# bergmanlab/TELR

Hardware: AMD Instinct MI355X
Metric: gbp_aligned_per_s (higher is better)
Workload: dtype int16

## Files before the change

### __graft_entry__.py

```python
import os
import sys

ROOT = os.path.dirname(os.path.abspath(__file__))
if ROOT not in sys.path:
    sys.path.insert(0, ROOT)


def build():
    from telr_amd import build as tb
    tb.build(verbose=True)
    from oracle import binding as ob
    ob.build()
    import telr_amd
    from telr_amd import _lib
    _lib.lib()


def smoke():
    import numpy as np
    from telr_amd.aligner import Engine
    from telr_amd.presets import preset
    from telr_amd.fasta import read_fasta
    from oracle import binding as ob
    d = os.path.join(ROOT, "tests", "data")
    _, ts = read_fasta(os.path.join(d, "ref_38kb.fasta"))
    _, qs = read_fasta(os.path.join(d, "reads.fasta"))
    eng = Engine(0)
    print("device:", eng.device_name())
    for pname in ("ngmlr-ont", "map-ont"):
        io, mo = preset(pname)
        ix = eng.index(ts, io)
        res = ix.map(qs, mo)
        ref = ob.OracleIndex(ts, io).map(qs, mo)
        assert len(res.alns) == len(ref["alns"]) and len(res.alns) > 0
        for f in ("qid", "tid", "qs", "qe", "ts", "te", "mlen", "blen", "dp_score", "flags", "mapq", "n_cigar"):
            np.testing.assert_array_equal(res.alns[f], ref["alns"][f], err_msg=pname + " " + f)
        for i in range(len(res.alns)):
            a, b = res.alns[i], ref["alns"][i]
            np.testing.assert_array_equal(res.cigars[a["cigar_off"]:a["cigar_off"] + a["n_cigar"]],
                                          ref["cigars"][b["cigar_off"]:b["cigar_off"] + b["n_cigar"]])
        print("smoke ok (%s): %d alignment records, bit-exact vs oracle" % (pname, len(res.alns)))


if __name__ == "__main__":
    build()
    if "--smoke" in sys.argv:
        smoke()
```

### telr_amd/_lib.py

```python
import ctypes as C
import os
from ._abi import IdxOpt, MapOpt, Aln, Counters, InsOpt, GenoOpt, DraftOpt, BridgeOpt, RefTeOpt, N_STAGES

os.environ.setdefault("GPU_MAX_HW_QUEUES", "2")
_HERE = os.path.dirname(os.path.abspath(__file__))
SO_PATH = os.environ.get("TELR_LIB") or os.path.join(_HERE, "libtelrhip.so")

EXPORTS = [
    "telr_init", "telr_destroy", "telr_strerror", "telr_last_error", "telr_device_name", "telr_preset",
    "telr_seqset_create", "telr_seqset_subset", "telr_seqset_subset_rc", "telr_seqset_free", "telr_seqset_bases", "telr_seqset_count",
    "telr_index_build", "telr_index_free", "telr_index_stats", "telr_map",
    "telr_result_from_arrays", "telr_result_count", "telr_result_alns", "telr_result_cigar_count", "telr_result_cigars", "telr_result_wait", "telr_result_free",
    "telr_init_background", "telr_release_scratch", "telr_device_mem", "telr_write_paf", "telr_write_sam", "telr_write_bam", "telr_write_bam_dev", "telr_bam_prepare", "telr_bam_release_wait", "telr_bam_discard", "telr_write_bam_slice", "telr_bam_segment_info", "telr_bam_segment_entries", "telr_bam_segment_write", "telr_bam_segment_free", "telr_bai_write", "telr_result_from_device_cigars", "telr_seqset_packed", "telr_seqset_from_packed", "telr_consensus_build", "telr_poa_build", "telr_consensus_count", "telr_consensus_seq", "telr_consensus_off", "telr_consensus_len", "telr_consensus_free", "telr_fasta_load", "telr_fasta_count", "telr_fasta_bases", "telr_fasta_extent", "telr_fasta_seq", "telr_fasta_off", "telr_fasta_len", "telr_fasta_names", "telr_fasta_free", "telr_depth_medians", "telr_window_reads", "telr_stage_ms", "telr_stage_name", "telr_last_counters", "telr_last_dp_classes",
    "telr_seqset_attach_qual", "telr_seqset_has_qual", "telr_fasta_qual", "telr_fasta_qual_off", "telr_write_sam_qual", "telr_write_bam_qual",
    "telr_ins_opt_default", "telr_call_insertions", "telr_ins_calls_count", "telr_ins_calls_calls", "telr_ins_calls_sig_count", "telr_ins_calls_sigs",
    "telr_ins_calls_read_off", "telr_ins_calls_reads", "telr_ins_calls_free",
    "telr_geno_opt_default", "telr_genotype_insertions", "telr_ins_geno_count", "telr_ins_geno_gt", "telr_ins_geno_ref_off", "telr_ins_geno_ref_reads",
    "telr_ins_geno_ambig_off", "telr_ins_geno_ambig_reads", "telr_ins_geno_free",
    "telr_draft_opt_default", "telr_draft_contigs", "telr_drafts_count", "telr_drafts_data", "telr_draft_contigs_free",
    "telr_bam_load", "telr_bam_in_free", "telr_bam_in_target_count", "telr_bam_in_target_names", "telr_bam_in_target_lens", "telr_bam_in_read_count",
    "telr_bam_in_read_names", "telr_bam_in_read_lens", "telr_bam_in_seqset", "telr_bam_in_result", "telr_bam_in_detach_seqset", "telr_bam_in_detach_result",
    "telr_bam_in_counters", "telr_bam_in_ascii", "telr_bam_in_phase_ms", "telr_bam_load_chunked", "telr_bam_chunk_plan", "telr_bam_in_chunk_info",
    "telr_seqset_extract", "telr_seqset_pieces", "telr_seqset_join",
    "telr_bridge_opt_default", "telr_bridge_contigs", "telr_bridges_count", "telr_bridges_data", "telr_bridge_contigs_free",
# ... 22 lines not shown
    L = C.CDLL(SO_PATH)
    vp, i32, i64, cp = C.c_void_p, C.c_int32, C.c_int64, C.c_char_p
    L.telr_init.restype = C.c_int; L.telr_init.argtypes = [C.c_int, C.POINTER(vp)]
    L.telr_init_background.restype = C.c_int; L.telr_init_background.argtypes = [C.c_int, C.POINTER(vp)]
    L.telr_release_scratch.restype = C.c_int; L.telr_release_scratch.argtypes = [vp]
    L.telr_device_mem.restype = C.c_int; L.telr_device_mem.argtypes = [vp, C.POINTER(i64), C.POINTER(i64)]
    L.telr_destroy.restype = None; L.telr_destroy.argtypes = [vp]
    L.telr_strerror.restype = cp; L.telr_strerror.argtypes = [C.c_int]
    L.telr_last_error.restype = cp; L.telr_last_error.argtypes = [vp]
    L.telr_device_name.restype = C.c_int; L.telr_device_name.argtypes = [vp, cp, C.c_int]
    L.telr_preset.restype = C.c_int; L.telr_preset.argtypes = [cp, C.POINTER(IdxOpt), C.POINTER(MapOpt)]
    L.telr_seqset_create.restype = C.c_int; L.telr_seqset_create.argtypes = [vp, i32, vp, vp, vp, C.POINTER(vp)]
    L.telr_seqset_subset.restype = C.c_int; L.telr_seqset_subset.argtypes = [vp, vp, i32, vp, C.POINTER(vp)]
    L.telr_seqset_subset_rc.restype = C.c_int; L.telr_seqset_subset_rc.argtypes = [vp, vp, i32, vp, vp, C.POINTER(vp)]
    L.telr_seqset_packed.restype = C.c_int; L.telr_seqset_packed.argtypes = [vp, C.POINTER(vp), C.POINTER(vp), C.POINTER(i64), C.POINTER(i64)]
    L.telr_seqset_from_packed.restype = C.c_int; L.telr_seqset_from_packed.argtypes = [vp, i32, vp, vp, i64, vp, i64, C.POINTER(vp)]
    L.telr_seqset_free.restype = None; L.telr_seqset_free.argtypes = [vp]
    L.telr_seqset_bases.restype = i64; L.telr_seqset_bases.argtypes = [vp]
    L.telr_seqset_count.restype = i32; L.telr_seqset_count.argtypes = [vp]
    L.telr_seqset_attach_qual.restype = C.c_int; L.telr_seqset_attach_qual.argtypes = [vp, vp, vp, vp, i32]
    L.telr_seqset_has_qual.restype = C.c_int; L.telr_seqset_has_qual.argtypes = [vp]
    L.telr_seqset_extract.restype = C.c_int; L.telr_seqset_extract.argtypes = [vp, vp, i64, vp, vp, vp, vp, vp, vp]
    L.telr_seqset_pieces.restype = C.c_int; L.telr_seqset_pieces.argtypes = [vp, vp, i32, vp, vp, vp, vp, C.POINTER(vp)]
    L.telr_seqset_join.restype = C.c_int; L.telr_seqset_join.argtypes = [vp, vp, i32, vp, vp, vp, vp, vp, C.POINTER(vp)]
    L.telr_tile_plan.restype = C.c_int; L.telr_tile_plan.argtypes = [i32, vp, i32, i32, vp, i64, C.POINTER(i64)]
    L.telr_refte_opt_default.restype = None; L.telr_refte_opt_default.argtypes = [C.POINTER(RefTeOpt)]
    L.telr_annotate_hits.restype = C.c_int; L.telr_annotate_hits.argtypes = [vp, vp, i64, vp, i32, vp, i32, C.POINTER(RefTeOpt), C.POINTER(vp)]
    L.telr_te_feats_count.restype = i64; L.telr_te_feats_count.argtypes = [vp]
    L.telr_te_feats_data.restype = vp; L.telr_te_feats_data.argtypes = [vp]
    L.telr_te_feats_free.restype = None; L.telr_te_feats_free.argtypes = [vp]
    L.telr_index_build.restype = C.c_int; L.telr_index_build.argtypes = [vp, vp, C.POINTER(IdxOpt), C.POINTER(vp)]
    L.telr_index_free.restype = None; L.telr_index_free.argtypes = [vp]
    L.telr_index_stats.restype = C.c_int; L.telr_index_stats.argtypes = [vp, C.POINTER(i64), C.POINTER(i64)]
    L.telr_map.restype = C.c_int; L.telr_map.argtypes = [vp, vp, vp, vp, C.POINTER(MapOpt), C.POINTER(vp)]
    L.telr_result_from_arrays.restype = C.c_int; L.telr_result_from_arrays.argtypes = [vp, vp, i64, vp, i64, C.POINTER(vp)]
    L.telr_result_count.restype = i64; L.telr_result_count.argtypes = [vp]
    L.telr_result_alns.restype = vp; L.telr_result_alns.argtypes = [vp]
    L.telr_result_cigar_count.restype = i64; L.telr_result_cigar_count.argtypes = [vp]
    L.telr_result_cigars.restype = vp; L.telr_result_cigars.argtypes = [vp]
    L.telr_result_wait.restype = C.c_int; L.telr_result_wait.argtypes = [vp]
    L.telr_result_free.restype = None; L.telr_result_free.argtypes = [vp]
    L.telr_depth_medians.restype = C.c_int
    L.telr_depth_medians.argtypes = [vp, vp, i32, vp, i32, vp, vp, vp, vp]
    L.telr_ins_opt_default.restype = None; L.telr_ins_opt_default.argtypes = [C.POINTER(InsOpt)]
    L.telr_call_insertions.restype = C.c_int; L.telr_call_insertions.argtypes = [vp, vp, i32, C.POINTER(InsOpt), C.POINTER(vp)]
    for fn in ("telr_ins_calls_count", "telr_ins_calls_sig_count"):
        getattr(L, fn).restype = i64; getattr(L, fn).argtypes = [vp]
    for fn in ("telr_ins_calls_calls", "telr_ins_calls_sigs", "telr_ins_calls_read_off", "telr_ins_calls_reads"):
        getattr(L, fn).restype = vp; getattr(L, fn).argtypes = [vp]
    L.telr_ins_calls_free.restype = None; L.telr_ins_calls_free.argtypes = [vp]
    L.telr_geno_opt_default.restype = None; L.telr_geno_opt_default.argtypes = [C.POINTER(GenoOpt)]
    L.telr_genotype_insertions.restype = C.c_int; L.telr_genotype_insertions.argtypes = [vp, vp, i32, i64, vp, vp, vp, C.POINTER(GenoOpt), C.POINTER(vp)]
    L.telr_ins_geno_count.restype = i64; L.telr_ins_geno_count.argtypes = [vp]
    for fn in ("telr_ins_geno_gt", "telr_ins_geno_ref_off", "telr_ins_geno_ref_reads", "telr_ins_geno_ambig_off", "telr_ins_geno_ambig_reads"):
        getattr(L, fn).restype = vp; getattr(L, fn).argtypes = [vp]
    L.telr_ins_geno_free.restype = None; L.telr_ins_geno_free.argtypes = [vp]
    L.telr_draft_opt_default.restype = None; L.telr_draft_opt_default.argtypes = [C.POINTER(DraftOpt)]
    L.telr_draft_contigs.restype = C.c_int
    L.telr_draft_contigs.argtypes = [vp, vp, i32, i64, vp, vp, vp, i64, vp, vp, C.POINTER(DraftOpt), C.POINTER(vp), C.POINTER(vp)]
    L.telr_drafts_count.restype = i64; L.telr_drafts_count.argtypes = [vp]
    L.telr_drafts_data.restype = vp; L.telr_drafts_data.argtypes = [vp]
    L.telr_draft_contigs_free.restype = None; L.telr_draft_contigs_free.argtypes = [vp]
    L.telr_bridge_opt_default.restype = None; L.telr_bridge_opt_default.argtypes = [C.POINTER(BridgeOpt)]
    L.telr_bridge_contigs.restype = C.c_int
    L.telr_bridge_contigs.argtypes = [vp, vp, i32, i64, vp, vp, vp, i64, vp, vp, vp, C.POINTER(BridgeOpt), C.POINTER(vp)]
    L.telr_bridges_count.restype = i64; L.telr_bridges_count.argtypes = [vp]
    L.telr_bridges_data.restype = vp; L.telr_bridges_data.argtypes = [vp]
    L.telr_bridge_contigs_free.restype = None; L.telr_bridge_contigs_free.argtypes = [vp]
    L.telr_bam_load.restype = C.c_int; L.telr_bam_load.argtypes = [vp, cp, i32, C.POINTER(vp)]
    L.telr_bam_in_free.restype = None; L.telr_bam_in_free.argtypes = [vp]
    for fn in ("telr_bam_in_target_count", "telr_bam_in_read_count"):
        getattr(L, fn).restype = i32; getattr(L, fn).argtypes = [vp]
    for fn in ("telr_bam_in_target_names", "telr_bam_in_target_lens", "telr_bam_in_read_names", "telr_bam_in_read_lens", "telr_bam_in_seqset", "telr_bam_in_result",
               "telr_bam_in_detach_seqset", "telr_bam_in_detach_result"):
        getattr(L, fn).restype = vp; getattr(L, fn).argtypes = [vp]
    L.telr_bam_in_counters.restype = C.c_int; L.telr_bam_in_counters.argtypes = [vp, vp]
    L.telr_bam_in_ascii.restype = C.c_int; L.telr_bam_in_ascii.argtypes = [vp, vp, vp]
    L.telr_bam_in_phase_ms.restype = C.c_int; L.telr_bam_in_phase_ms.argtypes = [vp, vp]
    L.telr_bam_load_chunked.restype = C.c_int; L.telr_bam_load_chunked.argtypes = [vp, cp, i32, i64, C.POINTER(vp)]
    L.telr_bam_chunk_plan.restype = C.c_int; L.telr_bam_chunk_plan.argtypes = [i64, vp, i64, vp, i64, C.POINTER(i64)]
    L.telr_bam_in_chunk_info.restype = C.c_int; L.telr_bam_in_chunk_info.argtypes = [vp, vp]
    L.telr_reads_load.restype = C.c_int; L.telr_reads_load.argtypes = [vp, cp, i32, i64, C.POINTER(vp)]
    L.telr_reads_in_free.restype = None; L.telr_reads_in_free.argtypes = [vp]
    L.telr_reads_in_count.restype = i32; L.telr_reads_in_count.argtypes = [vp]
    for fn in ("telr_reads_in_names", "telr_reads_in_lens", "telr_reads_in_seqset", "telr_reads_in_detach_seqset"):
        getattr(L, fn).restype = vp; getattr(L, fn).argtypes = [vp]
    for fn in ("telr_reads_in_counters", "telr_reads_in_chunk_info", "telr_reads_in_phase_ms"):
        getattr(L, fn).restype = C.c_int; getattr(L, fn).argtypes = [vp, vp]
    L.telr_debug_bgzf_inflate.restype = C.c_int; L.telr_debug_bgzf_inflate.argtypes = [vp, cp, vp, i64, C.POINTER(i64)]
    L.telr_debug_seqset_qual.restype = i64; L.telr_debug_seqset_qual.argtypes = [vp, vp, i64]
    L.telr_window_reads.restype = C.c_int; L.telr_window_reads.argtypes = [vp, i64, i32, vp, vp, vp, vp, vp, i64, vp]
    L.telr_write_paf.restype = C.c_int; L.telr_write_paf.argtypes = [vp, vp, vp, C.c_int, cp, C.c_int]
    L.telr_write_sam.restype = C.c_int
    L.telr_write_sam.argtypes = [vp, i32, vp, vp, vp, vp, i32, vp, vp, vp, vp, i32, cp, cp, cp, cp, cp]
    L.telr_write_bam.restype = C.c_int
    L.telr_write_bam.argtypes = [vp, i32, vp, vp, vp, vp, i32, vp, vp, vp, vp, i32, cp, cp, cp, cp, cp, i32, i32]
    L.telr_write_sam_qual.restype = C.c_int
    L.telr_write_sam_qual.argtypes = L.telr_write_sam.argtypes + [vp, vp, i32]
    L.telr_write_bam_qual.restype = C.c_int
    L.telr_write_bam_qual.argtypes = L.telr_write_bam.argtypes + [vp, vp, i32]
    L.telr_write_bam_dev.restype = C.c_int
    L.telr_write_bam_dev.argtypes = [vp, vp, vp, vp, vp, vp, i32, cp, cp, cp, cp, cp, i32, i32]
    L.telr_write_bam_dev_targets.restype = C.c_int
    L.telr_write_bam_dev_targets.argtypes = L.telr_write_bam_dev.argtypes
    L.telr_part_plan.restype = C.c_int; L.telr_part_plan.argtypes = [i32, vp, i64, vp, C.POINTER(i32)]
    L.telr_part_plan_error.restype = cp; L.telr_part_plan_error.argtypes = []
    L.telr_merge_parts.restype = C.c_int; L.telr_merge_parts.argtypes = [vp, i32, vp, vp, vp, i32, C.POINTER(MapOpt), C.POINTER(vp)]
    L.telr_debug_merge_ms.restype = C.c_int; L.telr_debug_merge_ms.argtypes = [vp]
    L.telr_fasta_load.restype = C.c_int; L.telr_fasta_load.argtypes = [cp, C.POINTER(vp)]
    L.telr_fasta_count.restype = i32; L.telr_fasta_count.argtypes = [vp]
    L.telr_fasta_bases.restype = i64; L.telr_fasta_bases.argtypes = [vp]
    L.telr_fasta_extent.restype = i64; L.telr_fasta_extent.argtypes = [vp]
    for fn in ("telr_fasta_seq", "telr_fasta_off", "telr_fasta_len", "telr_fasta_names", "telr_fasta_qual", "telr_fasta_qual_off"):
        getattr(L, fn).restype = vp; getattr(L, fn).argtypes = [vp]
    L.telr_fasta_free.restype = None; L.telr_fasta_free.argtypes = [vp]
    L.telr_consensus_build.restype = C.c_int; L.telr_consensus_build.argtypes = [vp, vp, vp, vp, i32, C.POINTER(vp)]
    L.telr_poa_build.restype = C.c_int; L.telr_poa_build.argtypes = [vp, vp, vp, vp, i32, C.POINTER(vp)]
    L.telr_consensus_count.restype = i32; L.telr_consensus_count.argtypes = [vp]
    for fn in ("telr_consensus_seq", "telr_consensus_off", "telr_consensus_len"):
        getattr(L, fn).restype = vp; getattr(L, fn).argtypes = [vp]
    L.telr_consensus_free.restype = None; L.telr_consensus_free.argtypes = [vp]
    L.telr_bam_prepare.restype = C.c_int; L.telr_bam_prepare.argtypes = [vp, cp, i64]
    L.telr_bam_release_wait.restype = C.c_int; L.telr_bam_release_wait.argtypes = []
    L.telr_bam_discard.restype = C.c_int; L.telr_bam_discard.argtypes = [vp]
    L.telr_write_bam_slice.restype = C.c_int; L.telr_write_bam_slice.argtypes = [vp, vp, vp, vp, vp, vp, i32, cp, cp, cp, cp, vp, i32, i32, C.POINTER(vp)]
    L.telr_bam_segment_info.restype = C.c_int; L.telr_bam_segment_info.argtypes = [vp, vp]
    L.telr_bam_segment_entries.restype = C.c_int; L.telr_bam_segment_entries.argtypes = [vp, i64, vp, vp, vp, vp, vp]
    L.telr_bam_segment_write.restype = C.c_int; L.telr_bam_segment_write.argtypes = [vp, vp, cp, i64, i32]
    L.telr_bam_segment_free.restype = None; L.telr_bam_segment_free.argtypes = [vp]
    L.telr_bai_write.restype = C.c_int; L.telr_bai_write.argtypes = [cp, i64, vp, vp, vp, vp, C.c_uint64, i64, i32, vp]
    L.telr_result_from_device_cigars.restype = C.c_int; L.telr_result_from_device_cigars.argtypes = [vp, vp, i64, vp, i64, C.POINTER(vp)]
    L.telr_debug_bam_twin.restype = C.c_int; L.telr_debug_bam_twin.argtypes = []
    L.telr_debug_result_twin.restype = i64; L.telr_debug_result_twin.argtypes = [vp, vp, i64]
    L.telr_debug_bam_sink_ms.restype = C.c_int; L.telr_debug_bam_sink_ms.argtypes = [vp]
    L.telr_debug_bam_ms.restype = C.c_int; L.telr_debug_bam_ms.argtypes = [vp]
    L.telr_debug_huff.restype = C.c_int; L.telr_debug_huff.argtypes = [vp, i32, i32, vp]
    L.telr_debug_check_records.restype = C.c_int; L.telr_debug_check_records.argtypes = [vp, i64, vp, i64, vp, i32, vp, i32, C.POINTER(i64)]
    L.telr_debug_deflate_host.restype = C.c_int; L.telr_debug_deflate_host.argtypes = [vp, i32, vp, i32, vp]
    L.telr_stage_ms.restype = C.c_int; L.telr_stage_ms.argtypes = [vp, vp]
    L.telr_stage_name.restype = cp; L.telr_stage_name.argtypes = [C.c_int]
    L.telr_last_counters.restype = C.c_int; L.telr_last_counters.argtypes = [vp, C.POINTER(Counters)]
    L.telr_last_dp_classes.restype = C.c_int; L.telr_last_dp_classes.argtypes = [vp, vp]
    L.telr_debug_n_anchor.restype = i64; L.telr_debug_n_anchor.argtypes = [vp]
    L.telr_debug_dp_retries.restype = i64; L.telr_debug_dp_retries.argtypes = [vp]
    L.telr_debug_pk_launches.restype = i64; L.telr_debug_pk_launches.argtypes = [vp]
    L.telr_debug_fetch.restype = C.c_int; L.telr_debug_fetch.argtypes = [vp, cp, vp, i64]
    L.telr_debug_n_chain.restype = i64; L.telr_debug_n_chain.argtypes = [vp]
    L.telr_debug_chains.restype = vp; L.telr_debug_chains.argtypes = [vp]
    L.telr_debug_index.restype = C.c_int; L.telr_debug_index.argtypes = [vp, vp, vp, vp, vp]
    L.telr_debug_pack.restype = C.c_int; L.telr_debug_pack.argtypes = [cp, i32, C.c_int, vp, vp]
    L.telr_debug_mid_occ.restype = i32; L.telr_debug_mid_occ.argtypes = [vp, C.POINTER(MapOpt)]
    L.telr_debug_dp_limits.restype = C.c_int; L.telr_debug_dp_limits.argtypes = [C.POINTER(MapOpt), vp]
    L.telr_debug_dp_class_table.restype = C.c_int; L.telr_debug_dp_class_table.argtypes = [vp]
    L.telr_debug_map_plan.restype = C.c_int; L.telr_debug_map_plan.argtypes = [vp, i32, i32, C.c_double, C.c_int, C.c_int, C.c_int, C.c_int, vp, vp]
    L.telr_debug_dp.restype = C.c_int; L.telr_debug_dp.argtypes = [vp, vp, vp, C.POINTER(MapOpt), vp, i32, vp, vp, vp, i64]
    L.telr_debug_stitch.restype = C.c_int; L.telr_debug_stitch.argtypes = [vp, i32, vp, vp, vp, vp, vp, i32, vp, vp, i64]
    L.telr_debug_align.restype = C.c_int
    L.telr_debug_align.argtypes = [vp, vp, vp, C.POINTER(MapOpt), i32, vp, vp, vp, vp, vp, vp, i64, C.POINTER(i32), vp]
    L.telr_debug_chain.restype = C.c_int; L.telr_debug_chain.argtypes = [vp, i32, vp, vp, C.POINTER(MapOpt), vp, vp]
    L.telr_debug_backtrack.restype = C.c_int
    L.telr_debug_backtrack.argtypes = [vp, i32, vp, vp, vp, vp, vp, i32, vp, vp, C.POINTER(MapOpt), vp, vp, vp, vp, vp, vp, vp, i64, vp]
    _lib = L
    return L
```

### telr_amd/aligner.py

```python
import ctypes as C
import numpy as np
from . import _lib
from ._abi import IdxOpt, MapOpt, Counters, InsOpt, GenoOpt, DraftOpt, BridgeOpt, RefTeOpt, ALN_DTYPE, INS_SIG_DTYPE, INS_CALL_DTYPE, GENO_DTYPE, DRAFT_DTYPE, BRIDGE_DTYPE, TILE_DTYPE, \
    TE_FEAT_DTYPE, TELR_E_ARG, TELR_E_RANGE, MF_PER_TARGET, MF_KEEP_CIGARS, N_STAGES, N_DPCLS, STITCH_CHAIN_COLUMNS, ALIGN_CHAIN_COLUMNS, ALIGN_PROB_COLUMNS
from .fasta import concat

BAM_CHUNK_FIT = -1

def _np_from(ptr, n, dtype):
    if n == 0 or not ptr:
        return np.zeros(0, dtype=dtype)
    dt = np.dtype(dtype)
    buf = (C.c_char * (n * dt.itemsize)).from_address(ptr)
    return np.frombuffer(buf, dtype=dt, count=n).copy()


def _ic_arrays(entry, ic, with_sigs=False):
    calls = np.ascontiguousarray(ic.calls, dtype=INS_CALL_DTYPE)
    sigs = np.ascontiguousarray(ic.sigs, dtype=INS_SIG_DTYPE) if with_sigs else None
    read_off = np.ascontiguousarray(ic.read_off, dtype=np.int64)
    reads = np.ascontiguousarray(ic.reads, dtype=np.int32)
    if len(read_off) != len(calls) + 1 or (len(calls) and int(read_off[-1]) > len(reads)):
        raise _lib.TelrError("%s: read_off must hold len(calls) + 1 offsets into reads" % entry)
    return calls, read_off, reads, sigs


def _qual_arrays(qual):
    if isinstance(qual, tuple) and len(qual) == 2:
        buf, off = qual
    else:
        buf, off, _ = concat([q.encode("latin-1") if isinstance(q, str) else q for q in qual])
    return np.ascontiguousarray(buf, dtype=np.uint8), np.ascontiguousarray(off, dtype=np.int64)


_DEFERRED = None


class deferred_frees:

    def __enter__(self):
        global _DEFERRED
        self.outer = _DEFERRED
        if _DEFERRED is None:
            _DEFERRED = []
        return self

    def __exit__(self, *exc):
        global _DEFERRED
        if self.outer is None:
            todo, _DEFERRED = _DEFERRED, None
            for fn, h in todo:
                fn(h)
        return False


class Engine:

    def __init__(self, device=0, background=False):
        self.L = _lib.lib()
        h = C.c_void_p()
        rc = (self.L.telr_init_background if background else self.L.telr_init)(device, C.byref(h))
        if rc != 0:
            raise _lib.TelrError("telr_init(%d): %s" % (device, self.L.telr_strerror(rc).decode()))
        self.h = h
        self.device = device

    def _chk(self, rc, what):
        if rc != 0:
            raise _lib.TelrError("%s: %s [%s]" % (what, self.L.telr_strerror(rc).decode(),
                                                  self.L.telr_last_error(self.h).decode()))

    def device_name(self):
        b = C.create_string_buffer(256)
        self.L.telr_device_name(self.h, b, 256)
        return b.value.decode()

    def seqset(self, seqs, qual=None):
        return SeqSet(self, seqs, qual)

    def index(self, targets, io):
        return Index(self, targets, io)

    @staticmethod
    def part_plan(lengths, max_bases=0):
        a = np.ascontiguousarray(lengths, dtype=np.int32)
        L = _lib.lib()
        part_of = np.zeros(max(len(a), 1), np.int32); n = C.c_int32(0)
        rc = L.telr_part_plan(len(a), a.ctypes.data, int(max_bases), part_of.ctypes.data, C.byref(n))
        if rc != 0:
            raise _lib.TelrError("telr_part_plan: %s [%s]" % (L.telr_strerror(rc).decode(), L.telr_part_plan_error().decode()), rc)
        return part_of[:len(a)]

    def index_parts(self, targets, io, max_part_bases=0, like=None):
        return PartIndex(self, targets, io, max_part_bases, like)

    @staticmethod
    def bam_chunk_plan(isize, chunk_bytes):
        a = np.ascontiguousarray(isize, dtype=np.int32)
        L = _lib.lib()
        first = np.zeros(max(len(a), 1), np.int64); n = C.c_int64(0)
        rc = L.telr_bam_chunk_plan(len(a), a.ctypes.data, int(chunk_bytes), first.ctypes.data, len(a), C.byref(n))
        if rc != 0:
            raise _lib.TelrError("telr_bam_chunk_plan: %s" % L.telr_strerror(rc).decode(), rc)
        return first[:int(n.value)]

    def load_bam(self, path, keep_qual=False, chunk_bytes=None):
        return BamInput(self, path, keep_qual, chunk_bytes)

    def load_reads(self, path, keep_qual=False, chunk_bytes=0):
        return ReadsInput(self, path, keep_qual, chunk_bytes)

    def stage_ms(self):
        a = np.zeros(N_STAGES, np.float32)
        self.L.telr_stage_ms(self.h, a.ctypes.data)
        return {self.L.telr_stage_name(i).decode(): float(a[i]) for i in range(N_STAGES)}

    def counters(self):
        c = Counters()
        self.L.telr_last_counters(self.h, C.byref(c))
        return {k: getattr(c, k) for k, _ in Counters._fields_}

    def dp_classes(self):
        a = np.zeros(N_DPCLS * 4, np.int64)
        self.L.telr_last_dp_classes(self.h, a.ctypes.data)
        return a.reshape(N_DPCLS, 4)

    DP_LIMITS = ("pk_steps_limit", "pk_wide_limit", "pk_wide_maxd", "pk_ext_limit", "pk_ext_maxd", "tb4_mask", "tb4_steps", "tag8_steps")

    @staticmethod
    def dp_limits(mo):
        a = np.zeros(8, np.int32)
        rc = _lib.lib().telr_debug_dp_limits(C.byref(mo), a.ctypes.data)
        if rc != 0:
            raise _lib.TelrError("telr_debug_dp_limits: %d" % rc, rc)
        return dict(zip(Engine.DP_LIMITS, (int(v) for v in a)))

    DP_CLASS_COLUMNS = ("maxd", "lanes", "regs", "row_dwords", "interleaved", "tiled")

    @staticmethod
    def dp_class_table():
        a = np.zeros((N_DPCLS, 6), np.int32)
        rc = _lib.lib().telr_debug_dp_class_table(a.ctypes.data)
        if rc != 0:
            raise _lib.TelrError("telr_debug_dp_class_table: %d" % rc, rc)
        return a

    MAP_PLAN_MODES = ("serial", "in_turn", "two_in_flight")

    @staticmethod
    def map_plan(lengths, per_base=0.0, qtarget=False, vote=False, debug=0, pipe_nomem=False):
        a = np.ascontiguousarray(lengths, dtype=np.int32)
        out = np.zeros(3, np.int64); ends = np.zeros(max(len(a), 1), np.int32)
        rc = _lib.lib().telr_debug_map_plan(a.ctypes.data, len(a), int(a.max()) if len(a) else 0, float(per_base), int(bool(qtarget)),
                                            int(bool(vote)), int(debug), int(bool(pipe_nomem)), out.ctypes.data, ends.ctypes.data)
        if rc != 0:
            raise _lib.TelrError("telr_debug_map_plan: %d" % rc, rc)
        return Engine.MAP_PLAN_MODES[int(out[0])], int(out[1]), [int(e) for e in ends[:int(out[2])]]

    @staticmethod
    def tile_plan(lengths, tile, stride):
        a = np.ascontiguousarray(lengths, dtype=np.int32)
        L = _lib.lib()
        need = C.c_int64(0)
        rc = L.telr_tile_plan(len(a), a.ctypes.data, int(tile), int(stride), None, 0, C.byref(need))
        if rc != 0 and not (rc == TELR_E_RANGE and need.value > 0):
            raise _lib.TelrError("telr_tile_plan: %s" % L.telr_strerror(rc).decode(), rc)
        out = np.zeros(need.value, TILE_DTYPE)
        if need.value:
            rc = L.telr_tile_plan(len(a), a.ctypes.data, int(tile), int(stride), out.ctypes.data, len(out), C.byref(need))
            if rc != 0:
                raise _lib.TelrError("telr_tile_plan: %s" % L.telr_strerror(rc).decode(), rc)
        return out

    def annotate_hits(self, r, tiles, target_len, n_families, opt=None):
        o = RefTeOpt.default() if opt is None else opt
        tiles = np.ascontiguousarray(tiles, dtype=TILE_DTYPE)
        tl = np.ascontiguousarray(target_len, dtype=np.int32)
        h = C.c_void_p()
        L = self.L
        rc = L.telr_annotate_hits(self.h, r, len(tiles), tiles.ctypes.data, len(tl), tl.ctypes.data, int(n_families), C.byref(o), C.byref(h))
        if rc != 0:
            raise _lib.TelrError("telr_annotate_hits: %s [%s]" % (L.telr_strerror(rc).decode(), L.telr_last_error(self.h).decode()), rc)
        try:
            return _np_from(L.telr_te_feats_data(h), int(L.telr_te_feats_count(h)), TE_FEAT_DTYPE)
        finally:
            L.telr_te_feats_free(h)

    def debug_dp(self, queries, targets, mo, probs):
        P = np.ascontiguousarray(probs, dtype=np.int32).reshape(-1, 12)
        npb = len(P)
        res = np.zeros((npb, 8), np.int32); tb = np.zeros(npb, np.int64)
        steps = P[:, 4].astype(np.int64) + P[:, 5]
        cap = int((6 * steps + 16).sum()) + 16
        cig = np.zeros(cap, np.uint32)
        self._chk(self.L.telr_debug_dp(self.h, queries.h, targets.h, C.byref(mo), P.ctypes.data, npb, res.ctypes.data,
                                       tb.ctypes.data, cig.ctypes.data, cap), "telr_debug_dp")
        out = {k: res[:, i].copy() for i, k in enumerate(("cls", "retry", "score", "bi", "bj", "mlen"))}
        out["tb_off"] = tb
        out["cigars"] = [cig[res[x, 7]:res[x, 7] + res[x, 6]].copy() for x in range(npb)]
        return out

    def debug_stitch(self, p_off, has_left, prob, cigars, cx_scale=0):
        O = np.ascontiguousarray(p_off, dtype=np.int32)
        HL = np.ascontiguousarray(has_left, dtype=np.int32)
        P = np.ascontiguousarray(prob, dtype=np.int32).reshape(-1, 5)
        if len(O) < 1 or len(HL) != len(O) - 1 or len(cigars) != len(P) or (len(O) > 1 and int(O[-1]) != len(P)):
            raise _lib.TelrError("telr_debug_stitch: p_off must hold n_chain + 1 offsets ending at the problem count", TELR_E_ARG)
        co = np.zeros(len(P) + 1, np.int64)
        co[1:] = np.cumsum([len(c) for c in cigars])
        raw = np.ascontiguousarray(np.concatenate([np.asarray(c, np.uint32) for c in cigars]) if len(cigars) else np.zeros(0), dtype=np.uint32)
        nk, cap = len(O) - 1, len(raw) + 1
        out = np.zeros((nk, len(STITCH_CHAIN_COLUMNS)), np.int32); cig = np.zeros(cap, np.uint32)
        self._chk(self.L.telr_debug_stitch(self.h, nk, O.ctypes.data, HL.ctypes.data, P.ctypes.data, co.ctypes.data, raw.ctypes.data, int(cx_scale),
                                           out.ctypes.data, cig.ctypes.data, cap), "telr_debug_stitch")
        r = {k: out[:, i].copy() for i, k in enumerate(STITCH_CHAIN_COLUMNS[:-1])}
        r["cigars"] = [cig[out[k, 8]:out[k, 8] + out[k, 7]].copy() for k in range(nk)]
        return r

    def debug_align(self, queries, targets, mo, chains, prob_off, probs):
        Cn = np.ascontiguousarray(chains, dtype=np.int32).reshape(-1, 7)
        O = np.ascontiguousarray(prob_off, dtype=np.int32)
        P = np.ascontiguousarray(probs, dtype=np.int32).reshape(-1, 12)
        if len(O) != len(Cn) + 1 or (len(Cn) and int(O[-1]) != len(P)):
            raise _lib.TelrError("telr_debug_align: prob_off must hold n_chain + 1 offsets ending at the problem count", TELR_E_ARG)
        nk, npb = len(Cn), len(P)
        cap = int((P[:, 4].astype(np.int64) + P[:, 5] + 2).sum()) + 16
        co = np.zeros((nk, len(ALIGN_CHAIN_COLUMNS)), np.int32); po = np.zeros((npb, len(ALIGN_PROB_COLUMNS)), np.int32)
        cig = np.zeros(cap, np.uint32); acc = np.zeros(N_DPCLS * 4 + 1, np.int64); n_retry = C.c_int32(0)
        self._chk(self.L.telr_debug_align(self.h, queries.h, targets.h, C.byref(mo), nk, Cn.ctypes.data, O.ctypes.data, P.ctypes.data, co.ctypes.data,
                                          po.ctypes.data, cig.ctypes.data, cap, C.byref(n_retry), acc.ctypes.data), "telr_debug_align")
        return dict(chains={k: co[:, i].copy() for i, k in enumerate(ALIGN_CHAIN_COLUMNS[:-1])},
                    cigars=[cig[co[k, 8]:co[k, 8] + co[k, 7]].copy() for k in range(nk)],
                    probs={k: po[:, i].copy() for i, k in enumerate(ALIGN_PROB_COLUMNS)}, n_retry=int(n_retry.value), acc=acc)

    def debug_chain(self, keys, q_aoff, mo):
        K = np.ascontiguousarray(keys, dtype=np.uint64)
        O = np.ascontiguousarray(q_aoff, dtype=np.int32)
        if len(O) < 1 or int(O[-1]) != len(K):
            raise ValueError("q_aoff must hold nq + 1 offsets ending at len(keys)")
        f = np.zeros(len(K), np.int32); p = np.zeros(len(K), np.int32)
        self._chk(self.L.telr_debug_chain(self.h, len(O) - 1, K.ctypes.data, O.ctypes.data, C.byref(mo), f.ctypes.data, p.ctypes.data),
                  "telr_debug_chain")
        return f, p

    def debug_backtrack(self, keys, q_aoff, f, p, qlen, goff, tlen, mo):
        K = np.ascontiguousarray(keys, dtype=np.uint64)
        O = np.ascontiguousarray(q_aoff, dtype=np.int32)
        F = np.ascontiguousarray(f, dtype=np.int32); P = np.ascontiguousarray(p, dtype=np.int32)
        QL = np.ascontiguousarray(qlen, dtype=np.int32)
        G = np.ascontiguousarray(goff, dtype=np.uint32); TL = np.ascontiguousarray(tlen, dtype=np.int32)
        nq, nt, na = len(O) - 1, len(TL), len(K)
        if nq < 0 or len(F) != na or len(P) != na or len(QL) != nq or len(G) != nt + 1:
            raise ValueError("array lengths: q_aoff nq + 1, f / p one per key, qlen nq, goff n_targets + 1")
        if nq < 1 or int(O[-1]) != na:
            raise _lib.TelrError("telr_debug_backtrack: q_aoff must hold nq + 1 >= 2 offsets ending at len(keys)")
        cap = 3 * na + 8
        ch_off = np.zeros(nq + 1, np.int32); chains = np.zeros((na + 1, 9), np.int32); ch_aoff = np.zeros(na + 2, np.int32)
        canch = np.zeros(na + 1, np.uint64); kept = np.zeros((na + 1, 10), np.int32); prob_off = np.zeros(na + 2, np.int32)
        probs = np.zeros((cap, 12), np.int32); n_out = np.zeros(3, np.int64)
        self._chk(self.L.telr_debug_backtrack(self.h, nq, O.ctypes.data, K.ctypes.data, F.ctypes.data, P.ctypes.data, QL.ctypes.data, nt,
                                              G.ctypes.data, TL.ctypes.data, C.byref(mo), ch_off.ctypes.data, chains.ctypes.data,
                                              ch_aoff.ctypes.data, canch.ctypes.data, kept.ctypes.data, prob_off.ctypes.data,
                                              probs.ctypes.data, cap, n_out.ctypes.data), "telr_debug_backtrack")
        nch, nk, npb = (int(v) for v in n_out)
        return dict(chains=chains[:nch].copy(), ch_off=ch_off, ch_aoff=ch_aoff[:nch + 1].copy(), canch=canch[:int(ch_aoff[nch])].copy(),
                    kept=kept[:nk].copy(), prob_off=prob_off[:nk + 1].copy(), probs=probs[:npb].copy())

    def release_scratch(self):
        self._chk(self.L.telr_release_scratch(self.h), "telr_release_scratch")

    def mem_info(self):
        fr, tot = C.c_int64(), C.c_int64()
        self._chk(self.L.telr_device_mem(self.h, C.byref(fr), C.byref(tot)), "telr_device_mem")
        return fr.value, tot.value

    def worker(self):
        w = getattr(self, "_worker", None)
        if w is None:
            w = self._worker = Engine(self.device, background=True)
        return w

    def close(self):
        w = getattr(self, "_worker", None)
        if w is not None:
            self._worker = None
            w.close()
        if getattr(self, "h", None):
            self.L.telr_destroy(self.h)
# ... 722 lines not shown
```

### telr_amd/build.py

```python
import os
import subprocess
import sys

HERE = os.path.dirname(os.path.abspath(__file__))
SRC = os.path.join(HERE, "csrc")
SO = os.path.join(HERE, "libtelrhip.so")
SOURCES = ["telr_engine.hip"]
DEPS = sorted(f for f in os.listdir(SRC) if f.endswith((".hip", ".h"))) + ["../../include/telr_hip.h"]


def needs_build():
    if not os.path.exists(SO):
        return True
    t = os.path.getmtime(SO)
    return any(os.path.getmtime(os.path.join(SRC, d)) > t for d in DEPS)


def build(force=False, verbose=False):
    if not force and not needs_build():
        return SO
    hipcc = os.environ.get("HIPCC", "/opt/rocm/bin/hipcc")
    cmd = [hipcc, "-O3", "-std=c++17", "--offload-arch=gfx950", "-fPIC", "-shared", "-o", SO] + \
          os.environ.get("TELR_EXTRA_FLAGS", "").split() + [os.path.join(SRC, s) for s in SOURCES] + ["-lz"]
    if verbose:
        print(" ".join(cmd), file=sys.stderr)
    subprocess.check_call(cmd)
    return SO


if __name__ == "__main__":
    build(force="--force" in sys.argv, verbose=True)
    print(SO)
```

### telr_amd/csrc/kernels.hip.h

```cpp
#pragma once
#include <hip/hip_runtime.h>
#include <stdint.h>

#define TELR_NEG      (-(1 << 28))
#include "part_plan.h"
#define SK_TILE       1024
#define SK_THREADS    256
#define DP_DMAX       4096

struct ChainOpt {
    int32_t max_gap, bw, min_cnt, min_chain_score, chain_gap_q8, chain_skip_q8;
    int32_t dense_n, dense_span, mw_n;
};
struct DpOpt {
    int32_t a, b, q, e, q2, e2, sc_ambi, zdrop;
    int32_t cx_scale, cx_open, cx_emax, cx_emin, cx_dec, cx_flat;
};
__host__ __device__ __forceinline__ int d_cx_ext(const DpOpt &o, int len) { int v = o.cx_emax - o.cx_dec * len; return v > o.cx_emin ? v : o.cx_emin; }
__host__ __device__ __forceinline__ int d_cx_cost(const DpOpt &o, int L)
{
    int t = o.cx_open;
    for (int i = 0; i < L && i < o.cx_flat; ++i) t += d_cx_ext(o, i);
    if (L > o.cx_flat) t += (L - o.cx_flat) * o.cx_emin;
    return t;
// ... 2162 lines not shown
    return c < 0 ? (int)CLS_LDSMAX : c;
}
template <typename F> constexpr uint32_t dp_cls_mask(F f) { uint32_t m = 0; for (int c = 0; c < DP_NCLS; ++c) if (f(DP_CLASS[c])) m |= 1u << c; return m; }
constexpr bool dp_row_is_reg(const DpClassRow &r) { return r.layout != TBL_BYTES; }
constexpr bool dp_row_is_rows2(const DpClassRow &r) { return r.layout == TBL_LINES || r.layout == TBL_TILES || r.layout == TBL_INTERLEAVED; }
constexpr bool dp_row_is_tiled(const DpClassRow &r) { return r.layout == TBL_TILES; }
constexpr bool dp_row_is_interleaved(const DpClassRow &r) { return r.layout == TBL_INTERLEAVED; }
constexpr bool dp_row_counts_cells(const DpClassRow &r) { return r.family == DPF_PK || r.family == DPF_PKW; }
constexpr bool dp_row_is_pk(const DpClassRow &r) { return r.family == DPF_PK; }
constexpr uint32_t CLSM_REGS = dp_cls_mask(dp_row_is_reg), CLSM_ROWS2 = dp_cls_mask(dp_row_is_rows2), CLSM_TILED = dp_cls_mask(dp_row_is_tiled),
                   CLSM_INTERLEAVED = dp_cls_mask(dp_row_is_interleaved), CLSM_CELLS = dp_cls_mask(dp_row_counts_cells), CLSM_PK = dp_cls_mask(dp_row_is_pk);
__host__ __device__ __forceinline__ constexpr bool d_cls_in(int cls, uint32_t mask) { return (mask >> cls) & 1u; }
constexpr int CLS_REGS_FIRST = __builtin_ctz(CLSM_REGS), CLS_ROWS2_FIRST = __builtin_ctz(CLSM_ROWS2);
static_assert(CLSM_REGS == ((1u << DP_NCLS) - (1u << CLS_REGS_FIRST)) && CLSM_ROWS2 == ((1u << DP_NCLS) - (1u << CLS_ROWS2_FIRST)), "these layouts take the upper class numbers");
__host__ __device__ __forceinline__ bool d_tb_regs(int cls) { return cls >= CLS_REGS_FIRST; }
__host__ __device__ __forceinline__ bool d_tb_rows2(int cls) { return cls >= CLS_ROWS2_FIRST; }
__host__ __device__ __forceinline__ bool d_tb_tiled(int cls) { return d_cls_in(cls, CLSM_TILED); }
__host__ __device__ __forceinline__ bool d_tb_interleaved(int cls) { return d_cls_in(cls, CLSM_INTERLEAVED); }
__host__ __device__ __forceinline__ int d_cls_slots(int cls) { return DP_CLASS[cls].slots; }
__host__ __device__ __forceinline__ int d_onep_d(int q, int e, int q2, int e2) { return e > e2 ? (q2 - q + (e - e2) - 1) / (e - e2) : 1 << 20; }
__host__ __device__ __forceinline__ bool d_tb4(int cls, int tb4) { return (DP_CLASS[cls].nibble & tb4) != 0; }
__host__ __device__ __forceinline__ int d_tb4_rowb(int cls) { return 4 * ((DP_CLASS[cls].regs + 1) / 2); }
__device__ __forceinline__ bool d_any_n(const uint32_t *__restrict__ nmask, int64_t lo, int n)
{
    if (n <= 0) return false;
    const int64_t hi = lo + n - 1;
    for (int64_t w = lo >> 5; w <= (hi >> 5); ++w) {
        uint32_t m = nmask[w];
        if (w == (lo >> 5)) m &= ~0u << (int)(lo & 31);
        if (w == (hi >> 5)) m &= ~0u >> (31 - (int)(hi & 31));
        if (m) return true;
    }
    return false;
}
__global__ void k_prob_sizes(DpProb *__restrict__ probs, int32_t np, int fill_margin, DpLimits L,
                             const uint32_t *__restrict__ qnmask, const uint32_t *__restrict__ tnmask,
                             int64_t *__restrict__ tb_bytes, int64_t *__restrict__ cig_ops)
{
    int i = blockIdx.x * blockDim.x + threadIdx.x;
    if (i >= np) return;
    const DpProb P = probs[i];
    int D = P.dhi - P.dlo + 1, stride = (D + 2) / 2;
    int cls = d_dp_class(P.kind, D, P.m + P.n, L);
    if (d_tb_rows2(cls) && P.kind < 3) {
        const bool hasn = d_any_n(qnmask, P.qstep > 0 ? P.qi0 : P.qi0 - P.m + 1, P.m) || d_any_n(tnmask, P.tstep > 0 ? P.ti0 : P.ti0 - P.n + 1, P.n);
        if (hasn) { DpLimits L0 = L; L0.pk_steps = L0.pk_ext = L0.pk_wide = 0; cls = d_dp_class(P.kind, D, P.m + P.n, L0); }
    }
    const int tb4 = L.tb4_mask;
    if (d_tb4(cls, tb4) && P.m + P.n > L.tb4_steps) cls = CLS_PK40;
    int64_t tb;
    if (P.kind == 5) {
        const int S = P.m < P.n ? P.m : P.n, lm = P.m < S + P.dhi ? P.m : S + P.dhi, ln = P.n < S + P.dhi ? P.n : S + P.dhi;
        tb = (2 * (int64_t)(lm + ln + 1) * (D * 4 + stride) + 127) & ~127LL;
    }
    else if (P.kind >= 3) tb = 0;
    else if (d_tb4(cls, tb4)) tb = ((int64_t)(((P.m + P.n) / 2 + 2) / 2) * (2 * d_tb4_rowb(cls)) + 63) & ~63LL;
    else if (d_tb_tiled(cls)) tb = (int64_t)(((P.m + P.n) / 2 + 4) / 4) * d_cls_slots(cls) * 16;
    else if (d_tb_rows2(cls)) tb = ((int64_t)((P.m + P.n) / 2 + 1) * d_cls_slots(cls) * 4 + 63) & ~63LL;
    else if (d_tb_regs(cls)) tb = (int64_t)((P.m + P.n) / 4 + 1) * d_cls_slots(cls) * 4;
    else tb = ((int64_t)(P.m + P.n + 1) * stride + 127) & ~127LL;
    int cells = 0;
    if (d_cls_in(cls, CLSM_CELLS)) for (int d = P.dlo; d <= P.dhi; ++d) {
        int ilo = d < 0 ? 1 - d : 1, ihi = P.n - d < P.m ? P.n - d : P.m;
        if (ihi >= ilo) cells += ihi - ilo + 1;
    }
    probs[i].pad[0] = cls | (fill_margin << 8); probs[i].pad[1] = cells;
    tb_bytes[i] = tb;
    if (P.kind == 5) { const int S = P.m < P.n ? P.m : P.n; cig_ops[i] = 3 * (int64_t)(2 * (S + P.dhi) + 2); }
    else cig_ops[i] = P.kind == 3 ? 2 : (int64_t)P.m + P.n;
}
struct ClsOff { int32_t off[DP_NCLS + 1]; };
__device__ __forceinline__ int d_cls_of_pos(const ClsOff &off, int i) { int c = 0; while (c < DP_NCLS - 1 && i >= off.off[c + 1]) ++c; return c; }
__global__ void __launch_bounds__(256) k_tb_gather(const int64_t *__restrict__ tb_bytes, const int32_t *__restrict__ list, int32_t np, ClsOff off, int64_t *__restrict__ out)
{
    const int32_t i = blockIdx.x * blockDim.x + threadIdx.x;
    if (i == np) out[np] = 0;
    if (i >= np) return;
    const int c = d_cls_of_pos(off, i);
    if (!d_tb_interleaved(c)) { out[i] = tb_bytes[list[i]]; return; }
    const int first = off.off[c] + ((i - off.off[c]) & ~63);
    const int last = first + 63 < off.off[c + 1] - 1 ? first + 63 : off.off[c + 1] - 1;
    out[i] = i == last ? tb_bytes[list[first]] * 64 : 0;
}
__global__ void __launch_bounds__(256) k_tb_scatter(DpProb *__restrict__ probs, const int32_t *__restrict__ list, int32_t np, ClsOff off, const int64_t *__restrict__ toff)
{
    const int32_t i = blockIdx.x * blockDim.x + threadIdx.x;
    if (i >= np) return;
    const int c = d_cls_of_pos(off, i);
    probs[list[i]].tb_off = toff[i] + (d_tb_interleaved(c) ? (int64_t)((i - off.off[c]) & 63) * 8 : 0);
}
__global__ void __launch_bounds__(256) k_prob_assign(DpProb *__restrict__ probs, int32_t np, const int64_t *__restrict__ tb_off, const int64_t *__restrict__ cig_off,
                                                     int32_t *__restrict__ cls_cnt, uint32_t *__restrict__ sort_key, int32_t *__restrict__ sort_val)
{
    __shared__ int32_t lcnt[DP_NCLS];
    int i = blockIdx.x * blockDim.x + threadIdx.x;
    if (threadIdx.x < DP_NCLS) lcnt[threadIdx.x] = 0;
    __syncthreads();
    if (i < np) {
        probs[i].tb_off = tb_off[i];
        if (cig_off) probs[i].cig_off = cig_off[i];
        const int c = probs[i].kind >= 3 ? 0 : (probs[i].pad[0] & 0xff);
        atomicAdd(&lcnt[c], 1);
        int steps = probs[i].m + probs[i].n; if (steps > 0x7FFFF) steps = 0x7FFFF;
        sort_key[i] = (uint32_t)c << 19 | (uint32_t)(0x7FFFF - steps);
        sort_val[i] = i;
    }
    __syncthreads();
    if (threadIdx.x < DP_NCLS && lcnt[threadIdx.x]) atomicAdd(&cls_cnt[threadIdx.x], lcnt[threadIdx.x]);
}

__global__ void k_retry_collect(const int32_t *__restrict__ flag, int32_t np, int32_t *__restrict__ cnt, int32_t *__restrict__ list)
{
    const int i = blockIdx.x * blockDim.x + threadIdx.x;
    const bool f = i < np && flag[i];
    const uint64_t m = __ballot(f);
    if (!m) return;
    const int lane = threadIdx.x & 63;
    int base = 0;
    if (lane == __ffsll((unsigned long long)m) - 1) base = atomicAdd(cnt, __popcll(m));
    base = __shfl(base, __ffsll((unsigned long long)m) - 1);
    if (f) list[base + __popcll(m & ((1ULL << lane) - 1))] = i;
}
__global__ void k_retry_build(const DpProb *__restrict__ probs, const int32_t *__restrict__ list, int32_t n, int32_t bw, int32_t band_q4, DpProb *__restrict__ out)
{
    int k = blockIdx.x * blockDim.x + threadIdx.x;
    if (k >= n) return;
    DpProb P = probs[list[k]];
    const int W = d_fill_band(P.m, P.n, bw, band_q4), W2 = d_fill_band_wide(P.m, P.n, bw, band_q4), dl = P.n - P.m;
    const int lo = d_even_lo((dl < 0 ? dl : 0) - W2), hi = (dl > 0 ? dl : 0) + W2;
    P.chain = list[k];
    P.pad[1] = 0;
    if (W2 > W && hi - lo + 1 <= DP_DMAX) { P.dlo = lo; P.dhi = hi; P.kind = 0; } else P.kind = 4;
    out[k] = P;
}
__global__ void k_retry_merge(const DpProb *__restrict__ probs2, const DpRes *__restrict__ res2, int32_t n, DpRes *__restrict__ res)
{
    int k = blockIdx.x * blockDim.x + threadIdx.x;
    if (k >= n || probs2[k].kind == 4) return;
    DpRes r = res2[k];
    r.cells += res[probs2[k].chain].cells;
    res[probs2[k].chain] = r;
}

struct DpArgs {
    const uint32_t *qseq2, *qnmask, *tseq2, *tnmask;
    int64_t qtot, ttot;
    const DpProb *probs; const int32_t *list; int32_t nlist;
    DpOpt o;
    uint8_t *tb; uint32_t *cig; DpRes *res;
    int32_t dcap;
    int32_t *retry;
    int32_t tb4;
    int32_t tag8_steps;
};

__device__ __forceinline__ int64_t d_wave_max64(int64_t v)
{
#pragma unroll
    for (int o = 32; o >= 1; o >>= 1) {
        int64_t w = (int64_t)((uint64_t)(uint32_t)__shfl_xor((int)(uint32_t)v, o) | (uint64_t)(uint32_t)__shfl_xor((int)(uint32_t)((uint64_t)v >> 32), o) << 32);
        v = w > v ? w : v;
    }
    return v;
}

__device__ __forceinline__ uint32_t d_cell(const DpOpt &o, int32_t hd, int32_t hl, int32_t e1l, int32_t e2l, int32_t hu, int32_t f1u, int32_t f2u,
                                           int qb, int tbv, int32_t &h, int32_t &ve1, int32_t &vf1, int32_t &ve2, int32_t &vf2)
{
    uint32_t t = 0; int32_t op, g;
    if (o.cx_scale) {
        const int le = e2l < 0 ? 0 : e2l > o.cx_flat ? o.cx_flat : e2l, lf = f2u < 0 ? 0 : f2u > o.cx_flat ? o.cx_flat : f2u;
        op = hl - o.cx_open - d_cx_ext(o, 0); g = e1l - d_cx_ext(o, le); if (g > op) { ve1 = g; t |= 8; ve2 = le + 1; } else { ve1 = op; ve2 = 1; }
        op = hu - o.cx_open - d_cx_ext(o, 0); g = f1u - d_cx_ext(o, lf); if (g > op) { vf1 = g; t |= 16; vf2 = lf + 1; } else { vf1 = op; vf2 = 1; }
        if (ve2 > o.cx_flat) ve2 = o.cx_flat;
        if (vf2 > o.cx_flat) vf2 = o.cx_flat;
        int scx;
        if (qb > 3 || tbv > 3) scx = -o.sc_ambi; else if (qb == tbv) { scx = o.a; t |= 128; } else scx = -o.b;
        h = hd + scx; uint32_t srcx = 0;
        if (ve1 > h) { h = ve1; srcx = 1; }
        if (vf1 > h) { h = vf1; srcx = 2; }
        return t | srcx;
    }
    op = hl - o.q - o.e;   g = e1l - o.e;  if (g > op) { ve1 = g; t |= 8; }  else ve1 = op;
    op = hu - o.q - o.e;   g = f1u - o.e;  if (g > op) { vf1 = g; t |= 16; } else vf1 = op;
    op = hl - o.q2 - o.e2; g = e2l - o.e2; if (g > op) { ve2 = g; t |= 32; } else ve2 = op;
    op = hu - o.q2 - o.e2; g = f2u - o.e2; if (g > op) { vf2 = g; t |= 64; } else vf2 = op;
    int sc;
    if (qb > 3 || tbv > 3) sc = -o.sc_ambi; else if (qb == tbv) { sc = o.a; t |= 128; } else sc = -o.b;
    h = hd + sc; uint32_t src = 0;
    if (ve1 > h) { h = ve1; src = 1; }
    if (vf1 > h) { h = vf1; src = 2; }
    if (ve2 > h) { h = ve2; src = 3; }
    if (vf2 > h) { h = vf2; src = 4; }
    return t | src;
}

__device__ __forceinline__ void d_wave_sync() { __builtin_amdgcn_fence(__ATOMIC_ACQ_REL, "workgroup"); __builtin_amdgcn_wave_barrier(); __builtin_amdgcn_fence(__ATOMIC_ACQ_REL, "workgroup"); }
__device__ __forceinline__ void d_longgap_half(const DpArgs &A, const DpProb &P, int side, int lm, int ln, int m, int n, int lane, int32_t *lds,
                                               int32_t *Hg, uint8_t *tbg, int &ncell)
{
    const DpOpt o = A.o;
    const int dlo = P.dlo, dhi = P.dhi, D = dhi - dlo + 1, stride = (D + 2) / 2;
    const int qstep = side ? -P.qstep : P.qstep, tstep = side ? -P.tstep : P.tstep;
    const int64_t qi0 = side ? P.qi0 + (int64_t)P.qstep * (m - 1) : P.qi0, ti0 = side ? P.ti0 + (int64_t)P.tstep * (n - 1) : P.ti0;
    int32_t *H = lds, *E1 = H + (A.dcap + 2), *F1 = E1 + (A.dcap + 2), *E2 = F1 + (A.dcap + 2), *F2 = E2 + (A.dcap + 2);
    d_wave_sync();
    for (int x = lane; x < D + 2; x += 64) { H[x] = TELR_NEG; E1[x] = TELR_NEG; F1[x] = TELR_NEG; E2[x] = TELR_NEG; F2[x] = TELR_NEG; }
    d_wave_sync();
    if (lane == 0) { H[0 - dlo + 1] = 0; Hg[0 - dlo] = 0; }
    d_wave_sync();
    for (int a = 1; a <= lm + ln; ++a) {
        int d0 = -a > dlo ? -a : dlo; if (a - 2 * lm > d0) d0 = a - 2 * lm;
        int d1 = a < dhi ? a : dhi;   if (2 * ln - a < d1) d1 = 2 * ln - a;
        if (((d0 - a) & 1) != 0) ++d0;
        for (int d = d0 + 2 * lane; d <= d1; d += 128) {
            const int i = (a - d) >> 1, j = (a + d) >> 1, x = d - dlo + 1;
            int32_t h, ve1, vf1, ve2, vf2;
            if (i == 0) { ve1 = -(o.q + j * o.e); ve2 = -(o.q2 + j * o.e2); vf1 = vf2 = TELR_NEG; h = ve1 > ve2 ? ve1 : ve2; }
            else if (j == 0) { vf1 = -(o.q + i * o.e); vf2 = -(o.q2 + i * o.e2); ve1 = ve2 = TELR_NEG; h = vf1 > vf2 ? vf1 : vf2; }
            else {
                int qb = d_base(A.qseq2, A.qnmask, qi0 + (int64_t)qstep * (i - 1));
                int tbv = d_base(A.tseq2, A.tnmask, ti0 + (int64_t)tstep * (j - 1));
                if (P.qcomp && qb < 4) qb = 3 - qb;
                const uint32_t t = d_cell(o, H[x], H[x - 1], E1[x - 1], E2[x - 1], H[x + 1], F1[x + 1], F2[x + 1], qb, tbv, h, ve1, vf1, ve2, vf2);
                tbg[(int64_t)a * stride + ((d - dlo) >> 1)] = (uint8_t)t;
                ++ncell;
            }
            if (h < TELR_NEG) h = TELR_NEG;
            if (ve1 < TELR_NEG) ve1 = TELR_NEG;
            if (vf1 < TELR_NEG) vf1 = TELR_NEG;
            if (ve2 < TELR_NEG) ve2 = TELR_NEG;
            if (vf2 < TELR_NEG) vf2 = TELR_NEG;
            H[x] = h; E1[x] = ve1; F1[x] = vf1; E2[x] = ve2; F2[x] = vf2;
            Hg[(int64_t)a * D + (d - dlo)] = h;
        }
        d_wave_sync();
    }
}
__device__ __forceinline__ int d_longgap_walk(const uint8_t *tbg, int dlo, int stride, int i, int j, uint32_t *out, int no, int &mcols, int &mlen)
{
    int state = 0;
    auto push = [&](uint32_t op) { if (no > 0 && (out[no - 1] & 0xfu) == op) out[no - 1] += 16u; else out[no++] = 16u | op; };
    while (i > 0 && j > 0) {
        const uint32_t t = tbg[(int64_t)(i + j) * stride + ((j - i - dlo) >> 1)];
        if (state == 0) state = (int)(t & 7u);
        if (state == 0) { push(0u); ++mcols; mlen += (int)(t >> 7 & 1u); --i; --j; }
        else if (state == 1) { push(2u); if (!(t & 8u))  state = 0; --j; }
        else if (state == 2) { push(1u); if (!(t & 16u)) state = 0; --i; }
        else if (state == 3) { push(2u); if (!(t & 32u)) state = 0; --j; }
        else                 { push(1u); if (!(t & 64u)) state = 0; --i; }
    }
    if (i > 0) { if (no > 0 && (out[no - 1] & 0xfu) == 1u) out[no - 1] += (uint32_t)i << 4; else out[no++] = (uint32_t)i << 4 | 1u; }
    if (j > 0) { if (no > 0 && (out[no - 1] & 0xfu) == 2u) out[no - 1] += (uint32_t)j << 4; else out[no++] = (uint32_t)j << 4 | 2u; }
    return no;
}
__device__ void d_longgap(const DpArgs &A, const DpProb &P, int prob, int lane, int32_t *lds)
{
    const DpOpt o = A.o;
    const int m = P.m, n = P.n, ins = m > n, S = ins ? n : m, W = P.dhi, dlo = P.dlo, D = P.dhi - dlo + 1, stride = (D + 2) / 2;
    const int lm = m < S + W ? m : S + W, ln = n < S + W ? n : S + W, na = lm + ln + 1;
    uint8_t *base = A.tb + P.tb_off;
    int32_t *HL = (int32_t*)base, *HR = HL + (int64_t)na * D;
    uint8_t *tbL = (uint8_t*)(HR + (int64_t)na * D), *tbR = tbL + (int64_t)na * stride;
    int ncell = 0;
    d_longgap_half(A, P, 0, lm, ln, m, n, lane, lds, HL, tbL, ncell);
    d_longgap_half(A, P, 1, lm, ln, m, n, lane, lds, HR, tbR, ncell);
    __threadfence_block();
    d_wave_sync();
    const int lim = ins ? lm : ln;
    int64_t bestk = INT64_MIN; int b_al = 0, b_ar = 0;
    for (int c = lane; c <= S; c += 64) {
        int64_t vl = INT64_MIN, vr = INT64_MIN; int al = 0, ar = 0;
        for (int k = c - W; k <= c + W; ++k) {
            if (k < 0 || k > lim) continue;
            const int i = ins ? k : c, j = ins ? c : k, d = j - i;
            if (d < dlo || d > P.dhi) continue;
            const int32_t h = HL[(int64_t)(i + j) * D + (d - dlo)];
            if (h <= TELR_NEG / 2) continue;
            const int64_t v = (int64_t)h + (int64_t)o.e2 * k;
            if (v > vl) { vl = v; al = k; }
        }
        const int c2 = S - c;
        for (int k = c2 - W; k <= c2 + W; ++k) {
            if (k < 0 || k > lim) continue;
            const int i = ins ? k : c2, j = ins ? c2 : k, d = j - i;
            if (d < dlo || d > P.dhi) continue;
            const int32_t h = HR[(int64_t)(i + j) * D + (d - dlo)];
            if (h <= TELR_NEG / 2) continue;
            const int64_t v = (int64_t)h + (int64_t)o.e2 * k;
            if (v > vr) { vr = v; ar = k; }
        }
        if (vl == INT64_MIN || vr == INT64_MIN) continue;
        if ((ins ? m : n) - al - ar < 1) continue;
        const int64_t key = (vl + vr) * 65536LL + (int64_t)(0xffff - c);
        if (key > bestk) { bestk = key; b_al = al; b_ar = ar; }
    }
    const int64_t wk = d_wave_max64(bestk);
    const uint64_t who = __ballot(bestk == wk);
    const int src = __ffsll((unsigned long long)who) - 1;
    const int bc = 0xffff - (int)(wk & 0xffff), al = __shfl(b_al, src), ar = __shfl(b_ar, src);
    int nc = ncell;
#pragma unroll
    for (int s = 32; s >= 1; s >>= 1) nc += __shfl_xor(nc, s);
    if (lane == 0) {
        const int g = (ins ? m : n) - al - ar;
        const int li = ins ? al : bc, lj = ins ? bc : al, ri = ins ? ar : S - bc, rj = ins ? S - bc : ar;
// ... 255 lines not shown
    uint32_t tbw[R];
#pragma unroll
    for (int r = 0; r < R; ++r) tbw[r] = 0;
    int ncell = 0;
    for (int a = 1; a <= amax; ++a) {
        const int sh = 8 * (a & 3);
        if (a & 1) {
            if ((((a - 1) >> 1) & 31) == 0) d_stream_fill(TS, A.tseq2, A.tnmask, P.ti0, ts_, ((a + de0 + 1) >> 1) + R - 2, 0, A.ttot);
#pragma unroll
            for (int r = 0; r < R - 1; ++r) tbs[r] = tbs[r + 1];
            tbs[R - 1] = d_stream_next(TS);
            int32_t hu = DPP_SHL1(TELR_NEG, He[0]), f1u = DPP_SHL1(TELR_NEG, F1e[0]), f2u = DPP_SHL1(TELR_NEG, F2e[0]);
            if (LPP < 64 && l == LPP - 1) { hu = TELR_NEG; f1u = TELR_NEG; f2u = TELR_NEG; }
            if (NW > 1 && wl == 63 && wv < NW - 1) { const int32_t *x = xch + (0 * NW + wv + 1) * 3; hu = x[0]; f1u = x[1]; f2u = x[2]; }
#pragma unroll
            for (int r = 0; r < R; ++r) {
                const int32_t uh = r < R - 1 ? He[r < R - 1 ? r + 1 : r] : hu, uf1 = r < R - 1 ? F1e[r < R - 1 ? r + 1 : r] : f1u, uf2 = r < R - 1 ? F2e[r < R - 1 ? r + 1 : r] : f2u;
                if ((uint32_t)(a - aloO[r]) <= (uint32_t)spanO[r]) {
                    int32_t h, ve1, vf1, ve2, vf2;
                    uint32_t t = d_cell_nc(o, Ho[r], He[r], E1e[r], E2e[r], uh, uf1, uf2, qbs[r], tbs[r], h, ve1, vf1, ve2, vf2);
                    tbw[r] |= t << sh; ++ncell;
                    Ho[r] = h; E1o[r] = ve1; F1o[r] = vf1; E2o[r] = ve2; F2o[r] = vf2;
                }
            }
        } else {
            if ((((a >> 1) - 1) & 31) == 0) d_stream_fill(QS, A.qseq2, A.qnmask, P.qi0, qs_, ((a - de0) >> 1) - 1, P.qcomp, A.qtot);
#pragma unroll
            for (int r = R - 1; r > 0; --r) qbs[r] = qbs[r - 1];
            qbs[0] = d_stream_next(QS);
            int32_t hl = DPP_SHR1(TELR_NEG, Ho[R - 1]), e1l = DPP_SHR1(TELR_NEG, E1o[R - 1]), e2l = DPP_SHR1(TELR_NEG, E2o[R - 1]);
            if (LPP < 64 && l == 0) { hl = TELR_NEG; e1l = TELR_NEG; e2l = TELR_NEG; }
            if (NW > 1 && wl == 0 && wv > 0) { const int32_t *x = xch + (1 * NW + wv - 1) * 3; hl = x[0]; e1l = x[1]; e2l = x[2]; }
#pragma unroll
            for (int r = R - 1; r >= 0; --r) {
                const int32_t lh = r > 0 ? Ho[r > 0 ? r - 1 : 0] : hl, le1 = r > 0 ? E1o[r > 0 ? r - 1 : 0] : e1l, le2 = r > 0 ? E2o[r > 0 ? r - 1 : 0] : e2l;
                if ((uint32_t)(a - aloE[r]) <= (uint32_t)spanE[r]) {
                    int32_t h, ve1, vf1, ve2, vf2;
                    uint32_t t = d_cell_nc(o, He[r], lh, le1, le2, Ho[r], F1o[r], F2o[r], qbs[r], tbs[r], h, ve1, vf1, ve2, vf2);
                    tbw[r] |= t << sh; ++ncell;
                    He[r] = h; E1e[r] = ve1; F1e[r] = vf1; E2e[r] = ve2; F2e[r] = vf2;
                }
            }
        }
        if (NW > 1) {
            if (a & 1) { if (wl == 63) { int32_t *x = xch + (1 * NW + wv) * 3; x[0] = Ho[R - 1]; x[1] = E1o[R - 1]; x[2] = E2o[R - 1]; } }
            else if (wl == 0) { int32_t *x = xch + (0 * NW + wv) * 3; x[0] = He[0]; x[1] = F1e[0]; x[2] = F2e[0]; }
            __syncthreads();
        }
        if ((a & 3) == 3 || a == amax) {
            if ((a >> 2) <= last_row) {
#pragma unroll
                for (int r = 0; r < R; ++r) tb32[(int64_t)(a >> 2) * SLOTS + l * R + r] = tbw[r];
            }
#pragma unroll
            for (int r = 0; r < R; ++r) tbw[r] = 0;
        }
    }
#pragma unroll
    for (int s = (NW > 1 ? 32 : LPP / 2); s >= 1; s >>= 1) ncell += __shfl_xor(ncell, s);
    if (NW > 1) {
        if (wl == 0) atomicAdd(&ncell_sh, ncell);
        __syncthreads();
        ncell = ncell_sh;
    }
    if (have) {
        const int xf = (n - m) - de0;
        if (xf >= 0 && xf < 2 * R) {
            int32_t sc = TELR_NEG;
#pragma unroll
            for (int r = 0; r < R; ++r) { if (xf == 2 * r) sc = He[r]; if (xf == 2 * r + 1) sc = Ho[r]; }
            DpRes Rr; Rr.score = sc; Rr.bi = m; Rr.bj = n; Rr.nops = 0; Rr.mlen = 0; Rr.cells = ncell; Rr.tbases = n; Rr.mcols = 0;
            A.res[prob] = Rr;
        }
    }
}

typedef short pk_s2 __attribute__((ext_vector_type(2)));
__device__ __forceinline__ pk_s2 PKS(uint32_t v) { return __builtin_bit_cast(pk_s2, v); }
__device__ __forceinline__ uint32_t PKU(pk_s2 v) { return __builtin_bit_cast(uint32_t, v); }
__device__ __forceinline__ uint32_t pk_add(uint32_t a, uint32_t b) { return PKU(PKS(a) + PKS(b)); }
__device__ __forceinline__ uint32_t pk_sub(uint32_t a, uint32_t b) { return PKU(PKS(a) - PKS(b)); }
__device__ __forceinline__ uint32_t pk_max(uint32_t a, uint32_t b) { return PKU(__builtin_elementwise_max(PKS(a), PKS(b))); }
__device__ __forceinline__ uint32_t pk_min(uint32_t a, uint32_t b) { return PKU(__builtin_elementwise_min(PKS(a), PKS(b))); }
__device__ __forceinline__ uint32_t pk_mul(uint32_t a, uint32_t b) { return PKU(PKS(a) * PKS(b)); }
__device__ __forceinline__ uint32_t pk_sign(uint32_t a)
{
    uint32_t r;
    asm("v_pk_ashrrev_i16 %0, 15, %1 op_sel_hi:[0,1]" : "=v"(r) : "v"(a));
    return r;
}
__device__ __forceinline__ uint32_t pk_sel(uint32_t m, uint32_t a, uint32_t b)
{
    uint32_t r;
    asm("v_bfi_b32 %0, %1, %2, %3" : "=v"(r) : "v"(m), "v"(a), "v"(b));
    return r;
}
__device__ __forceinline__ uint32_t pk_dup(int v) { return ((uint32_t)v & 0xffffu) * 0x00010001u; }
#define PK_NEG 0xC000C000u
#ifdef TB_NT
typedef uint32_t tb_u2 __attribute__((ext_vector_type(2)));
#define TB_ST2(p, a, b) __builtin_nontemporal_store(tb_u2{(a), (b)}, (tb_u2*)(p))
#define TB_LD2(p) ({ const tb_u2 v_ = __builtin_nontemporal_load((const tb_u2*)(p)); make_uint2(v_.x, v_.y); })
#else
#define TB_ST2(p, a, b) (*(uint2*)(p) = make_uint2((a), (b)))
#define TB_LD2(p) (*(const uint2*)(p))
#endif

struct PkConst { uint32_t qe, e, q2e2, e2, ab, b, a, nab, qeF, q2e2F;
                 uint32_t cx_oe0, cx_e1, cx_emin, cx_dec; };

template <bool ONEP = false>
__device__ __forceinline__ uint32_t d_cell_pk(const PkConst &c, uint32_t hd, uint32_t hl, uint32_t e1l, uint32_t e2l, uint32_t hu, uint32_t f1u, uint32_t f2u,
                                              uint32_t qb, uint32_t tbv, uint32_t &h, uint32_t &ve1, uint32_t &vf1, uint32_t &ve2, uint32_t &vf2)
{
    uint32_t op, g, t;
    op = pk_sub(hl, c.qe);   g = pk_sub(e1l, c.e);  ve1 = pk_max(op, g); t  = pk_sign(pk_sub(op, g)) & 0x00080008u;
    op = pk_sub(hu, c.qe);   g = pk_sub(f1u, c.e);  vf1 = pk_max(op, g); t |= pk_sign(pk_sub(op, g)) & 0x00100010u;
    if (!ONEP) {
        op = pk_sub(hl, c.q2e2); g = pk_sub(e2l, c.e2); ve2 = pk_max(op, g); t |= pk_sign(pk_sub(op, g)) & 0x00200020u;
        op = pk_sub(hu, c.q2e2); g = pk_sub(f2u, c.e2); vf2 = pk_max(op, g); t |= pk_sign(pk_sub(op, g)) & 0x00400040u;
    } else { ve2 = PK_NEG; vf2 = PK_NEG; }
    const uint32_t eq = pk_sign(pk_sub(qb ^ tbv, 0x00010001u));
    const uint32_t sc = pk_sub(eq & c.ab, c.b);
    t |= eq & 0x00800080u;
    h = pk_add(hd, sc);
    uint32_t m, src;
    m = pk_sign(pk_sub(h, ve1)); h = pk_max(h, ve1); src = m & 0x00010001u;
    m = pk_sign(pk_sub(h, vf1)); h = pk_max(h, vf1); src = pk_sel(m, 0x00020002u, src);
    if (!ONEP) {
        m = pk_sign(pk_sub(h, ve2)); h = pk_max(h, ve2); src = pk_sel(m, 0x00030003u, src);
        m = pk_sign(pk_sub(h, vf2)); h = pk_max(h, vf2); src = pk_sel(m, 0x00040004u, src);
    }
    return t | src;
}

__device__ __forceinline__ uint32_t d_cell_pk_cx(const PkConst &c, uint32_t hd, uint32_t hl, uint32_t el, uint32_t xel, uint32_t hu, uint32_t fu, uint32_t xfu,
                                                 uint32_t qb, uint32_t tbv, uint32_t &h, uint32_t &ve, uint32_t &vf, uint32_t &nxe, uint32_t &nxf)
{
    uint32_t op, g, m, t;
    op = pk_sub(hl, c.cx_oe0); g = pk_sub(el, xel); ve = pk_max(op, g); m = pk_sign(pk_sub(op, g)); t  = m & 0x00080008u;
    nxe = pk_sel(m, pk_max(pk_sub(xel, c.cx_dec), c.cx_emin), c.cx_e1);
    op = pk_sub(hu, c.cx_oe0); g = pk_sub(fu, xfu); vf = pk_max(op, g); m = pk_sign(pk_sub(op, g)); t |= m & 0x00100010u;
    nxf = pk_sel(m, pk_max(pk_sub(xfu, c.cx_dec), c.cx_emin), c.cx_e1);
    const uint32_t eq = pk_sign(pk_sub(qb ^ tbv, 0x00010001u));
    const uint32_t sc = pk_sub(eq & c.ab, c.b);
    t |= eq & 0x00800080u;
    h = pk_add(hd, sc);
    uint32_t src;
    m = pk_sign(pk_sub(h, ve)); h = pk_max(h, ve); src = m & 0x00010001u;
    m = pk_sign(pk_sub(h, vf)); h = pk_max(h, vf); src = pk_sel(m, 0x00020002u, src);
    return t | src;
}

template <int SH>
__device__ __forceinline__ uint32_t d_cell_pk4(const PkConst &c, uint32_t hd, uint32_t hl, uint32_t e1l, uint32_t hu, uint32_t f1u,
                                               uint32_t qb, uint32_t tbv, uint32_t &h, uint32_t &ve1, uint32_t &vf1)
{
    const uint32_t et = pk_max(pk_sub(hl, c.qe), pk_sub(e1l, c.e));
    const uint32_t ft = pk_max(pk_sub(hu, c.qeF), pk_sub(f1u, c.e));
    asm("v_and_or_b32 %0, %1, %2, %3" : "=v"(ve1) : "v"(et), "v"(0xFFFCFFFCu), "v"(0x00010001u));
    vf1 = ft & 0xFFFCFFFCu;
    uint32_t ne, hda = pk_add(hd, c.a), ht;
    asm("v_pk_min_u16 %0, %1, %2" : "=v"(ne) : "v"(qb ^ tbv), "v"(0x00010001u));
    asm("v_pk_mad_i16 %0, %1, %2, %3" : "=v"(ht) : "v"(ne), "v"(c.nab), "v"(hda));
    ht = pk_max(pk_max(ht, ve1), vf1);
    h = ht & 0xFFFCFFFCu;
    uint32_t n = ht & 0x00030003u;
    asm("v_lshl_or_b32 %0, %1, %2, %3" : "=v"(n) : "v"(et & 0x00010001u), "v"(2), "v"(n));
    asm("v_lshl_or_b32 %0, %1, %2, %3" : "=v"(n) : "v"(ft & 0x00010001u), "v"(3), "v"(n));
    return SH ? n << SH : n;
}

__device__ __forceinline__ uint32_t d_cell_pk8(const PkConst &c, uint32_t hd, uint32_t hl, uint32_t e1l, uint32_t e2l, uint32_t hu, uint32_t f1u, uint32_t f2u,
                                               uint32_t qb, uint32_t tbv, uint32_t &h, uint32_t &ve1, uint32_t &vf1, uint32_t &ve2, uint32_t &vf2)
{
    const uint32_t et1 = pk_max(pk_sub(hl, c.qe), pk_sub(e1l, c.e));
    const uint32_t ft1 = pk_max(pk_sub(hu, c.qeF), pk_sub(f1u, c.e));
    const uint32_t et2 = pk_max(pk_sub(hl, c.q2e2), pk_sub(e2l, c.e2));
    const uint32_t ft2 = pk_max(pk_sub(hu, c.q2e2F), pk_sub(f2u, c.e2));
    asm("v_and_or_b32 %0, %1, %2, %3" : "=v"(ve1) : "v"(et1), "v"(0xFFF8FFF8u), "v"(0x00030003u));
    asm("v_and_or_b32 %0, %1, %2, %3" : "=v"(vf1) : "v"(ft1), "v"(0xFFF8FFF8u), "v"(0x00020002u));
    asm("v_and_or_b32 %0, %1, %2, %3" : "=v"(ve2) : "v"(et2), "v"(0xFFF8FFF8u), "v"(0x00010001u));
    vf2 = ft2 & 0xFFF8FFF8u;
    uint32_t ne, hda = pk_add(hd, c.a), ht;
    asm("v_pk_min_u16 %0, %1, %2" : "=v"(ne) : "v"(qb ^ tbv), "v"(0x00010001u));
    asm("v_pk_mad_i16 %0, %1, %2, %3" : "=v"(ht) : "v"(ne), "v"(c.nab), "v"(hda));
    ht = pk_max(pk_max(ht, ve1), pk_max(vf1, pk_max(ve2, vf2)));
    h = ht & 0xFFF8FFF8u;
    uint32_t n = ht & 0x00070007u;
    asm("v_lshl_or_b32 %0, %1, %2, %3" : "=v"(n) : "v"(et1 & 0x00010001u), "v"(3), "v"(n));
    asm("v_lshl_or_b32 %0, %1, %2, %3" : "=v"(n) : "v"(ft1 & 0x00010001u), "v"(4), "v"(n));
    asm("v_lshl_or_b32 %0, %1, %2, %3" : "=v"(n) : "v"(et2 & 0x00010001u), "v"(5), "v"(n));
    asm("v_lshl_or_b32 %0, %1, %2, %3" : "=v"(n) : "v"(ft2 & 0x00010001u), "v"(6), "v"(n));
    return n;
}

template <int R> __device__ __forceinline__ void d_push_q(uint32_t (&qb)[R], uint32_t v)
{
#pragma unroll
    for (int r = R - 1; r >= 1; --r) qb[r] = __builtin_amdgcn_alignbit(qb[r], qb[r - 1], 16);
    qb[0] = (qb[0] << 16) | v;
}
template <int R> __device__ __forceinline__ void d_push_t(uint32_t (&tb)[R], uint32_t v)
{
#pragma unroll
    for (int r = 0; r < R - 1; ++r) tb[r] = __builtin_amdgcn_alignbit(tb[r + 1], tb[r], 16);
    tb[R - 1] = (tb[R - 1] >> 16) | (v << 16);
}

template <int LPP, int R> __device__ __forceinline__ int d_pk_rowmax(const uint32_t (&hv)[R])
{
    uint32_t M = hv[0];
#pragma unroll
    for (int r = 1; r < R; ++r) M = pk_max(M, hv[r]);
    int lo = (int)(short)(M & 0xffffu), hi = (int)M >> 16, cur = lo > hi ? lo : hi;
#pragma unroll
    for (int s = 1; s < LPP; s <<= 1) { const int v = __shfl_xor(cur, s); cur = v > cur ? v : cur; }
    return cur;
}
template <int LPP, int R> __device__ __forceinline__ int d_pk_argd(const uint32_t (&hv)[R], int cur, int de0, int par)
{
    int d = 0x7fffffff;
#pragma unroll
    for (int r = R - 1; r >= 0; --r) {
        const int lo = (int)(short)(hv[r] & 0xffffu), hi = (int)hv[r] >> 16;
        if (hi == cur) d = de0 + 4 * r + 2 + par;
        if (lo == cur) d = de0 + 4 * r + par;
    }
#pragma unroll
    for (int s = 1; s < LPP; s <<= 1) { const int v = __shfl_xor(d, s); d = v < d ? v : d; }
    return d;
}
__device__ __forceinline__ int d_step_cells(int a, int m, int n, int dlo, int dhi)
{
    int lo = dlo > a - 2 * m ? dlo : a - 2 * m; if (2 - a > lo) lo = 2 - a;
    int hi = dhi < 2 * n - a ? dhi : 2 * n - a; if (a - 2 < hi) hi = a - 2;
    if ((lo - a) & 1) ++lo;
    return hi >= lo ? ((hi - lo) >> 1) + 1 : 0;
}

template <int LPP, int R, bool EXT, int NW = 1, int FULL = 0, bool ONEP = false, bool TB4 = false, bool TAG8 = false, bool CX = false>
__device__ __forceinline__ void d_dp_pkr(const DpArgs &A, const int32_t *__restrict__ list, int nlist, int first_prob, uint32_t *xch = nullptr)
{
    static_assert(NW == 1 || LPP == 64 * NW, "multi-wave problems use whole waves");
    static_assert(!TB4 || (ONEP && LPP == 1 && !EXT), "nibble spill: one-piece cell, one problem per lane");
    static_assert(!TAG8 || (!ONEP && !TB4 && !EXT && NW == 1), "tagged two-piece cell: fills of the one-launch classes");
    static_assert(!CX || (!ONEP && !TB4 && !TAG8), "convex cell: plain flags, byte spill");
    constexpr int RW = LPP * R;
    const int lane = threadIdx.x, sub = lane / LPP, l = lane % LPP;
    const int wv = NW > 1 ? lane >> 6 : 0, wl = lane & 63;
    const int pi = first_prob + sub;
    const bool have = pi < nlist;
    const int prob = list[have ? pi : 0];
    const DpProb P = A.probs[prob];
    const DpOpt o = A.o;
    PkConst c; c.qe = pk_dup(o.q + o.e); c.e = pk_dup(o.e); c.q2e2 = pk_dup(o.q2 + o.e2); c.e2 = pk_dup(o.e2);
    c.ab = pk_dup(o.a + o.b); c.b = pk_dup(o.b); c.a = pk_dup(o.a); c.nab = pk_dup(-(o.a + o.b)); c.qeF = c.qe;
    c.q2e2F = c.q2e2;
    c.cx_oe0 = pk_dup(o.cx_open + d_cx_ext(o, 0)); c.cx_e1 = pk_dup(d_cx_ext(o, 1)); c.cx_emin = pk_dup(o.cx_emin); c.cx_dec = pk_dup(o.cx_dec);
    const uint32_t XN = CX ? c.cx_emin : PK_NEG;
    if constexpr (TB4) {
        c.qe = pk_dup(4 * (o.q + o.e) - 2); c.qeF = pk_dup(4 * (o.q + o.e) - 1); c.e = pk_dup(4 * o.e);
        c.a = pk_dup(4 * o.a + 2); c.nab = pk_dup(-4 * (o.a + o.b));
    }
    if constexpr (TAG8) {
        c.qe = pk_dup(8 * (o.q + o.e) - 4); c.qeF = pk_dup(8 * (o.q + o.e) - 3); c.e = pk_dup(8 * o.e);
        c.q2e2 = pk_dup(8 * (o.q2 + o.e2) - 2); c.q2e2F = pk_dup(8 * (o.q2 + o.e2) - 1); c.e2 = pk_dup(8 * o.e2);
        c.a = pk_dup(8 * o.a + 4); c.nab = pk_dup(-8 * (o.a + o.b));
    }
    const int m = have ? P.m : 0, n = have ? P.n : 0, dlo = P.dlo;
    const int de0 = dlo + 4 * R * l;
    const int dhi = have ? P.dhi : dlo - 1;
    uint32_t He[R], E1e[R], E2e[R], F1e[R], F2e[R], Ho[R], E1o[R], E2o[R], F1o[R], F2o[R], inE[R], inO[R], qb[R], tbv[R];
#pragma unroll
    for (int r = 0; r < R; ++r) {
        He[r] = E1e[r] = F1e[r] = Ho[r] = E1o[r] = F1o[r] = PK_NEG; E2e[r] = F2e[r] = E2o[r] = F2o[r] = XN;
        if constexpr (TB4) { E1e[r] |= 0x00010001u; E1o[r] |= 0x00010001u; }
        if constexpr (TAG8) { E1e[r] |= 0x00030003u; E1o[r] |= 0x00030003u; F1e[r] |= 0x00020002u; F1o[r] |= 0x00020002u; E2e[r] |= 0x00010001u; E2o[r] |= 0x00010001u; }
        const int d0 = de0 + 4 * r;
        if (d0 == 0) He[r] &= 0xffff0000u;
        if (d0 + 2 == 0) He[r] &= 0x0000ffffu;
        inE[r] = (d0 <= dhi ? 0x0000ffffu : 0u) | (d0 + 2 <= dhi ? 0xffff0000u : 0u);
        inO[r] = (d0 + 1 <= dhi ? 0x0000ffffu : 0u) | (d0 + 3 <= dhi ? 0xffff0000u : 0u);
        qb[r] = 0; tbv[r] = 0;
    }
    const int mn = m + n;
    int amax = mn, amin = have ? mn : 0x7fffffff;
    if (NW == 1) {
#pragma unroll
        for (int s = 32; s >= 1; s >>= 1) { int v = __shfl_xor(amax, s); amax = v > amax ? v : amax; v = __shfl_xor(amin, s); amin = v < amin ? v : amin; }
    }
    amin = __builtin_amdgcn_readfirstlane(amin);
    uint32_t *tb32 = (uint32_t*)(A.tb + P.tb_off) + (EXT ? ((l * R) >> 2) * 16 + ((l * R) & 3) : l * R);
    const int last_row = have ? mn >> 1 : -1;
    const int qs_ = P.qstep, ts_ = P.tstep;
    BaseStream QS, TS;
    d_stream_fill_acgt(QS, A.qseq2, P.qi0, qs_, -(de0 >> 1) - 2 * R, P.qcomp, A.qtot);
    d_stream_fill_acgt(TS, A.tseq2, P.ti0, ts_, (de0 >> 1) - 1, 0, A.ttot);
#pragma unroll
    for (int z = 0; z < 2 * R; ++z) {
        uint32_t qv = (uint32_t)d_stream_next_acgt(QS), tv = (uint32_t)d_stream_next_acgt(TS);
        if (EXT) { if (-(de0 >> 1) - 2 * R + z >= m) qv |= 8u; if ((de0 >> 1) - 1 + z >= n) tv |= 8u; }
        d_push_q<R>(qb, qv); d_push_t<R>(tbv, tv);
    }
    int qleft = 32 - 2 * R, tleft = 32 - 2 * R;
    int best = 0, bi = 0, bj = 0, prev_cur = -16384, done = have ? 0 : 1, ncell = 0;
    const int zdrop = o.zdrop;
    constexpr bool REB = CX;
    int off = 0, fin_off = 0;
    const bool first = l == 0, last = l == LPP - 1;
    const int xf = (n - m) - de0;
    const bool fin_here = have && xf >= 0 && xf < 4 * R;
    const int fin_r = xf >> 2, fin_hi = (xf >> 1) & 1;
    uint32_t fin = PK_NEG, te[R], prow[R];
#pragma unroll
    for (int r = 0; r < R; ++r) { te[r] = 0; prow[r] = 0; }
    if (NW > 1) {
        if (wl == 0) { uint32_t *x = xch + (0 * NW + wv) * 3; x[0] = He[0]; x[1] = F1e[0]; x[2] = F2e[0]; }
        __syncthreads();
    }
    for (int k = 0; 2 * k <= amax; ++k) {
        uint32_t h, ve1, vf1, ve2, vf2;
        if (k > 0) {
            const int a = 2 * k;
            if (qleft == 0) { d_stream_fill_acgt(QS, A.qseq2, P.qi0, qs_, ((a - de0) >> 1) - 1, P.qcomp, A.qtot); qleft = 32; }
            { uint32_t qv = (uint32_t)d_stream_next_acgt(QS); if (EXT && ((a - de0) >> 1) - 1 >= m) qv |= 8u; d_push_q<R>(qb, qv); } --qleft;
            uint32_t ph = PK_NEG, pe1 = PK_NEG, pe2 = XN;
            if (LPP > 1) {
                ph = DPP_SHR1((int)PK_NEG, (int)Ho[R - 1]); pe1 = DPP_SHR1((int)PK_NEG, (int)E1o[R - 1]); pe2 = DPP_SHR1((int)XN, (int)E2o[R - 1]);
                if (NW > 1 && wl == 0 && wv > 0) { const uint32_t *x = xch + (1 * NW + wv - 1) * 3; ph = x[0]; pe1 = x[1]; pe2 = x[2]; }
                if (first) { ph = PK_NEG; pe1 = PK_NEG; pe2 = XN; }
            }
#pragma unroll
            for (int r = 0; r < R; ++r) {
                const uint32_t lh = r ? Ho[r - 1] : ph, le1 = r ? E1o[r - 1] : pe1, le2 = r ? E2o[r - 1] : pe2;
                const uint32_t hl = __builtin_amdgcn_alignbit(Ho[r], lh, 16), e1l = __builtin_amdgcn_alignbit(E1o[r], le1, 16), e2l = __builtin_amdgcn_alignbit(E2o[r], le2, 16);
                if constexpr (TB4) { te[r] = d_cell_pk4<0>(c, He[r], hl, e1l, Ho[r], F1o[r], qb[r], tbv[r], h, ve1, vf1); ve2 = PK_NEG; vf2 = PK_NEG; }
                else if constexpr (TAG8) te[r] = d_cell_pk8(c, He[r], hl, e1l, e2l, Ho[r], F1o[r], F2o[r], qb[r], tbv[r], h, ve1, vf1, ve2, vf2);
                else if constexpr (CX) te[r] = d_cell_pk_cx(c, He[r], hl, e1l, e2l, Ho[r], F1o[r], F2o[r], qb[r], tbv[r], h, ve1, vf1, ve2, vf2);
                else te[r] = d_cell_pk<ONEP>(c, He[r], hl, e1l, e2l, Ho[r], F1o[r], F2o[r], qb[r], tbv[r], h, ve1, vf1, ve2, vf2);
                if (r < FULL) { He[r] = h; F1e[r] = vf1; F2e[r] = vf2; }
                else { He[r] = (h & inE[r]) | (PK_NEG & ~inE[r]); F1e[r] = (vf1 & inE[r]) | (PK_NEG & ~inE[r]); F2e[r] = (vf2 & inE[r]) | (XN & ~inE[r]); }
                E1e[r] = ve1; E2e[r] = ve2;
            }
            if (!EXT && a >= amin) {
#pragma unroll
                for (int r = 0; r < R; ++r) if (a == mn && r == fin_r) { fin = He[r]; fin_off = off; }
            }
            if (NW > 1) {
                if (wl == 0) { uint32_t *x = xch + (0 * NW + wv) * 3; x[0] = He[0]; x[1] = F1e[0]; x[2] = F2e[0]; }
                __syncthreads();
            }
            if (EXT) {
                uint32_t hv[R];
#pragma unroll
                for (int r = 0; r < R; ++r) hv[r] = pk_sel(pk_sign(PKU(PKS(qb[r] | tbv[r]) << (pk_s2)(12))), PK_NEG, He[r]);
                const int cur_rel = d_pk_rowmax<LPP, R>(hv), cur = cur_rel + off;
                if (!done) {
                    if (cur > best) { const int cd = d_pk_argd<LPP, R>(hv, cur_rel, de0, 0); best = cur; bi = (a - cd) >> 1; bj = (a + cd) >> 1; }
                    ncell += d_step_cells(a, m, n, dlo, dhi);
                    if (best - (cur > prev_cur ? cur : prev_cur) > zdrop || a >= mn) done = 1;
                }
                prev_cur = cur;
            }
        }
        {
            const int a = 2 * k + 1;
            if (tleft == 0) { d_stream_fill_acgt(TS, A.tseq2, P.ti0, ts_, ((a + de0 + 1) >> 1) + 2 * R - 2, 0, A.ttot); tleft = 32; }
            { uint32_t tv = (uint32_t)d_stream_next_acgt(TS); if (EXT && ((a + de0 + 1) >> 1) + 2 * R - 2 >= n) tv |= 8u; d_push_t<R>(tbv, tv); } --tleft;
            uint32_t nh = PK_NEG, nf1 = PK_NEG, nf2 = XN;
            if (LPP > 1) {
                nh = DPP_SHL1((int)PK_NEG, (int)He[0]); nf1 = DPP_SHL1((int)PK_NEG, (int)F1e[0]); nf2 = DPP_SHL1((int)XN, (int)F2e[0]);
                if (NW > 1 && wl == 63 && wv < NW - 1) { const uint32_t *x = xch + (0 * NW + wv + 1) * 3; nh = x[0]; nf1 = x[1]; nf2 = x[2]; }
                if (last) { nh = PK_NEG; nf1 = PK_NEG; nf2 = XN; }
            }
            uint32_t row[R];
#pragma unroll
            for (int r = 0; r < R; ++r) {
                const uint32_t uh = r < R - 1 ? He[r + 1] : nh, uf1 = r < R - 1 ? F1e[r + 1] : nf1, uf2 = r < R - 1 ? F2e[r + 1] : nf2;
                const uint32_t hu = __builtin_amdgcn_alignbit(uh, He[r], 16), f1u = __builtin_amdgcn_alignbit(uf1, F1e[r], 16), f2u = __builtin_amdgcn_alignbit(uf2, F2e[r], 16);
                uint32_t t;
                if constexpr (TB4) { t = d_cell_pk4<4>(c, Ho[r], He[r], E1e[r], hu, f1u, qb[r], tbv[r], h, ve1, vf1); ve2 = PK_NEG; vf2 = PK_NEG; }
                else if constexpr (TAG8) t = d_cell_pk8(c, Ho[r], He[r], E1e[r], E2e[r], hu, f1u, f2u, qb[r], tbv[r], h, ve1, vf1, ve2, vf2);
                else if constexpr (CX) t = d_cell_pk_cx(c, Ho[r], He[r], E1e[r], E2e[r], hu, f1u, f2u, qb[r], tbv[r], h, ve1, vf1, ve2, vf2);
                else t = d_cell_pk<ONEP>(c, Ho[r], He[r], E1e[r], E2e[r], hu, f1u, f2u, qb[r], tbv[r], h, ve1, vf1, ve2, vf2);
                if (r < FULL) { Ho[r] = h; F1o[r] = vf1; F2o[r] = vf2; }
                else { Ho[r] = (h & inO[r]) | (PK_NEG & ~inO[r]); F1o[r] = (vf1 & inO[r]) | (PK_NEG & ~inO[r]); F2o[r] = (vf2 & inO[r]) | (XN & ~inO[r]); }
                E1o[r] = ve1; E2o[r] = ve2;
                row[r] = TB4 ? (te[r] | t) : __builtin_amdgcn_perm(t, te[r], 0x06040200u);
            }
            if (!EXT && a >= amin) {
#pragma unroll
                for (int r = 0; r < R; ++r) if (a == mn && r == fin_r) { fin = Ho[r]; fin_off = off; }
            }
            if (EXT) {
                uint32_t hv[R];
#pragma unroll
                for (int r = 0; r < R; ++r) hv[r] = pk_sel(pk_sign(PKU(PKS(qb[r] | tbv[r]) << (pk_s2)(12))), PK_NEG, Ho[r]);
                const int cur_rel = d_pk_rowmax<LPP, R>(hv), cur = cur_rel + off;
                if (!done) {
                    if (cur > best) { const int cd = d_pk_argd<LPP, R>(hv, cur_rel, de0, 1); best = cur; bi = (a - cd) >> 1; bj = (a + cd) >> 1; }
                    ncell += d_step_cells(a, m, n, dlo, dhi);
                    if (best - (cur > prev_cur ? cur : prev_cur) > zdrop || a >= mn) done = 1;
                }
                prev_cur = cur;
            }
            if constexpr (TB4) {
                constexpr int RW4 = (R + 1) / 2;
                uint32_t rq[RW4];
#pragma unroll
                for (int j = 0; j < RW4; ++j) rq[j] = __builtin_amdgcn_perm(2 * j + 1 < R ? row[2 * j + 1] : 0u, row[2 * j], 0x06040200u);
                uint32_t sq[2 * RW4 + 1];
                if (k & 1) {
#pragma unroll
                    for (int j = 0; j < RW4; ++j) { sq[j] = prow[j]; sq[RW4 + j] = rq[j]; }
                    sq[2 * RW4] = 0;
                    uint32_t *dst = tb32 + (int64_t)((k - 1) / 2 * RW4) * 128;
                    if (k <= last_row) {
#pragma unroll
                        for (int u = 0; u < RW4; ++u) TB_ST2(dst + u * 128, sq[2 * u], sq[2 * u + 1]);
                    } else if (k - 1 <= last_row) {
#pragma unroll
                        for (int u = 0; u < (RW4 + 1) / 2; ++u) TB_ST2(dst + u * 128, sq[2 * u], sq[2 * u + 1]);
                    }
                } else {
#pragma unroll
                    for (int j = 0; j < RW4; ++j) prow[j] = rq[j];
                    if (2 * (k + 1) > amax && k <= last_row) {
#pragma unroll
                        for (int j = 0; j < RW4; ++j) sq[j] = rq[j];
                        sq[RW4] = 0;
                        uint32_t *dst = tb32 + (int64_t)(k / 2 * RW4) * 128;
#pragma unroll
                        for (int u = 0; u < (RW4 + 1) / 2; ++u) TB_ST2(dst + u * 128, sq[2 * u], sq[2 * u + 1]);
                    }
                }
            } else if constexpr (LPP == 1 && !EXT) {
                uint32_t sq[2 * R + 1];
                if (k & 1) {
#pragma unroll
                    for (int r = 0; r < R; ++r) { sq[r] = prow[r]; sq[R + r] = row[r]; }
                    sq[2 * R] = 0;
                    uint32_t *dst = tb32 + (int64_t)((k - 1) / 2 * R) * 128;
                    if (k <= last_row) {
#pragma unroll
                        for (int u = 0; u < R; ++u) TB_ST2(dst + u * 128, sq[2 * u], sq[2 * u + 1]);
                    } else if (k - 1 <= last_row) {
#pragma unroll
                        for (int u = 0; u < (R + 1) / 2; ++u) TB_ST2(dst + u * 128, sq[2 * u], sq[2 * u + 1]);
                    }
                } else {
#pragma unroll
                    for (int r = 0; r < R; ++r) prow[r] = row[r];
                    if (2 * (k + 1) > amax && k <= last_row) {
#pragma unroll
                        for (int r = 0; r < R; ++r) sq[r] = row[r];
                        sq[R] = 0;
                        uint32_t *dst = tb32 + (int64_t)(k / 2 * R) * 128;
#pragma unroll
                        for (int u = 0; u < (R + 1) / 2; ++u) TB_ST2(dst + u * 128, sq[2 * u], sq[2 * u + 1]);
                    }
                }
            } else if constexpr (EXT) {
                static_assert(!EXT || R == 4 || R == 1, "tiled spill: a lane owns a whole 16-byte group (R = 4) or one dword of it (R = 1)");
                if (k <= last_row) {
                    uint32_t *dst = tb32 + (int64_t)(k >> 2) * (4 * RW) + (k & 3) * 4;
                    if constexpr (R == 4) *(uint4*)dst = make_uint4(row[0], row[1], row[2], row[3]);
                    else dst[0] = row[0];
                }
            } else if (k <= last_row) {
                uint32_t *dst = tb32 + (int64_t)k * RW;
                if constexpr (R % 4 == 0) {
#pragma unroll
                    for (int r = 0; r < R; r += 4) *(uint4*)(dst + r) = make_uint4(row[r], row[r + 1], row[r + 2], row[r + 3]);
                } else if constexpr (R % 2 == 0) {
#pragma unroll
                    for (int r = 0; r < R; r += 2) *(uint2*)(dst + r) = make_uint2(row[r], row[r + 1]);
                } else {
#pragma unroll
                    for (int r = 0; r < R; ++r) dst[r] = row[r];
                }
            }
        }
        if constexpr (REB) {
            if ((k & 31) == 31) {
                uint32_t hv[R];
#pragma unroll
                for (int r = 0; r < R; ++r) hv[r] = pk_max(He[r], Ho[r]);
                int mx = d_pk_rowmax<(LPP > 64 ? 64 : LPP), R>(hv);
                if (NW > 1) {
                    int32_t *xm = (int32_t*)(xch + 2 * NW * 3);
                    if (wl == 0) xm[wv] = mx;
                    __syncthreads();
#pragma unroll
                    for (int w_ = 0; w_ < NW; ++w_) mx = xm[w_] > mx ? xm[w_] : mx;
                }
                const int delta = mx < -8192 ? 0 : mx;
                const uint32_t dd = pk_dup(delta), thr = pk_dup(delta - 12000);
#define REB_ONE(x) { const uint32_t dead = pk_sign(pk_sub((x), thr)); (x) = pk_sel(dead, PK_NEG, pk_max(pk_sub((x), dd), PK_NEG)); }
#pragma unroll
                for (int r = 0; r < R; ++r) { REB_ONE(He[r]) REB_ONE(Ho[r]) REB_ONE(E1e[r]) REB_ONE(E1o[r]) REB_ONE(F1e[r]) REB_ONE(F1o[r]) }
#undef REB_ONE
                off += delta;
            }
        }
        if (NW > 1) {
            if (wl == 63) { uint32_t *x = xch + (1 * NW + wv) * 3; x[0] = Ho[R - 1]; x[1] = E1o[R - 1]; x[2] = E2o[R - 1]; }
            __syncthreads();
        }
        if (EXT && __all(done)) break;
    }
    if (EXT) {
        if (have && l == 0) {
            DpRes Rr; Rr.score = best; Rr.bi = bi; Rr.bj = bj; Rr.nops = 0; Rr.mlen = 0; Rr.cells = ncell; Rr.tbases = n; Rr.mcols = 0;
            A.res[prob] = Rr;
        }
        return;
    }
    if (fin_here) {
        int sc = (int)(short)(fin_hi ? (fin >> 16) : (fin & 0xffffu)) + fin_off;
        if constexpr (TB4) sc >>= 2;
        if constexpr (TAG8) sc >>= 3;
        DpRes Rr; Rr.score = sc; Rr.bi = m; Rr.bj = n; Rr.nops = 0; Rr.mlen = 0; Rr.cells = P.pad[1]; Rr.tbases = n; Rr.mcols = 0;
        A.res[prob] = Rr;
    }
}

#define PK_NC 9
static_assert(__builtin_popcount(CLSM_PK) == PK_NC, "PK_NC counts the DPF_PK rows of DP_CLASS");
__host__ __device__ __forceinline__ constexpr int PK_IDX(int cls) { return __builtin_popcount(CLSM_PK & ((1u << cls) - 1u)); }
__host__ __device__ __forceinline__ constexpr int PK_CLS(int c) { int cls = 0; for (int k = 0; k < DP_NCLS; ++k) if (d_cls_in(k, CLSM_PK) && PK_IDX(k) == c) cls = k; return cls; }
struct PkPlan { int32_t woff[PK_NC + 1]; };
__global__ void k_pk_waves(const DpProb *__restrict__ probs, const int32_t *__restrict__ cls_list, ClsOff off, PkPlan plan,
                           uint32_t *__restrict__ keys, uint32_t *__restrict__ vals)
{
    const int i = blockIdx.x * blockDim.x + threadIdx.x;
    if (i >= plan.woff[PK_NC]) return;
    int c = 0;
    while (i >= plan.woff[c + 1]) ++c;
    const int cls = PK_CLS(c), first = (i - plan.woff[c]) * (64 / DP_CLASS[cls].lpp);
    const DpProb P = probs[cls_list[off.off[cls] + first]];
    const uint32_t cost = (uint32_t)((P.m + P.n) * DP_CLASS[cls].regs);
    keys[i] = cost > 0xFFFFu ? 0xFFFFu : cost;
    vals[i] = (uint32_t)cls << 26 | (uint32_t)first;
}
enum PkCell : int { CELL_PLAIN, CELL_TAG8, CELL_CX, CELL_ONEP, CELL_NIBBLE };
__device__ __forceinline__ int d_pk_cell(int cls, const DpOpt &o, int tb4, int tag8_steps, const DpProb *__restrict__ probs, const int32_t *__restrict__ first)
{
    if (o.cx_scale) return CELL_CX;
    const int onep_d = d_onep_d(o.q, o.e, o.q2, o.e2);
    static_assert(DP_CLASS[CLS_PK16].nibble == 1 && DP_CLASS[CLS_PK20].nibble == 2, "the nibble classes and their tb4_mask bits");
    if ((cls == CLS_PK16 && onep_d >= DP_CLASS[CLS_PK16].maxd) || (cls == CLS_PK20 && onep_d >= DP_CLASS[CLS_PK20].maxd)) return d_tb4(cls, tb4) ? CELL_NIBBLE : CELL_ONEP;
    const DpProb P0 = probs[*first];
    return P0.m + P0.n <= tag8_steps ? CELL_TAG8 : CELL_PLAIN;
}
template <int CLS, bool EXACT, bool ONEP, bool TB4, bool TAG8, bool CX>
__device__ __forceinline__ void d_dp_pk_cls(const DpArgs &A, const int32_t *__restrict__ list, int n, int first)
{
    static_assert(DP_CLASS[CLS].family == DPF_PK && EXACT == (DP_CLASS[CLS].layout == TBL_INTERLEAVED && CLS != CLS_PK16), "class table");
    d_dp_pkr<DP_CLASS[CLS].lpp, DP_CLASS[CLS].regs, false, 1, EXACT ? DP_CLASS[CLS].regs - 1 : 0, ONEP, TB4, TAG8, CX>(A, list, n, first);
}
template <bool TAG8, bool CX>
__device__ __forceinline__ void d_dp_pk_any(int cls, const DpArgs &A, const int32_t *__restrict__ list, int n, int first)
{
    switch (cls) {
    case CLS_PK20: d_dp_pk_cls<CLS_PK20, true, false, false, TAG8, CX>(A, list, n, first); break;
    case CLS_PK24: d_dp_pk_cls<CLS_PK24, true, false, false, TAG8, CX>(A, list, n, first); break;
    case CLS_PK28: d_dp_pk_cls<CLS_PK28, true, false, false, TAG8, CX>(A, list, n, first); break;
    case CLS_PK32: d_dp_pk_cls<CLS_PK32, true, false, false, TAG8, CX>(A, list, n, first); break;
    case CLS_PK16: d_dp_pk_cls<CLS_PK16, false, false, false, TAG8, CX>(A, list, n, first); break;
    case CLS_PK40: d_dp_pk_cls<CLS_PK40, false, false, false, TAG8, CX>(A, list, n, first); break;
    case CLS_PK48: d_dp_pk_cls<CLS_PK48, false, false, false, TAG8, CX>(A, list, n, first); break;
    case CLS_PK128: d_dp_pk_cls<CLS_PK128, false, false, false, TAG8, CX>(A, list, n, first); break;
    default: d_dp_pk_cls<CLS_PK64, false, false, false, TAG8, CX>(A, list, n, first); break;
    }
}
#ifndef PK_WPE
#define PK_WPE 2
#endif
__global__ void __launch_bounds__(64) __attribute__((amdgpu_waves_per_eu(PK_WPE))) k_dp_pk(DpArgs A, const uint32_t *__restrict__ waves, const int32_t *__restrict__ cls_list,
                                              ClsOff off)
{
    const uint32_t w = waves[blockIdx.x];
    const int cls = (int)(w >> 26), first = (int)(w & 0x3ffffffu);
    const int32_t *list = cls_list + off.off[cls];
    const int n = off.off[cls + 1] - off.off[cls];
    const int cell = d_pk_cell(cls, A.o, A.tb4, A.tag8_steps, A.probs, list + first);
    if (cell == CELL_CX) { d_dp_pk_any<false, true>(cls, A, list, n, first); return; }
    if (cell >= CELL_ONEP && cls == CLS_PK16) { if (cell == CELL_NIBBLE) d_dp_pk_cls<CLS_PK16, false, true, true, false, false>(A, list, n, first); else d_dp_pk_cls<CLS_PK16, false, true, false, false, false>(A, list, n, first); return; }
    if (cell >= CELL_ONEP) { if (cell == CELL_NIBBLE) d_dp_pk_cls<CLS_PK20, true, true, true, false, false>(A, list, n, first); else d_dp_pk_cls<CLS_PK20, true, true, false, false, false>(A, list, n, first); return; }
    if (cell == CELL_TAG8) { d_dp_pk_any<true, false>(cls, A, list, n, first); return; }
    d_dp_pk_any<false, false>(cls, A, list, n, first);
}
template <int NW>
__global__ void __launch_bounds__(64 * NW) k_dp_pkw(DpArgs A)
{
    __shared__ uint32_t xch[2 * NW * 3 + NW];
    __builtin_amdgcn_s_setprio(3);
    if (A.o.cx_scale) d_dp_pkr<64 * NW, 1, false, NW, 0, false, false, false, true>(A, A.list, A.nlist, blockIdx.x, xch);
    else d_dp_pkr<64 * NW, 1, false, NW>(A, A.list, A.nlist, blockIdx.x, xch);
}
constexpr int PKX_LPP = DP_CLASS[CLS_PKX64].lpp, PKX_R = DP_CLASS[CLS_PKX64].regs;
__global__ void __launch_bounds__(64) k_dp_pkx(DpArgs A)
{
    __builtin_amdgcn_s_setprio(3);
    if (A.o.cx_scale) d_dp_pkr<PKX_LPP, PKX_R, true, 1, 0, false, false, false, true>(A, A.list, A.nlist, blockIdx.x * (64 / PKX_LPP));
    else d_dp_pkr<PKX_LPP, PKX_R, true>(A, A.list, A.nlist, blockIdx.x * (64 / PKX_LPP));
}
__global__ void __launch_bounds__(64) k_dp_pkx16(DpArgs A)
{
    __builtin_amdgcn_s_setprio(3);
    if (A.o.cx_scale) d_dp_pkr<16, 1, true, 1, 0, false, false, false, true>(A, A.list, A.nlist, blockIdx.x * 4);
    else d_dp_pkr<16, 1, true>(A, A.list, A.nlist, blockIdx.x * 4);
}

constexpr int PKX8_LPP = DP_CLASS[CLS_PKX128].lpp;
static_assert(DP_CLASS[CLS_PKX128].regs == 32 / PKX8_LPP && DP_CLASS[CLS_PKX256].lpp == 16 && DP_CLASS[CLS_PKX256].regs == 4, "class table");
__global__ void __launch_bounds__(64) k_dp_pkx_w8(DpArgs A)
{
    __builtin_amdgcn_s_setprio(3);
    if (A.o.cx_scale) d_dp_pkr<PKX8_LPP, 32 / PKX8_LPP, true, 1, 0, false, false, false, true>(A, A.list, A.nlist, blockIdx.x * (64 / PKX8_LPP));
    else d_dp_pkr<PKX8_LPP, 32 / PKX8_LPP, true>(A, A.list, A.nlist, blockIdx.x * (64 / PKX8_LPP));
}
__global__ void __launch_bounds__(64) k_dp_pkx_w16(DpArgs A)
{
    __builtin_amdgcn_s_setprio(3);
    if (A.o.cx_scale) d_dp_pkr<16, 4, true, 1, 0, false, false, false, true>(A, A.list, A.nlist, blockIdx.x * 4);
    else d_dp_pkr<16, 4, true>(A, A.list, A.nlist, blockIdx.x * 4);
}

#ifndef TB_SLOTS
#define TB_SLOTS 2
#endif
template <int LAYOUT>
__device__ __forceinline__ void d_traceback_lane(const DpProb *__restrict__ probs, DpRes *__restrict__ res, int pi,
                                                 const uint8_t *__restrict__ tb_all, uint32_t *__restrict__ cig, int32_t *__restrict__ retry,
                                                 uint32_t *stage)
{
    const int lane = threadIdx.x;
    const DpProb P = probs[pi];
    if (P.kind >= 3) return;
    const int dhi_ = P.dhi; int touched = 0;
    const int cls = P.pad[0] & 0xff, dlo = P.dlo, mg = P.pad[0] >> 8;
    const int D = P.dhi - dlo + 1, stride = (D + 2) / 2;
    const int lpp = d_cls_slots(cls);
    const bool packed = d_tb_regs(cls), tiled = d_tb_tiled(cls), rows2 = d_tb_rows2(cls);
    int i = res[pi].bi, j = res[pi].bj;
    uint32_t *cg = cig + P.cig_off;
    int no = 0, ml = 0, mc = 0, state = 0, cur_op = -1, cur_len = 0;
    const int rowb = tiled ? lpp * 16 : packed ? lpp * 4 : stride;
    int64_t tag0 = -1, tag1 = -1, pfb = -2;
    uint4 v0 = make_uint4(0, 0, 0, 0), v1 = v0, v2 = v0, v3 = v0, v4 = v0, v5 = v0, v6 = v0, v7 = v0;
    while (i > 0 && j > 0) {
        const int a = i + j, sl = (j - i - dlo) >> 1;
        const int64_t off = tiled ? ((((int64_t)(a >> 3) * (4 * lpp) + ((sl >> 3) << 4) + (((a >> 1) & 3) << 2) + ((sl >> 1) & 3)) << 2) + ((a & 1) << 1) + (sl & 1))
                          : (LAYOUT == 2 || rows2) ? ((((int64_t)(a >> 1) * lpp + (sl >> 1)) << 2) + ((a & 1) << 1) + (sl & 1))
                          : packed ? ((((int64_t)(a >> 2) * lpp + sl) << 2) + (a & 3)) : ((int64_t)a * stride + sl);
        const int64_t abs_off = P.tb_off + (d_tb_interleaved(cls) ? ((off >> 3) << 9) + (off & 7) : off), line = abs_off >> 6;
        const int slot = TB_SLOTS > 1 ? (int)(line & 1) : 0;
        if ((slot ? tag1 : tag0) != line) {
            const int64_t blk = line >> 1;
            if (pfb != blk) {
                const uint4 *src = (const uint4*)(tb_all + (blk << 7));
                v0 = src[0]; v1 = src[1]; v2 = src[2]; v3 = src[3]; v4 = src[4]; v5 = src[5]; v6 = src[6]; v7 = src[7];
            }
            uint32_t *dst = stage + slot * 1024 + lane;
            if (line & 1) {
                dst[0 * 64] = v4.x; dst[1 * 64] = v4.y; dst[2 * 64] = v4.z; dst[3 * 64] = v4.w;
                dst[4 * 64] = v5.x; dst[5 * 64] = v5.y; dst[6 * 64] = v5.z; dst[7 * 64] = v5.w;
                dst[8 * 64] = v6.x; dst[9 * 64] = v6.y; dst[10 * 64] = v6.z; dst[11 * 64] = v6.w;
                dst[12 * 64] = v7.x; dst[13 * 64] = v7.y; dst[14 * 64] = v7.z; dst[15 * 64] = v7.w;
            } else {
                dst[0 * 64] = v0.x; dst[1 * 64] = v0.y; dst[2 * 64] = v0.z; dst[3 * 64] = v0.w;
                dst[4 * 64] = v1.x; dst[5 * 64] = v1.y; dst[6 * 64] = v1.z; dst[7 * 64] = v1.w;
                dst[8 * 64] = v2.x; dst[9 * 64] = v2.y; dst[10 * 64] = v2.z; dst[11 * 64] = v2.w;
                dst[12 * 64] = v3.x; dst[13 * 64] = v3.y; dst[14 * 64] = v3.z; dst[15 * 64] = v3.w;
            }
            if (slot) tag1 = line; else tag0 = line;
            const int64_t nl = rowb >= 64 ? (abs_off - rowb) >> 6 : line - 1, nb = nl >> 1;
            pfb = blk;
            if (nb != blk && nl >= 0) {
                const uint4 *src = (const uint4*)(tb_all + (nb << 7));
                v0 = src[0]; v1 = src[1]; v2 = src[2]; v3 = src[3]; v4 = src[4]; v5 = src[5]; v6 = src[6]; v7 = src[7];
                pfb = nb;
            }
        }
        const int w = (int)(abs_off & 63);
        const uint8_t *st8 = (const uint8_t*)stage + ((slot * 1024 + lane) << 2);
        const uint32_t t = st8[(w >> 2) * 256 + (w & 3)];
        const int mij = i < j ? i : j, kr = tiled ? (a >> 1) & 3 : 0;
        const bool up1 = kr >= 1 && mij > 1, up2 = kr >= 2 && mij > 2, up3 = kr >= 3 && mij > 3;
        const uint32_t t1 = up1 ? st8[((w - 16) >> 2) * 256 + (w & 3)] : 0xffu, t2 = up2 ? st8[((w - 32) >> 2) * 256 + (w & 3)] : 0xffu, t3 = up3 ? st8[((w - 48) >> 2) * 256 + (w & 3)] : 0xffu;
        const uint32_t nd = (uint32_t)((t1 & 7u) != 0u) << 1 | (uint32_t)((t2 & 7u) != 0u) << 2 | (uint32_t)((t3 & 7u) != 0u) << 3;
        const uint32_t mb = (t >> 7) | ((t1 >> 7) & 1u) << 1 | ((t2 >> 7) & 1u) << 2 | ((t3 >> 7) & 1u) << 3;
        touched |= (j - i - dlo <= mg) | (dhi_ - (j - i) <= mg);
        const int s0 = state ? state : (int)(t & 7);
        const int isM = s0 == 0, isD = s0 & 1;
        const int op = isM ? 0 : (isD ? 2 : 1);
        const int nn = isM ? __builtin_ctz(nd | 16u) : 1;
        state = (isM || !((t >> (2 + s0)) & 1)) ? 0 : s0;
        ml += isM ? __builtin_popcount(mb & ((1u << nn) - 1u)) : 0; mc += isM ? nn : 0;
        i -= isM ? nn : (isD ^ 1); j -= isM ? nn : isD;
        const bool same = op == cur_op;
        if (!same && cur_len) cg[no++] = (uint32_t)cur_len << 4 | (uint32_t)cur_op;
        cur_len = same ? cur_len + nn : nn; cur_op = op;
    }
    if (i > 0) { if (cur_op == 1) cur_len += i; else { if (cur_len) cg[no++] = (uint32_t)cur_len << 4 | (uint32_t)cur_op; cur_op = 1; cur_len = i; } }
    if (j > 0) { if (cur_op == 2) cur_len += j; else { if (cur_len) cg[no++] = (uint32_t)cur_len << 4 | (uint32_t)cur_op; cur_op = 2; cur_len = j; } }
    if (cur_len) cg[no++] = (uint32_t)cur_len << 4 | (uint32_t)cur_op;
    res[pi].nops = no; res[pi].mlen = ml; res[pi].mcols = mc;
    if (retry && P.kind == 0 && touched && P.m + P.n <= ADAPT_MAX_STEPS) retry[pi] = 1;
}
__global__ void __launch_bounds__(64) k_traceback(const DpProb *__restrict__ probs, DpRes *__restrict__ res, int32_t np,
                                                  const uint8_t *__restrict__ tb_all, uint32_t *__restrict__ cig, int32_t *__restrict__ retry,
                                                  const int32_t *__restrict__ list)
{
    __shared__ uint32_t stage[TB_SLOTS * 16 * 64];
    const int ti = blockIdx.x * blockDim.x + threadIdx.x;
    if (ti >= np) return;
    d_traceback_lane<-1>(probs, res, list ? list[ti] : ti, tb_all, cig, retry, stage);
}
template <int ENC, bool IL>
__device__ __forceinline__ void d_traceback_rows(const DpProb *__restrict__ probs, DpRes *__restrict__ res, int pi, bool have, int lpp, int rb4_, const DpOpt o_,
                                                 const uint8_t *__restrict__ tb_all, uint32_t *__restrict__ cig, int32_t *__restrict__ retry,
                                                 uint32_t *stage)
{
    constexpr bool il = IL, tag8 = ENC == 1, nib = ENC == 2;
    const int rb4 = ENC == 2 ? rb4_ : 0;
    const int lane = threadIdx.x;
    DpProb P = probs[pi];
    if (P.kind >= 3) have = false;
    const int rowb = nib ? rb4 : lpp * 4, dlo = P.dlo, dhi_ = P.dhi, mg = P.pad[0] >> 8;
    int gc = 0;
    int i = 0, j = 0;
    if (have) { i = res[pi].bi; j = res[pi].bj; }
    const uint8_t *tb = tb_all + P.tb_off;
    uint32_t *cg = cig + P.cig_off;
    int no = 0, ml = 0, mc = 0, state = 0, cur_op = -1, cur_len = 0, touched = 0;
    const int mytop = have && i > 0 && j > 0 ? (i + j) >> 1 : -1;
    const int mytopline = mytop >= 0 ? (mytop * rowb + rowb - 1) >> 6 : -1;
    int rtop = mytop;
// ... 393 lines not shown
```

### telr_amd/csrc/telr_engine.hip

```cpp
#include <hip/hip_runtime.h>
#include <cstring>
#include <string.h>
#include <rocprim/rocprim.hpp>
#include <algorithm>
#include <atomic>
#include <immintrin.h>
#include <chrono>
#include <cmath>
#include <condition_variable>
#include <cstdio>
#include <cstdlib>
#include <cstring>
#include <map>
#include <memory>
#include <mutex>
#include <string>
#include <thread>
#include <sys/mman.h>
#include <vector>
#include "../../include/telr_hip.h"
#include "kernels.hip.h"
#include "range_plan.h"
#include "sam_records.h"
#define TELR_HAVE_SEED_ARGS 1
// ... 1127 lines not shown
}
extern "C" int64_t telr_result_cigar_count(const telr_result *r) { return r ? (int64_t)r->ncig : 0; }
extern "C" const uint32_t *telr_result_cigars(const telr_result *r) { result_wait(r); return r ? r->cig : nullptr; }
extern "C" void telr_result_free(telr_result *r) { delete r; }


static int host_threads()
{
    static int cached = 0;
    if (cached) return cached;
    int n = (int)std::thread::hardware_concurrency();
    if (FILE *f = fopen("/sys/fs/cgroup/cpu.max", "r")) {
        char q[64]; long period = 0;
        if (fscanf(f, "%63s %ld", q, &period) == 2 && strcmp(q, "max") != 0 && period > 0) {
            long quota = atol(q);
            int c = (int)((quota + period - 1) / period);
            if (c >= 1 && c < n) n = c;
        }
        fclose(f);
    }
    n = n + n / 2;
    if (const char *e = getenv("LOCAL_WORLD_SIZE")) { int v = atoi(e); if (v > 1) n = std::max(4, n / v); }
    if (const char *e = getenv("TELR_HOST_THREADS")) { int v = atoi(e); if (v > 0) n = v; }
    if (n < 1) n = 1;
    if (n > 48) n = 48;
    cached = n;
    return n;
}
static void unmap_in_pieces(void *p, size_t bytes)
{
    const size_t piece = (size_t)32 << 20;
    for (size_t o = 0; o < bytes; o += piece) { munmap((char*)p + o, std::min(piece, bytes - o)); std::this_thread::yield(); }
}
#include <condition_variable>
#include <functional>
#include <mutex>
#include <atomic>
class HostPool {
public:
    static HostPool &get() { static HostPool p; return p; }
    void run(int ntask, const std::function<void(int)> &f)
    {
        if (ntask <= 0) return;
        std::unique_lock<std::mutex> job(job_mu_);
        ensure(ntask - 1);
        {
            std::lock_guard<std::mutex> lk(mu_);
            fn_ = &f; ntask_ = ntask; next_.store(0); pending_ = ntask; ++gen_;
        }
        cv_.notify_all();
        work();
        std::unique_lock<std::mutex> lk(mu_);
        done_.wait(lk, [&] { return pending_ == 0 && active_ == 0; });
        fn_ = nullptr;
    }
private:
    HostPool() {}
    ~HostPool()
    {
        { std::lock_guard<std::mutex> lk(mu_); stop_ = true; ++gen_; }
        cv_.notify_all();
        for (auto &t : th_) t.join();
    }
    void ensure(int n) { while ((int)th_.size() < n && (int)th_.size() < 47) th_.emplace_back([this, g = gen_]() mutable { loop(g); }); }
    void work()
    {
        for (;;) {
            const int i = next_.fetch_add(1);
            if (i >= ntask_) break;
            (*fn_)(i);
            std::lock_guard<std::mutex> lk(mu_);
            if (--pending_ == 0) done_.notify_all();
        }
    }
    void loop(uint64_t seen)
    {
        for (;;) {
            {
                std::unique_lock<std::mutex> lk(mu_);
                cv_.wait(lk, [&] { return gen_ != seen; });
                seen = gen_;
                if (stop_) return;
                if (pending_ == 0) continue;
                ++active_;
            }
            work();
            std::lock_guard<std::mutex> lk(mu_);
            if (--active_ == 0 && pending_ == 0) done_.notify_all();
        }
    }
    std::mutex mu_, job_mu_;
    std::condition_variable cv_, done_;
    std::vector<std::thread> th_;
    const std::function<void(int)> *fn_ = nullptr;
    std::atomic<int> next_{0};
    int ntask_ = 0, pending_ = 0, active_ = 0;
    uint64_t gen_ = 0;
    bool stop_ = false;
};
template <typename F> static void parallel_ranges(int nt, int n, F f)
{
    if (n <= 0) return;
    if (nt > n) nt = n;
    if (nt <= 1 || n < 64) { f(0, 0, n); return; }
    HostPool::get().run(nt, [&](int t) {
        const int a = (int)((int64_t)n * t / nt), b = (int)((int64_t)n * (t + 1) / nt);
        f(t, a, b);
    });
}


static inline int cx_gap(const telr_map_opt *mo, int L)
{
    int t = mo->cx_open;
    for (int i = 0; i < L; ++i) { const int e = mo->cx_ext_max - mo->cx_decay * i; t += e > mo->cx_ext_min ? e : mo->cx_ext_min; }
    return t;
}
static inline bool pk_cx_ok(const telr_map_opt *mo, int D)
{
    const int S = mo->cx_scale, bS = mo->b * S, aS = mo->a * S;
    if (ab_on("no_pk") || bS > 400 || aS > 400 || mo->sc_ambi * S > 400 || mo->cx_open + mo->cx_ext_max > 320 || mo->cx_ext_max < mo->cx_ext_min || mo->cx_ext_min < 0 || mo->cx_decay < 0) return false;
    return cx_gap(mo, D) + aS * D / 2 <= 11900;
}
static inline int affine_steps(const telr_map_opt *mo, int hb, int D, int ha, int gap_open, int gap_ext)
{
    const int by_b = 2 * (hb - gap_open - D * gap_ext) / (mo->b > 0 ? mo->b : 1) - 2, by_a = ha / (mo->a > 0 ? mo->a : 1) - 2;
    const int lim = by_b < by_a ? by_b : by_a;
    return lim > 0 ? lim : 0;
}
static inline int pk_ext_d(const telr_map_opt *mo) { const int c = d_cls_fit<DPF_PKX>(2 * mo->ext_band + 2, DP_DMAX); return DP_CLASS[c < 0 ? (int)CLS_PKX256 : c].maxd; }
static DpLimits dp_limits(const telr_map_opt *mo)
{
    static const bool one_launch = ab_on("tb_one_launch"), tb8 = ab_on("tb8"), no_tag8 = ab_on("no_tag8");
    const bool cx = mo->cx_scale > 0;
    DpLimits L = { 0, 0, 0, 0, 64, 0, 0, 0 };
    if (cx) L.pk_steps = pk_cx_ok(mo, 128) ? 7900 : 0;
    else if (mo->b <= 9 && mo->a <= 4 && mo->q2 + mo->e2 <= 64 && mo->sc_ambi <= 9 && !ab_on("no_pk")) L.pk_steps = affine_steps(mo, 15800, 128, 32000, mo->q2, mo->e2);
    L.pk_wide_maxd = !cx || pk_cx_ok(mo, 1024) ? 1024 : pk_cx_ok(mo, 512) ? 512 : pk_cx_ok(mo, 256) ? 256 : 0;
    if (L.pk_steps && !ab_on("no_pkw")) L.pk_wide = cx ? (pk_cx_ok(mo, 256) ? 7900 : 0) : affine_steps(mo, 15800, 1024, 32000, mo->q2, mo->e2);
    if (L.pk_steps && !ab_on("no_pkext")) {
        const int D = pk_ext_d(mo);
        if (cx) L.pk_ext = mo->zdrop * mo->cx_scale <= 30000 && pk_cx_ok(mo, D) ? 7900 : 0;
        else if (mo->zdrop <= 4000) L.pk_ext = affine_steps(mo, 15800, D, 32000, mo->q2, mo->e2);
        if (L.pk_ext) L.pk_ext_maxd = D;
    }
    if (L.pk_steps && !cx && !one_launch && !tb8) {
        const int d = d_onep_d(mo->q, mo->e, mo->q2, mo->e2);
        for (const DpClassRow &r : DP_CLASS) if (r.nibble && d >= r.maxd) L.tb4_mask |= r.nibble;
    }
    L.tb4_steps = affine_steps(mo, 3850, 32, 7700, mo->q, mo->e);
    if (L.pk_steps && !cx && !one_launch && !no_tag8) L.tag8_steps = affine_steps(mo, 1975, 128, 4000, mo->q2, mo->e2);
    return L;
}
typedef void (*DpKernel)(DpArgs);
template <int CLS> static constexpr DpKernel reg_kernel() { return k_dp_reg<DP_CLASS[CLS].lpp, DP_CLASS[CLS].regs, (DP_CLASS[CLS].lpp + 63) / 64>; }
template <int CLS> static constexpr DpKernel pkw_kernel() { return k_dp_pkw<DP_CLASS[CLS].lpp / 64>; }
struct SideLaunch { int cls; DpKernel kernel; bool lane_walk; };
static const SideLaunch SIDE_LAUNCH[] = {
    { CLS_REG1024, reg_kernel<CLS_REG1024>(), false },
    { CLS_LDSMAX, k_dp_w4, false },
    { CLS_LDS1024, k_dp_w4, false },
    { CLS_PKW1024, pkw_kernel<CLS_PKW1024>(), false },
    { CLS_REG512, reg_kernel<CLS_REG512>(), false },
    { CLS_PKW512, pkw_kernel<CLS_PKW512>(), false },
    { CLS_PKX256, k_dp_pkx_w16, true },
    { CLS_PKX128, k_dp_pkx_w8, true },
    { CLS_PKX64, k_dp_pkx, true },
    { CLS_LDS256, k_dp, false },
    { CLS_REG256, reg_kernel<CLS_REG256>(), false },
    { CLS_PKW256, pkw_kernel<CLS_PKW256>(), false },
    { CLS_LDS128, k_dp, false },
    { CLS_LDS64, k_dp, true },
};
static int dp_pass(telr_ctx *ctx, const telr_seqset *qs, const telr_seqset *tg, const telr_map_opt *mo, DpProb *d_probs, int np, DpRes *d_res,
                   uint32_t **d_rawcig_io, int32_t *d_retry, const std::string &sfx, bool primary)
{
    hipStream_t st = ctx->stream;
    const DpLimits L = dp_limits(mo);
    int64_t *d_tbb, *d_cgo, *d_tboff, *d_cgoff; int32_t *d_clscnt, *d_clslist; uint32_t *d_clskey, *d_keytmp; int32_t *d_listtmp;
    ClsOff coff;
    TRY(ctx_buf_t(ctx, ("tb_bytes" + sfx).c_str(), (size_t)np + 1, &d_tbb));
    TRY(ctx_buf_t(ctx, ("cig_ops" + sfx).c_str(), (size_t)np + 1, &d_cgo));
    TRY(ctx_buf_t(ctx, ("tb_off" + sfx).c_str(), (size_t)np + 1, &d_tboff));
    TRY(ctx_buf_t(ctx, ("cig_off" + sfx).c_str(), (size_t)np + 1, &d_cgoff));
    TRY(ctx_buf_t(ctx, ("cls_cnt" + sfx).c_str(), 32, &d_clscnt));
    TRY(ctx_buf_t(ctx, ("cls_list" + sfx).c_str(), (size_t)np, &d_clslist));
    TRY(ctx_buf_t(ctx, ("cls_key" + sfx).c_str(), (size_t)np, &d_clskey));
    TRY(ctx_buf_t(ctx, ("cls_keytmp" + sfx).c_str(), (size_t)np, &d_keytmp));
    TRY(ctx_buf_t(ctx, ("cls_listtmp" + sfx).c_str(), (size_t)np, &d_listtmp));
    hipLaunchKernelGGL(k_prob_sizes, dim3((np + 255) / 256), dim3(256), 0, st, d_probs, np, primary ? mo->fill_margin : 0, L, qs->d_nmask, tg->d_nmask, d_tbb, d_cgo);
    HIPCHK(hipGetLastError());
    HIPCHK(hipMemsetAsync(d_tbb + np, 0, 8, st));
    HIPCHK(hipMemsetAsync(d_cgo + np, 0, 8, st));
    TRY((dev_exclusive_scan<int64_t, int64_t>(ctx, d_tbb, d_tboff, (size_t)np + 1)));
    if (primary) TRY((dev_exclusive_scan<int64_t, int64_t>(ctx, d_cgo, d_cgoff, (size_t)np + 1)));
    HIPCHK(hipMemsetAsync(d_clscnt, 0, 128, st));
    hipLaunchKernelGGL(k_prob_assign, dim3((np + 255) / 256), dim3(256), 0, st, d_probs, np, d_tboff, primary ? d_cgoff : (const int64_t*)nullptr, d_clscnt, d_clskey, d_listtmp);
    HIPCHK(hipGetLastError());
    int64_t tb_total = 0, cg_total = 0; int32_t h_cls[32];
    static_assert(DP_NCLS <= 32 && DP_NCLS == TELR_N_DPCLS, "class table");
    HIPCHK(hipMemcpyAsync(&tb_total, d_tboff + np, 8, hipMemcpyDeviceToHost, st));
    if (primary) HIPCHK(hipMemcpyAsync(&cg_total, d_cgoff + np, 8, hipMemcpyDeviceToHost, st));
    HIPCHK(hipMemcpyAsync(h_cls, d_clscnt, 128, hipMemcpyDeviceToHost, st));
    HIPCHK(hipStreamSynchronize(st));
    coff.off[0] = 0;
    for (int c = 0; c < DP_NCLS; ++c) coff.off[c + 1] = coff.off[c] + h_cls[c];
    {
        size_t tbytes = 0;
        HIPCHK(rocprim::radix_sort_pairs(nullptr, tbytes, d_clskey, d_keytmp, d_listtmp, d_clslist, (size_t)np, 0, 24, st));
        void *tmp; TRY(ctx_buf(ctx, "rp_tmp", tbytes, &tmp));
        HIPCHK(rocprim::radix_sort_pairs(tmp, tbytes, d_clskey, d_keytmp, d_listtmp, d_clslist, (size_t)np, 0, 24, st));
    }
    if (np > 0) {
        int64_t *d_tbs;
        TRY(ctx_buf_t(ctx, ("tb_sorted" + sfx).c_str(), (size_t)np + 1, &d_tbs));
        hipLaunchKernelGGL(k_tb_gather, dim3(np / 256 + 1), dim3(256), 0, st, d_tbb, d_clslist, np, coff, d_tbs);
        TRY((dev_exclusive_scan<int64_t, int64_t>(ctx, d_tbs, d_tboff, (size_t)np + 1)));
        hipLaunchKernelGGL(k_tb_scatter, dim3(np / 256 + 1), dim3(256), 0, st, d_probs, d_clslist, np, coff, d_tboff);
        HIPCHK(hipGetLastError());
        HIPCHK(hipMemcpyAsync(&tb_total, d_tboff + np, 8, hipMemcpyDeviceToHost, st));
        HIPCHK(hipStreamSynchronize(st));
    }
    uint8_t *d_tb;
    TRY(ctx_buf_t(ctx, ("tb" + sfx).c_str(), (size_t)tb_total + 256, &d_tb));
    if (primary) TRY(ctx_buf_t(ctx, "rawcig", (size_t)cg_total + 16, d_rawcig_io));
    DpArgs D; D.qseq2 = qs->d_seq2; D.qnmask = qs->d_nmask; D.tseq2 = tg->d_seq2; D.tnmask = tg->d_nmask; D.probs = d_probs;
    D.qtot = qs->padded_bases; D.ttot = tg->padded_bases;
    D.o.a = mo->a; D.o.b = mo->b; D.o.q = mo->q; D.o.e = mo->e; D.o.q2 = mo->q2; D.o.e2 = mo->e2; D.o.sc_ambi = mo->sc_ambi; D.o.zdrop = mo->zdrop;
    D.o.cx_scale = D.o.cx_open = D.o.cx_emax = D.o.cx_emin = D.o.cx_dec = D.o.cx_flat = 0;
    if (mo->cx_scale > 0) {
        const int S = mo->cx_scale;
        D.o.a *= S; D.o.b *= S; D.o.sc_ambi *= S; D.o.zdrop *= S;
        D.o.cx_scale = S; D.o.cx_open = mo->cx_open; D.o.cx_emax = mo->cx_ext_max; D.o.cx_emin = mo->cx_ext_min; D.o.cx_dec = mo->cx_decay;
        D.o.cx_flat = mo->cx_decay > 0 && mo->cx_ext_max > mo->cx_ext_min ? (mo->cx_ext_max - mo->cx_ext_min + mo->cx_decay - 1) / mo->cx_decay : 0;
    }
    D.tb = d_tb; D.cig = *d_rawcig_io; D.res = d_res; D.dcap = 0;
    D.retry = d_retry; D.tb4 = L.tb4_mask; D.tag8_steps = L.tag8_steps;
    static const bool tb_split = !ab_on("tb_one_launch");
    int nw = 0; uint32_t *d_wv2 = nullptr;
    {
        PkPlan plan; plan.woff[0] = 0;
        for (int c = 0; c < PK_NC; ++c) { const int ppw = 64 / DP_CLASS[PK_CLS(c)].lpp; plan.woff[c + 1] = plan.woff[c] + (h_cls[PK_CLS(c)] + ppw - 1) / ppw; }
        nw = plan.woff[PK_NC];
        if (nw > 0) {
            uint32_t *d_wk, *d_wv, *d_wk2;
            TRY(ctx_buf_t(ctx, ("pk_wkey" + sfx).c_str(), (size_t)nw, &d_wk));
            TRY(ctx_buf_t(ctx, ("pk_wval" + sfx).c_str(), (size_t)nw, &d_wv));
            TRY(ctx_buf_t(ctx, ("pk_wkey2" + sfx).c_str(), (size_t)nw, &d_wk2));
            TRY(ctx_buf_t(ctx, ("pk_wval2" + sfx).c_str(), (size_t)nw, &d_wv2));
            hipLaunchKernelGGL(k_pk_waves, dim3((nw + 255) / 256), dim3(256), 0, st, d_probs, d_clslist, coff, plan, d_wk, d_wv);
            HIPCHK(hipGetLastError());
            size_t tbytes = 0;
            HIPCHK(rocprim::radix_sort_pairs_desc(nullptr, tbytes, d_wk, d_wk2, d_wv, d_wv2, (size_t)nw, 0, 16, st));
            void *tmp; TRY(ctx_buf(ctx, "rp_tmp", tbytes, &tmp));
            HIPCHK(rocprim::radix_sort_pairs_desc(tmp, tbytes, d_wk, d_wk2, d_wv, d_wv2, (size_t)nw, 0, 16, st));
        }
    }
    HIPCHK(hipEventRecord(ctx->ev_fork, st));
    int side = 0;
    std::vector<hipStream_t> used;
    static const bool serial = getenv("TELR_SERIAL") != nullptr;
    auto side_stream = [&]() { if (serial) return st; hipStream_t s2 = ctx->side[side % TELR_NSIDE]; ++side; used.push_back(s2); return s2; };
    auto launch = [&](int c, DpKernel kernel, hipStream_t s2) -> int {
        const int nl = h_cls[c];
        int threads = DP_CLASS[c].lpp > 64 ? DP_CLASS[c].lpp : 64, ppb = DP_CLASS[c].lpp < 64 ? 64 / DP_CLASS[c].lpp : 1;
        size_t lds = 0;
        D.list = d_clslist + coff.off[c]; D.nlist = nl; D.dcap = 0;
        if (DP_CLASS[c].family == DPF_LDS) {
            D.dcap = DP_CLASS[c].maxd;
            lds = (size_t)(D.dcap + 2) * 5 * 4;
            static const bool one_wave = ab_on("dp_one_wave");
            if (one_wave) { kernel = k_dp; threads = 64; }
            if (lds > 48 * 1024) HIPCHK(hipFuncSetAttribute((const void*)kernel, hipFuncAttributeMaxDynamicSharedMemorySize, (int)lds));
        }
        if (c == CLS_PKX64 && nl < 8192) { kernel = k_dp_pkx16; ppb = 4; }
        hipLaunchKernelGGL(kernel, dim3((nl + ppb - 1) / ppb), dim3(threads), lds, s2, D);
        HIPCHK(hipGetLastError());
        return TELR_OK;
    };
    for (const SideLaunch &row : SIDE_LAUNCH) {
        const int c = row.cls, nl = h_cls[c];
        if (nl == 0) continue;
        hipStream_t s2 = side_stream();
        HIPCHK(hipStreamWaitEvent(s2, ctx->ev_fork, 0));
        TRY(launch(c, row.kernel, s2));
        if (tb_split) {
            const int tbw_max = 2048;
            if (row.lane_walk || nl > tbw_max) hipLaunchKernelGGL(k_traceback, dim3((nl + 63) / 64), dim3(64), 0, s2, d_probs, d_res, nl, d_tb, *d_rawcig_io, d_retry, D.list);
            else hipLaunchKernelGGL(k_traceback_w, dim3(nl), dim3(64), 0, s2, d_probs, d_res, nl, d_tb, *d_rawcig_io, d_retry, D.list);
            HIPCHK(hipGetLastError());
        }
    }
    D.dcap = 0;
    const bool tb_over = tb_split && !serial && nw > 0;
    if (primary) HIPCHK(hipEventRecord(ctx->evk[5], st));
    if (primary && nw > 0) ++ctx->pk_launches;
    if (nw > 0) {
        D.list = nullptr; D.nlist = 0;
        if (tb_over) { HIPCHK(hipStreamWaitEvent(ctx->tb_stream, ctx->ev_fork, 0)); if (primary) HIPCHK(hipEventRecord(ctx->evk[3], ctx->tb_stream)); }
        hipLaunchKernelGGL(k_dp_pk, dim3(nw), dim3(64), 0, st, D, d_wv2, d_clslist, coff);
        HIPCHK(hipGetLastError());
        if (tb_over) {
            HIPCHK(hipEventRecord(ctx->ev_pk, st));
            HIPCHK(hipStreamWaitEvent(ctx->tb_stream, ctx->ev_pk, 0));
            hipLaunchKernelGGL(k_traceback_pk, dim3(nw), dim3(64), 0, ctx->tb_stream, d_probs, d_res, d_tb, *d_rawcig_io, d_retry, d_wv2, d_clslist, coff, L.tb4_mask, D.o, L.tag8_steps);
            HIPCHK(hipGetLastError());
            if (primary) HIPCHK(hipEventRecord(ctx->evk[4], ctx->tb_stream));
            used.push_back(ctx->tb_stream);
        }
    }
    if (primary) HIPCHK(hipEventRecord(ctx->evk[0], st));
    if (h_cls[CLS_REG64]) TRY(launch(CLS_REG64, reg_kernel<CLS_REG64>(), st));
    if (h_cls[CLS_REG128]) TRY(launch(CLS_REG128, reg_kernel<CLS_REG128>(), st));
    if (primary) HIPCHK(hipEventRecord(ctx->evk[1], st));
    if (tb_split) {
        if (!tb_over && primary) HIPCHK(hipEventRecord(ctx->evk[3], st));
        if (!tb_over && nw > 0) hipLaunchKernelGGL(k_traceback_pk, dim3(nw), dim3(64), 0, st, d_probs, d_res, d_tb, *d_rawcig_io, d_retry, d_wv2, d_clslist, coff, L.tb4_mask, D.o, L.tag8_steps);
        for (int c : { (int)CLS_REG128, (int)CLS_REG64 }) {
            if (h_cls[c] == 0) continue;
            hipLaunchKernelGGL(k_traceback, dim3((h_cls[c] + 63) / 64), dim3(64), 0, st, d_probs, d_res, h_cls[c], d_tb, *d_rawcig_io, d_retry, (const int32_t*)(d_clslist + coff.off[c]));
        }
        if (!tb_over && primary) HIPCHK(hipEventRecord(ctx->evk[4], st));
        HIPCHK(hipGetLastError());
    }
    for (size_t u = 0; u < used.size(); ++u) {
        HIPCHK(hipEventRecord(ctx->ev_side[u % TELR_NSIDE], used[u]));
        HIPCHK(hipStreamWaitEvent(st, ctx->ev_side[u % TELR_NSIDE], 0));
    }
#ifdef TB_PROF
    if (nw > 0) {
        HIPCHK(hipDeviceSynchronize());
        unsigned long long h[8]; HIPCHK(hipMemcpyFromSymbol(h, HIP_SYMBOL(g_tb_prof), sizeof(h)));
        unsigned long long z[8] = {0, 0, 0, 0, ~0ULL, 0, 0, 0}; HIPCHK(hipMemcpyToSymbol(HIP_SYMBOL(g_tb_prof), z, sizeof(z)));
        if (h[2]) fprintf(stderr, "[tb prof] k_traceback_pk: %llu waves, span %.3f ms, longest wave %.3f ms (%llu lines), mean wave %.3f ms, %.1f lines per wave, wave-ms / span = %.1f waves on the device on average\n",
                          h[2], (double)(h[5] - h[4]) / 1e5, (double)(h[1] >> 16) / 1e5, h[1] & 0xffffULL, (double)h[0] / (double)h[2] / 1e5, (double)h[3] / (double)h[2], (double)h[0] / (double)(h[5] - h[4] ? h[5] - h[4] : 1));
    }
#endif
    if (!tb_split) {
        if (primary) HIPCHK(hipEventRecord(ctx->evk[3], st));
        hipLaunchKernelGGL(k_traceback, dim3((np + 63) / 64), dim3(64), 0, st, d_probs, d_res, np, d_tb, *d_rawcig_io, d_retry, (const int32_t*)nullptr);
        if (primary) HIPCHK(hipEventRecord(ctx->evk[4], st));
    }
    HIPCHK(hipGetLastError());
    return TELR_OK;
}

struct HostTrace {
    bool on; const char *tag; std::chrono::steady_clock::time_point t0, last;
    HostTrace(const char *t) : tag(t) { static const bool e = trace_on("host"); on = e; t0 = last = std::chrono::steady_clock::now(); }
    void mark(const char *what) {
        if (!on) return;
        auto now = std::chrono::steady_clock::now();
        fprintf(stderr, "[host %s] %-28s +%7.3f ms  (%8.3f)\n", tag, what, std::chrono::duration<double, std::milli>(now - last).count(), std::chrono::duration<double, std::milli>(now - t0).count());
        last = now;
    }
};

struct OccCut { int32_t mid_occ; const int32_t *d_tmid; };
static int chain_dispatch(telr_ctx *ctx, hipStream_t st, const telr_map_opt *mo, const uint64_t *d_skeys, const int32_t *d_qaoff, int nq, int32_t na,
                          int32_t n_over, const int32_t *d_overlist, const int32_t *d_qorder, int32_t *d_f, int32_t *d_p)
{
    ChainOpt co; co.max_gap = mo->max_gap; co.bw = mo->bw_long > mo->bw ? mo->bw_long : mo->bw; co.min_cnt = mo->min_cnt; co.min_chain_score = mo->min_chain_score;
    co.chain_gap_q8 = mo->chain_gap_q8; co.chain_skip_q8 = mo->chain_skip_q8;
    static const bool chain_push = ab_on("chain_push"), chain_lazy = ab_on("chain_lazy"), chain_no_mw = ab_on("chain_no_mw");
    static int dense_v[3] = {2048, 48, 1 << 19};
    static const bool dense_env = [] { if (const char *e = getenv("TELR_CHAIN_DENSE")) sscanf(e, "%d%*[,:]%d%*[,:]%d", &dense_v[0], &dense_v[1], &dense_v[2]); return true; }();
    (void)dense_env;
    const int Rr = mo->chain_lookback / 64;
    const bool mw_all = dense_v[2] <= SEGSORT_CAP;
    static const bool no_islands = ab_on("no_islands");
    static const bool chain_no_pack = ab_on("chain_no_pack");
    const bool islands = nq <= CHAIN_ISL_NQ && na > 0 && !no_islands;
    const bool mw = !(mo->flags & TELR_MF_CHAIN_SKIP) && !chain_push && !chain_lazy && !chain_no_mw && Rr >= 2 && na > 0 && !islands && dense_v[2] > 0 && (mw_all || n_over > 0);
    co.dense_n = dense_v[0]; co.dense_span = dense_v[1]; co.mw_n = mw ? dense_v[2] : 0;
#define CHAIN_LAUNCH(RR, SK) do { if (chain_push) hipLaunchKernelGGL((k_chain<RR, SK, 0>), dim3(nq), dim3(64), 0, st, d_skeys, d_qaoff, nq, co, d_f, d_p, d_qorder, 0, 0); \
                                  else if (chain_lazy) hipLaunchKernelGGL((k_chain<RR, SK, 1>), dim3(nq), dim3(64), 0, st, d_skeys, d_qaoff, nq, co, d_f, d_p, d_qorder, 0, 0); \
                                  else hipLaunchKernelGGL((k_chain<RR, SK, 2>), dim3(nq), dim3(64), 0, st, d_skeys, d_qaoff, nq, co, d_f, d_p, d_qorder, mw ? 1 : 0, chain_no_pack ? 0 : 1); } while (0)
#define CHAIN_MW(RR, SK) hipLaunchKernelGGL((k_chain_mw<RR, SK>), dim3(mw_all ? nq : n_over), dim3(64 * RR), 0, ctx->side[0], d_skeys, d_qaoff, mw_all ? nq : n_over, mw_all ? (const int32_t*)nullptr : (const int32_t*)d_overlist, co, d_f, d_p)
    const bool skip = co.chain_skip_q8 != 0;
    if (mo->flags & TELR_MF_CHAIN_SKIP) {
        int32_t *d_mark;
        TRY(ctx_buf_t(ctx, "chain_mark", (size_t)na + 1, &d_mark));
        if (islands) {
            int32_t *d_head, *d_rank, *d_ioff, *d_ipd;
            TRY(ctx_buf_t(ctx, "isl_head", (size_t)na + 1, &d_head));
            TRY(ctx_buf_t(ctx, "isl_rank", (size_t)na + 1, &d_rank));
            TRY(ctx_buf_t(ctx, "isl_off", (size_t)na + 2, &d_ioff));
            TRY(ctx_buf_t(ctx, "isl_pd", (size_t)na + 1, &d_ipd));
            HIPCHK(hipMemsetAsync(d_head + na, 0, 4, st));
            hipLaunchKernelGGL(k_isl_heads, dim3(nq), dim3(256), 0, st, d_skeys, d_qaoff, nq, (uint32_t)co.max_gap, d_head);
// ... 777 lines not shown
        mem_note(ctx, "telr_map: two ranges in flight ran out");
        telr_destroy(ctx->slot1); ctx->slot1 = nullptr;
        (void)hipDeviceSynchronize();
        for (auto &kv : ctx->bufs) if (kv.first.compare(0, 4, "bam_") == 0 && kv.second.p) { (void)hipFree(kv.second.p); kv.second.p = nullptr; kv.second.bytes = 0; }
        result_rollback(C.R);
        mem_note(ctx, "telr_map: after giving back slot 2 + writer");
        call_reset(ctx);
        const int32_t *len = C.queries->len.data(); const int32_t nq = C.queries->n;
        const int64_t lim = std::min<int64_t>(P.batch_bases, 1024LL << 20);
        for (int32_t q0 = 0; q0 < nq; ) {
            const int32_t q1 = range_cut(len, nq, q0, lim);
            TRY(run_range(ctx, C, q0, q1));
            q0 = q1;
        }
    } else if (prc != TELR_OK) return prc;
    else call_merge(ctx, S[1]);
    density_update(ctx, C.ix);
    return TELR_OK;
}

extern "C" int telr_map(telr_ctx *ctx, const telr_index *ix, const telr_seqset *queries, const int32_t *qtarget, const telr_map_opt *mo, telr_result **out)
{
    (void)hipGetLastError();
    if (!ctx || !ix || !queries || !mo || !out) return TELR_E_ARG;
    TRY(check_map_opt(ctx, mo));
    if (queries->max_len >= (1 << 24)) return TELR_E_RANGE;
    HIPCHK(hipSetDevice(ctx->device));
    call_reset(ctx);
    const int nq = queries->n;
    if (qtarget) for (int i = 0; i < nq; ++i) if (qtarget[i] >= ix->targets->n) return TELR_E_ARG;
    int32_t *d_qt = nullptr;
    if (qtarget && nq > 0) {
        TRY(ctx_buf_t(ctx, "qtarget", (size_t)nq, &d_qt));
        HIPCHK(hipMemcpyAsync(d_qt, qtarget, (size_t)nq * 4, hipMemcpyHostToDevice, ctx->stream)); HIPCHK(hipStreamSynchronize(ctx->stream));
    }
    OccCut mid_occ; mid_occ.mid_occ = index_mid_occ(ix, mo); mid_occ.d_tmid = nullptr;
    if (qtarget || (mo->flags & TELR_MF_PER_TARGET)) TRY(index_per_target_occ(ctx, ix, mo, &mid_occ.d_tmid));
    telr_result *R = new telr_result();
    R->ctx = ctx;
    if (!ctx->aln_pool.empty()) {
        size_t best = 0;
        for (size_t i = 1; i < ctx->aln_pool.size(); ++i) if (ctx->aln_pool[i].capacity() > ctx->aln_pool[best].capacity()) best = i;
        R->alns = std::move(ctx->aln_pool[best]); R->alns.clear();
        ctx->aln_pool.erase(ctx->aln_pool.begin() + best);
    }
    const auto t_wall0 = std::chrono::steady_clock::now();
    int64_t env_bases = 0; double per_base = 0;
    if (!range_size_from_env(&env_bases)) per_base = ix->anchors_per_base > 0 ? ix->anchors_per_base : call_density_bound(ix, mid_occ.mid_occ, mo);
    const bool vote = mo->vote_len > 0 && !qtarget && !(mo->flags & TELR_MF_PER_TARGET);
    const RangePlan P = plan_ranges(queries->len.data(), nq, queries->max_len, per_base, qtarget != nullptr, vote, ctx->debug, ctx->pipe_nomem);
    ctx->twin_owner = ctx; ctx->twin_bases = P.total_bases;
    { static const bool tr = trace_on("host");
      if (tr) fprintf(stderr, "[host plan] %d queries, %.1f Mbp, %zu range(s) of <= %.1f Mbp, %s, anchors per base seen %.3f%s\n", nq, P.total_bases / 1048576.0, P.ranges.size(), P.batch_bases / 1048576.0,
                      P.mode == RANGE_TWO ? "two in flight" : "one at a time", ix->anchors_per_base, qtarget ? ", per-query targets" : ""); }
    const MapCall C = { ix, queries, qtarget, d_qt, mo, mid_occ, R };
    const int r = P.mode == RANGE_IN_TURN ? run_in_turn(ctx, C, P) : P.mode == RANGE_TWO ? run_two_slots(ctx, C, P) : run_serial(ctx, C, P, per_base);
    if (r != TELR_OK) { delete R; return r; }
    ctx->stage_ms[ST_MAP_WALL] = std::chrono::duration<float, std::milli>(std::chrono::steady_clock::now() - t_wall0).count();
    *out = R;
    return TELR_OK;
}

extern "C" int telr_debug_map_plan(const int32_t *len, int32_t n, int32_t max_len, double per_base, int has_qtarget, int vote, int debug, int pipe_nomem,
                                   int64_t *out, int32_t *range_end)
{
    if (n < 0 || (n > 0 && !len) || !out) return TELR_E_ARG;
    const RangePlan P = plan_ranges(len, n, max_len, per_base, has_qtarget != 0, vote != 0, debug, pipe_nomem != 0);
    out[0] = P.mode; out[1] = P.batch_bases; out[2] = (int64_t)P.ranges.size();
    if (range_end) for (size_t i = 0; i < P.ranges.size(); ++i) range_end[i] = P.ranges[i].second;
    return TELR_OK;
}

extern "C" int telr_window_reads(const telr_aln *recs, int64_t n_rec, int32_t n_win, const int32_t *win_tid, const int32_t *win_lo, const int32_t *win_hi,
                                 int64_t *out_off, int32_t *out_qid, int64_t cap, int64_t *needed)
{
    if (n_rec < 0 || n_win < 0 || (n_rec > 0 && !recs) || (n_win > 0 && (!win_tid || !win_lo || !win_hi)) || !out_off || !needed || cap < 0 || (cap > 0 && !out_qid)) return TELR_E_ARG;
    if (n_rec >= (1LL << 31)) return TELR_E_RANGE;
    std::vector<int32_t> ord(n_win);
    for (int i = 0; i < n_win; ++i) ord[i] = i;
    std::sort(ord.begin(), ord.end(), [&](int32_t a, int32_t b) { const int32_t la = win_lo[a] > 0 ? win_lo[a] : 0, lb = win_lo[b] > 0 ? win_lo[b] : 0;
        return win_tid[a] != win_tid[b] ? win_tid[a] < win_tid[b] : la != lb ? la < lb : a < b; });
    std::vector<int64_t> key(n_win); std::vector<int32_t> hmax(n_win), hi(n_win);
    for (int j = 0; j < n_win; ++j) {
        const int w = ord[j];
        key[j] = (int64_t)win_tid[w] << 32 | (uint32_t)(win_lo[w] > 0 ? win_lo[w] : 0); hi[j] = win_hi[w];
        hmax[j] = (j > 0 && win_tid[ord[j - 1]] == win_tid[w] && hmax[j - 1] > hi[j]) ? hmax[j - 1] : hi[j];
    }
    const int NT = host_threads();
    std::vector<std::vector<uint64_t>> part(NT);
    parallel_ranges(NT, (int)n_rec, [&](int t, int a, int b) {
        std::vector<uint64_t> &P = part[t];
        for (int x = a; x < b; ++x) {
            const telr_aln &r = recs[x];
            if (r.tid < 0) continue;
            const int64_t k = (int64_t)r.tid << 32 | (uint32_t)r.te;
            int j1 = (int)(std::lower_bound(key.begin(), key.end(), k) - key.begin());
            for (int j = j1 - 1; j >= 0 && (key[j] >> 32) == r.tid && hmax[j] > r.ts; --j)
                if (hi[j] > r.ts) P.push_back((uint64_t)j << 32 | (uint32_t)r.qid);
        }
    });
    std::vector<int64_t> cnt((size_t)n_win + 1, 0);
    for (int t = 0; t < NT; ++t) for (uint64_t v : part[t]) ++cnt[(size_t)(v >> 32) + 1];
    for (int j = 0; j < n_win; ++j) cnt[j + 1] += cnt[j];
    std::vector<int32_t> all((size_t)cnt[n_win]);
    { std::vector<int64_t> fill(cnt.begin(), cnt.end() - 1);
      for (int t = 0; t < NT; ++t) for (uint64_t v : part[t]) all[(size_t)fill[v >> 32]++] = (int32_t)(uint32_t)v; }
    std::vector<int64_t> uniq(n_win, 0);
    parallel_ranges(NT, n_win, [&](int, int a, int b) {
        for (int j = a; j < b; ++j) {
            int32_t *f = all.data() + cnt[j], *l = all.data() + cnt[j + 1];
            std::sort(f, l);
            uniq[j] = std::unique(f, l) - f;
        }
    });
    std::vector<int64_t> len_of(n_win, 0), src_of(n_win, 0);
    for (int j = 0; j < n_win; ++j) { len_of[ord[j]] = uniq[j]; src_of[ord[j]] = cnt[j]; }
    out_off[0] = 0;
    for (int w = 0; w < n_win; ++w) out_off[w + 1] = out_off[w] + len_of[w];
    *needed = out_off[n_win];
    if (*needed > cap) return TELR_E_RANGE;
    for (int w = 0; w < n_win; ++w) if (len_of[w]) memcpy(out_qid + out_off[w], all.data() + src_of[w], (size_t)len_of[w] * 4);
    return TELR_OK;
}

extern "C" int64_t telr_debug_dp_retries(const telr_ctx *ctx) { return ctx ? ctx->dp_retries : 0; }
extern "C" int64_t telr_debug_pk_launches(const telr_ctx *ctx) { return ctx ? ctx->pk_launches : 0; }
extern "C" int64_t telr_debug_n_anchor(const telr_ctx *ctx) { return ctx ? ctx->dbg_na : 0; }
extern "C" int telr_debug_fetch(telr_ctx *ctx, const char *what, void *dst, int64_t bytes)
{
    if (!ctx || !what || !dst) return TELR_E_ARG;
    auto it = ctx->bufs.find(what);
    if (it == ctx->bufs.end() || !it->second.p || (size_t)bytes > it->second.bytes) return TELR_E_ARG;
    HIPCHK(hipMemcpy(dst, it->second.p, (size_t)bytes, hipMemcpyDeviceToHost));
    return TELR_OK;
}
extern "C" int64_t telr_debug_n_chain(const telr_ctx *ctx) { return ctx ? (int64_t)ctx->dbg_chain.size() / 9 : 0; }
extern "C" const int32_t *telr_debug_chains(const telr_ctx *ctx) { return ctx ? ctx->dbg_chain.data() : nullptr; }
extern "C" int telr_debug_index(telr_ctx *ctx, const telr_index *ix, uint64_t *ent_hash, uint32_t *ent_off, uint32_t *pos)
{
    if (!ctx || !ix) return TELR_E_ARG;
    if (ent_hash) HIPCHK(hipMemcpy(ent_hash, ix->d_ent_hash, (size_t)ix->n_ent * 8, hipMemcpyDeviceToHost));
    if (ent_off) HIPCHK(hipMemcpy(ent_off, ix->d_ent_off, ((size_t)ix->n_ent + 1) * 4, hipMemcpyDeviceToHost));
    if (pos) HIPCHK(hipMemcpy(pos, ix->d_pos, (size_t)ix->n_mz * 4, hipMemcpyDeviceToHost));
    return TELR_OK;
}
extern "C" int32_t telr_debug_mid_occ(const telr_index *ix, const telr_map_opt *mo) { return ix && mo ? index_mid_occ(ix, mo) : -1; }
extern "C" int telr_debug_dp_limits(const telr_map_opt *mo, int32_t *out)
{
    if (!mo || !out) return TELR_E_ARG;
    const DpLimits L = dp_limits(mo);
    out[0] = L.pk_steps; out[1] = L.pk_wide; out[2] = L.pk_wide_maxd; out[3] = L.pk_ext;
    out[4] = L.pk_ext_maxd; out[5] = L.tb4_mask; out[6] = L.tb4_steps; out[7] = L.tag8_steps;
    return TELR_OK;
}
extern "C" int telr_debug_dp_class_table(int32_t *out)
{
    if (!out) return TELR_E_ARG;
    for (int c = 0; c < DP_NCLS; ++c) {
        const DpClassRow &r = DP_CLASS[c];
        int32_t *o = out + c * 6;
        o[0] = r.maxd; o[1] = r.lpp; o[2] = r.regs; o[3] = r.slots; o[4] = d_tb_interleaved(c); o[5] = d_tb_tiled(c);
    }
    return TELR_OK;
}
extern "C" int telr_debug_chain(telr_ctx *ctx, int32_t nq, const uint64_t *keys, const int32_t *q_aoff, const telr_map_opt *mo, int32_t *f, int32_t *p)
{
    (void)hipGetLastError();
    if (!ctx || !mo || nq < 0 || nq > (1 << 24) || (nq > 0 && !q_aoff)) return TELR_E_ARG;
    TRY(check_map_opt(ctx, mo));
    if (nq == 0) return TELR_OK;
    if (q_aoff[0] != 0) { ctx->err = "telr_debug_chain: q_aoff[0] must be 0"; return TELR_E_ARG; }
    int32_t n_over = 0;
    std::vector<int32_t> over;
    for (int q = 0; q < nq; ++q) {
        const int32_t a0 = q_aoff[q], a1 = q_aoff[q + 1];
        if (a1 < a0 || a1 > (1 << 30)) { ctx->err = "telr_debug_chain: q_aoff must ascend (at most 2^30 anchors)"; return TELR_E_ARG; }
        for (int32_t i = a0 + 1; i < a1; ++i)
            if (keys[i] < keys[i - 1]) { ctx->err = "telr_debug_chain: the anchors of query " + std::to_string(q) + " are not sorted"; return TELR_E_ARG; }
        if (a1 - a0 > SEGSORT_CAP) { over.push_back(q); ++n_over; }
    }
    const int32_t na = q_aoff[nq];
    if (na > 0 && (!keys || !f || !p)) return TELR_E_ARG;
    if (na == 0) return TELR_OK;
    HIPCHK(hipSetDevice(ctx->device));
    hipStream_t st = ctx->stream;
    uint64_t *d_keys; int32_t *d_qaoff, *d_over, *d_f, *d_p;
    TRY(ctx_buf_t(ctx, "dbg_ch_keys", (size_t)na, &d_keys));
    TRY(ctx_buf_t(ctx, "dbg_ch_qaoff", (size_t)nq + 1, &d_qaoff));
    TRY(ctx_buf_t(ctx, "dbg_ch_over", (size_t)n_over + 1, &d_over));
    TRY(ctx_buf_t(ctx, "dbg_ch_f", (size_t)na, &d_f));
    TRY(ctx_buf_t(ctx, "dbg_ch_p", (size_t)na, &d_p));
    HIPCHK(hipMemcpyAsync(d_keys, keys, (size_t)na * 8, hipMemcpyHostToDevice, st));
    HIPCHK(hipMemcpyAsync(d_qaoff, q_aoff, ((size_t)nq + 1) * 4, hipMemcpyHostToDevice, st));
    if (n_over) HIPCHK(hipMemcpyAsync(d_over, over.data(), (size_t)n_over * 4, hipMemcpyHostToDevice, st));
    TRY(chain_dispatch(ctx, st, mo, d_keys, d_qaoff, nq, na, n_over, d_over, nullptr, d_f, d_p));
    HIPCHK(hipMemcpyAsync(f, d_f, (size_t)na * 4, hipMemcpyDeviceToHost, st));
    HIPCHK(hipMemcpyAsync(p, d_p, (size_t)na * 4, hipMemcpyDeviceToHost, st));
    HIPCHK(hipStreamSynchronize(st));
    return TELR_OK;
}
extern "C" int telr_debug_backtrack(telr_ctx *ctx, int32_t nq, const int32_t *q_aoff, const uint64_t *keys, const int32_t *f, const int32_t *p, const int32_t *qlen,
                                    int32_t n_targets, const uint32_t *goff, const int32_t *tlen, const telr_map_opt *mo,
                                    int32_t *ch_off, int32_t *chains, int32_t *ch_aoff, uint64_t *canch, int32_t *kept, int32_t *prob_off, int32_t *probs,
                                    int64_t prob_cap, int64_t *n_out)
{
    (void)hipGetLastError();
    if (!ctx || !mo || !q_aoff || !qlen || !goff || !tlen || !ch_off || !ch_aoff || !prob_off || !n_out) return TELR_E_ARG;
    auto bad = [&](const std::string &why) { ctx->err = "telr_debug_backtrack: " + why; return TELR_E_ARG; };
    TRY(check_map_opt(ctx, mo));
    if (nq < 1 || nq > (1 << 16)) return bad("nq must be 1..2^16");
    if (n_targets < 1 || n_targets > (1 << 24)) return bad("n_targets must be 1..2^24");
    if (q_aoff[0] != 0) return bad("q_aoff[0] must be 0");
    for (int q = 0; q < nq; ++q) if (q_aoff[q + 1] < q_aoff[q] || q_aoff[q + 1] > (1 << 22)) return bad("q_aoff must ascend (at most 2^22 anchors)");
    const int32_t na = q_aoff[nq];
    if (na > 0 && (!keys || !f || !p || !chains || !canch || !kept)) return TELR_E_ARG;
    if (prob_cap < 0 || (prob_cap > 0 && !probs)) return TELR_E_ARG;
    for (int t = 0; t < n_targets; ++t) {
        if (goff[t + 1] < goff[t] || goff[t + 1] >= (1u << 31)) return bad("goff must ascend below 2^31");
        if (tlen[t] < 0 || (uint32_t)tlen[t] > goff[t + 1] - goff[t]) return bad("tlen[" + std::to_string(t) + "] outside its piece of goff");
    }
    const int32_t max_link = (mo->flags & TELR_MF_CHAIN_SKIP) ? (int32_t)CHAIN_SCAN_H : mo->chain_lookback;
    bool any_over = false;
    for (int q = 0; q < nq; ++q) {
        const int32_t a0 = q_aoff[q], n = q_aoff[q + 1] - a0;
        if (qlen[q] < 0 || qlen[q] > (1 << 24)) return bad("qlen[" + std::to_string(q) + "] must be 0..2^24");
        if (n > SEGSORT_CAP) any_over = true;
        for (int32_t i = 0; i < n; ++i) {
            const uint64_t key = keys[a0 + i];
            const std::string at = "anchor " + std::to_string(i) + " of query " + std::to_string(q);
            if (p[a0 + i] < -1 || p[a0 + i] >= i) return bad(at + ": p must be -1 or an earlier anchor of the query");
            if (p[a0 + i] >= 0 && i - p[a0 + i] > max_link) return bad(at + ": link longer than the look-back (" + std::to_string(max_link) + ")");
            if ((uint32_t)A_G(key) < goff[0] || (uint32_t)A_G(key) >= goff[n_targets]) return bad(at + ": reference position outside goff");
            if (A_Q(key) >= qlen[q]) return bad(at + ": query position outside the query");
        }
    }
    n_out[0] = n_out[1] = n_out[2] = 0;
    for (int q = 0; q <= nq; ++q) ch_off[q] = 0;
    ch_aoff[0] = 0; prob_off[0] = 0;
    if (na == 0) return TELR_OK;
    HIPCHK(hipSetDevice(ctx->device));
    hipStream_t st = ctx->stream;
    uint64_t *d_keys; int32_t *d_qaoff, *d_f, *d_p, *d_qlen, *d_tlen; uint32_t *d_goff; int64_t *d_zero;
    TRY(ctx_buf_t(ctx, "dbg_bt_keys", (size_t)na, &d_keys));
    TRY(ctx_buf_t(ctx, "dbg_bt_qaoff", (size_t)nq + 1, &d_qaoff));
    TRY(ctx_buf_t(ctx, "dbg_bt_f", (size_t)na, &d_f));
    TRY(ctx_buf_t(ctx, "dbg_bt_p", (size_t)na, &d_p));
    TRY(ctx_buf_t(ctx, "dbg_bt_qlen", (size_t)nq, &d_qlen));
    TRY(ctx_buf_t(ctx, "dbg_bt_goff", (size_t)n_targets + 1, &d_goff));
    TRY(ctx_buf_t(ctx, "dbg_bt_tlen", (size_t)n_targets, &d_tlen));
    TRY(ctx_buf_t(ctx, "dbg_bt_zero", (size_t)std::max(nq, n_targets), &d_zero));
    HIPCHK(hipMemcpyAsync(d_keys, keys, (size_t)na * 8, hipMemcpyHostToDevice, st));
    HIPCHK(hipMemcpyAsync(d_qaoff, q_aoff, ((size_t)nq + 1) * 4, hipMemcpyHostToDevice, st));
    HIPCHK(hipMemcpyAsync(d_f, f, (size_t)na * 4, hipMemcpyHostToDevice, st));
    HIPCHK(hipMemcpyAsync(d_p, p, (size_t)na * 4, hipMemcpyHostToDevice, st));
    HIPCHK(hipMemcpyAsync(d_qlen, qlen, (size_t)nq * 4, hipMemcpyHostToDevice, st));
    HIPCHK(hipMemcpyAsync(d_goff, goff, ((size_t)n_targets + 1) * 4, hipMemcpyHostToDevice, st));
    HIPCHK(hipMemcpyAsync(d_tlen, tlen, (size_t)n_targets * 4, hipMemcpyHostToDevice, st));
    HIPCHK(hipMemsetAsync(d_zero, 0, (size_t)std::max(nq, n_targets) * 8, st));
    BtOut bt;
    TRY(backtrack_dispatch(ctx, st, mo, d_keys, d_qaoff, nq, na, any_over, nullptr, d_f, d_p, &bt));
    std::vector<int32_t> h_nch((size_t)nq + 1), h_choff((size_t)nq + 1), q_k0((size_t)nq + 1, 0);
    std::vector<ChainRec> h_rec((size_t)bt.npk_tot + 1);
    std::vector<uint64_t> h_canch((size_t)na);
    HIPCHK(hipMemcpyAsync(h_nch.data(), bt.d_nch, (size_t)nq * 4, hipMemcpyDeviceToHost, st));
    HIPCHK(hipMemcpyAsync(h_choff.data(), bt.d_choff, ((size_t)nq + 1) * 4, hipMemcpyDeviceToHost, st));
    if (bt.npk_tot) HIPCHK(hipMemcpyAsync(h_rec.data(), bt.d_rec, (size_t)bt.npk_tot * sizeof(ChainRec), hipMemcpyDeviceToHost, st));
    HIPCHK(hipMemcpyAsync(h_canch.data(), bt.d_canch, (size_t)na * 8, hipMemcpyDeviceToHost, st));
    HIPCHK(hipStreamSynchronize(st));
    std::vector<int32_t> row_of((size_t)bt.npk_tot + 1, -1);
    int64_t nch = 0, nca = 0;
    for (int q = 0; q < nq; ++q) {
        ch_off[q] = (int32_t)nch;
        for (int c = 0; c < h_nch[q]; ++c) {
            const ChainRec &r = h_rec[(size_t)h_choff[q] + c];
            if (nch >= na || r.cnt < 1 || r.a_off < 0 || nca + r.cnt > na || (int64_t)q_aoff[q] + r.a_off + r.cnt > q_aoff[q + 1]) { ctx->err = "telr_debug_backtrack: a chain record outside its query"; return TELR_E_RANGE; }
            chain_row(r, q, goff, n_targets, chains + nch * 9);
            row_of[(size_t)h_choff[q] + c] = (int32_t)nch;
            ch_aoff[nch] = (int32_t)nca;
            memcpy(canch + nca, h_canch.data() + q_aoff[q] + r.a_off, (size_t)r.cnt * 8);
            nca += r.cnt; ++nch;
        }
    }
    ch_off[nq] = (int32_t)nch; ch_aoff[nch] = (int32_t)nca;
    SelOut so;
    TRY(select1_dispatch(ctx, st, mo, bt.d_choff, bt.d_nch, bt.d_rec, bt.npk_tot, d_qaoff, nq, 0, d_qlen, d_zero, d_goff, d_tlen, d_zero, n_targets, any_over, nullptr,
                         true, h_nch.data(), q_k0.data(), &so));
    const int nk = so.nk;
    if (nk > nch) { ctx->err = "telr_debug_backtrack: more kept chains than chains"; return TELR_E_RANGE; }
    std::vector<uint64_t> h_sk2((size_t)bt.npk_tot + 1); std::vector<uint8_t> h_keep((size_t)bt.npk_tot + 1);
    if (bt.npk_tot) {
        HIPCHK(hipMemcpyAsync(h_sk2.data(), so.d_sk2, (size_t)bt.npk_tot * 8, hipMemcpyDeviceToHost, st));
        HIPCHK(hipMemcpyAsync(h_keep.data(), so.d_keep, (size_t)bt.npk_tot, hipMemcpyDeviceToHost, st));
        HIPCHK(hipStreamSynchronize(st));
    }
    int x = 0;
    for (int q = 0; q < nq; ++q) for (int i = 0; i < h_nch[q]; ++i) {
        if (!h_keep[(size_t)h_choff[q] + i]) continue;
        if (x >= nk) { ctx->err = "telr_debug_backtrack: the keep flags and the kept list disagree"; return TELR_E_RANGE; }
        const uint32_t c = (uint32_t)(h_sk2[(size_t)h_choff[q] + i] & 0xffffffffu);
        const KeptLite &L = so.hl[x];
        int32_t v[10] = { L.qid, L.score, L.cnt, L.rev, L.tid, L.rs, L.re, L.qs, L.qe, c < (uint32_t)h_nch[q] ? row_of[(size_t)h_choff[q] + c] : -1 };
        memcpy(kept + (size_t)x * 10, v, sizeof(v));
        ++x;
    }
    if (x != nk) { ctx->err = "telr_debug_backtrack: the keep flags and the kept list disagree"; return TELR_E_RANGE; }
    n_out[0] = nch; n_out[1] = nk;
// ... 374 lines not shown
```

Baseline: 23.39.

## Bias packed int16 DP scores to use plain integer add/sub in tagged cells

Adds a biased-score variant of the tagged packed int16 DP cells (TB4 nibble and TAG8). Initial values and boundaries are offset by a constant bias, and per-problem step limits are computed on the host so the two halves provably never overflow or underflow. Within those limits the saturating packed subtract and add are replaced by ordinary 32-bit add and subtract, which is cheaper per cell. It also adds build variants, one with the fast path disabled and one with a range-checking tap, plus debug exports, and it risks correctness if the bound analysis is wrong.

```diff
diff --git a/__graft_entry__.py b/__graft_entry__.py
--- a/__graft_entry__.py
+++ b/__graft_entry__.py
@@ -8,7 +8,7 @@
 
 def build():
     from telr_amd import build as tb
-    tb.build(verbose=True)
+    tb.build(verbose=True, variants=True)
     from oracle import binding as ob
     ob.build()
     import telr_amd
diff --git a/telr_amd/_lib.py b/telr_amd/_lib.py
--- a/telr_amd/_lib.py
+++ b/telr_amd/_lib.py
@@ -198,6 +198,10 @@
     L.telr_debug_mid_occ.restype = i32; L.telr_debug_mid_occ.argtypes = [vp, C.POINTER(MapOpt)]
     L.telr_debug_dp_limits.restype = C.c_int; L.telr_debug_dp_limits.argtypes = [C.POINTER(MapOpt), vp]
     L.telr_debug_dp_class_table.restype = C.c_int; L.telr_debug_dp_class_table.argtypes = [vp]
+    if hasattr(L, "telr_debug_pk_bias"):
+        L.telr_debug_pk_bias.restype = C.c_int; L.telr_debug_pk_bias.argtypes = [C.POINTER(MapOpt), vp]
+        L.telr_debug_pk_build.restype = C.c_int; L.telr_debug_pk_build.argtypes = [vp]
+        L.telr_debug_pk_range_tap.restype = i64; L.telr_debug_pk_range_tap.argtypes = [vp]
     L.telr_debug_map_plan.restype = C.c_int; L.telr_debug_map_plan.argtypes = [vp, i32, i32, C.c_double, C.c_int, C.c_int, C.c_int, C.c_int, vp, vp]
     L.telr_debug_dp.restype = C.c_int; L.telr_debug_dp.argtypes = [vp, vp, vp, C.POINTER(MapOpt), vp, i32, vp, vp, vp, i64]
     L.telr_debug_stitch.restype = C.c_int; L.telr_debug_stitch.argtypes = [vp, i32, vp, vp, vp, vp, vp, i32, vp, vp, i64]
diff --git a/telr_amd/aligner.py b/telr_amd/aligner.py
--- a/telr_amd/aligner.py
+++ b/telr_amd/aligner.py
@@ -134,6 +134,25 @@
         if rc != 0:
             raise _lib.TelrError("telr_debug_dp_limits: %d" % rc, rc)
         return dict(zip(Engine.DP_LIMITS, (int(v) for v in a)))
+
+    @staticmethod
+    def pk_bias(mo):
+        a = np.zeros(2, np.int32)
+        rc = _lib.lib().telr_debug_pk_bias(C.byref(mo), a.ctypes.data)
+        if rc != 0:
+            raise _lib.TelrError("telr_debug_pk_bias: %d" % rc, rc)
+        return int(a[0]), int(a[1])
+
+    @staticmethod
+    def pk_build():
+        a = np.zeros(4, np.int32)
+        rc = _lib.lib().telr_debug_pk_build(a.ctypes.data)
+        if rc != 0:
+            raise _lib.TelrError("telr_debug_pk_build: %d" % rc, rc)
+        return {"fullrate": int(a[0]), "range_tap": int(a[1]), "bias4": int(a[2]), "bias8": int(a[3])}
+
+    def pk_range_tap(self):
+        return int(self.L.telr_debug_pk_range_tap(self.h))
 
     DP_CLASS_COLUMNS = ("maxd", "lanes", "regs", "row_dwords", "interleaved", "tiled")
 
diff --git a/telr_amd/build.py b/telr_amd/build.py
--- a/telr_amd/build.py
+++ b/telr_amd/build.py
@@ -7,27 +7,46 @@
 SO = os.path.join(HERE, "libtelrhip.so")
 SOURCES = ["telr_engine.hip"]
 DEPS = sorted(f for f in os.listdir(SRC) if f.endswith((".hip", ".h"))) + ["../../include/telr_hip.h"]
+VARIANTS = {"fr0": ["-DPK_FULLRATE=0"], "tap": ["-DPK_RANGE_TAP"]}
+
+
+def variant_path(name):
+    return os.path.join(HERE, "libtelrhip_%s.so" % name)
+
+
+def _stale(so):
+    if not os.path.exists(so):
+        return True
+    t = os.path.getmtime(so)
+    return any(os.path.getmtime(os.path.join(SRC, d)) > t for d in DEPS)
 
 
 def needs_build():
-    if not os.path.exists(SO):
-        return True
-    t = os.path.getmtime(SO)
-    return any(os.path.getmtime(os.path.join(SRC, d)) > t for d in DEPS)
+    return _stale(SO)
 
 
-def build(force=False, verbose=False):
-    if not force and not needs_build():
-        return SO
+def _cmd(so, flags):
     hipcc = os.environ.get("HIPCC", "/opt/rocm/bin/hipcc")
-    cmd = [hipcc, "-O3", "-std=c++17", "--offload-arch=gfx950", "-fPIC", "-shared", "-o", SO] + \
-          os.environ.get("TELR_EXTRA_FLAGS", "").split() + [os.path.join(SRC, s) for s in SOURCES] + ["-lz"]
-    if verbose:
-        print(" ".join(cmd), file=sys.stderr)
-    subprocess.check_call(cmd)
+    return [hipcc, "-O3", "-std=c++17", "--offload-arch=gfx950", "-fPIC", "-shared", "-o", so] + \
+        os.environ.get("TELR_EXTRA_FLAGS", "").split() + flags + [os.path.join(SRC, s) for s in SOURCES] + ["-lz"]
+
+
+def build(force=False, verbose=False, variants=False):
+    todo = [(SO, [])] if force or _stale(SO) else []
+    if variants:
+        todo += [(variant_path(n), f) for n, f in VARIANTS.items() if force or _stale(variant_path(n))]
+    procs = []
+    for so, flags in todo:
+        cmd = _cmd(so, flags)
+        if verbose:
+            print(" ".join(cmd), file=sys.stderr)
+        procs.append((cmd, subprocess.Popen(cmd)))
+    failed = [(cmd, p.returncode) for cmd, p in procs if p.wait() != 0]
+    if failed:
+        raise subprocess.CalledProcessError(failed[0][1], failed[0][0])
     return SO
 
 
 if __name__ == "__main__":
-    build(force="--force" in sys.argv, verbose=True)
+    build(force="--force" in sys.argv, verbose=True, variants="--variants" in sys.argv)
     print(SO)
diff --git a/telr_amd/csrc/kernels.hip.h b/telr_amd/csrc/kernels.hip.h
--- a/telr_amd/csrc/kernels.hip.h
+++ b/telr_amd/csrc/kernels.hip.h
@@ -2338,6 +2338,7 @@
     int32_t *retry;
     int32_t tb4;
     int32_t tag8_steps;
+    int32_t bias_steps4, bias_steps8;
 };
 
 __device__ __forceinline__ int64_t d_wave_max64(int64_t v)
@@ -2899,15 +2900,21 @@
     return t | src;
 }
 
-template <int SH>
+#ifndef PK_FULLRATE
+#define PK_FULLRATE 1
+#endif
+constexpr int PK_BIAS4 = 0x4800, PK_BIAS8 = 0x5800;
+template <bool FR> __device__ __forceinline__ uint32_t pk_subc(uint32_t a, uint32_t c) { if constexpr (FR) return a - c; else return pk_sub(a, c); }
+template <bool FR> __device__ __forceinline__ uint32_t pk_addc(uint32_t a, uint32_t c) { if constexpr (FR) return a + c; else return pk_add(a, c); }
+template <int SH, bool FR = false>
 __device__ __forceinline__ uint32_t d_cell_pk4(const PkConst &c, uint32_t hd, uint32_t hl, uint32_t e1l, uint32_t hu, uint32_t f1u,
                                                uint32_t qb, uint32_t tbv, uint32_t &h, uint32_t &ve1, uint32_t &vf1)
 {
-    const uint32_t et = pk_max(pk_sub(hl, c.qe), pk_sub(e1l, c.e));
-    const uint32_t ft = pk_max(pk_sub(hu, c.qeF), pk_sub(f1u, c.e));
+    const uint32_t et = pk_max(pk_subc<FR>(hl, c.qe), pk_subc<FR>(e1l, c.e));
+    const uint32_t ft = pk_max(pk_subc<FR>(hu, c.qeF), pk_subc<FR>(f1u, c.e));
     asm("v_and_or_b32 %0, %1, %2, %3" : "=v"(ve1) : "v"(et), "v"(0xFFFCFFFCu), "v"(0x00010001u));
     vf1 = ft & 0xFFFCFFFCu;
-    uint32_t ne, hda = pk_add(hd, c.a), ht;
+    uint32_t ne, hda = pk_addc<FR>(hd, c.a), ht;
     asm("v_pk_min_u16 %0, %1, %2" : "=v"(ne) : "v"(qb ^ tbv), "v"(0x00010001u));
     asm("v_pk_mad_i16 %0, %1, %2, %3" : "=v"(ht) : "v"(ne), "v"(c.nab), "v"(hda));
     ht = pk_max(pk_max(ht, ve1), vf1);
@@ -2918,18 +2925,19 @@
     return SH ? n << SH : n;
 }
 
+template <bool FR = false>
 __device__ __forceinline__ uint32_t d_cell_pk8(const PkConst &c, uint32_t hd, uint32_t hl, uint32_t e1l, uint32_t e2l, uint32_t hu, uint32_t f1u, uint32_t f2u,
                                                uint32_t qb, uint32_t tbv, uint32_t &h, uint32_t &ve1, uint32_t &vf1, uint32_t &ve2, uint32_t &vf2)
 {
-    const uint32_t et1 = pk_max(pk_sub(hl, c.qe), pk_sub(e1l, c.e));
-    const uint32_t ft1 = pk_max(pk_sub(hu, c.qeF), pk_sub(f1u, c.e));
-    const uint32_t et2 = pk_max(pk_sub(hl, c.q2e2), pk_sub(e2l, c.e2));
-    const uint32_t ft2 = pk_max(pk_sub(hu, c.q2e2F), pk_sub(f2u, c.e2));
+    const uint32_t et1 = pk_max(pk_subc<FR>(hl, c.qe), pk_subc<FR>(e1l, c.e));
+    const uint32_t ft1 = pk_max(pk_subc<FR>(hu, c.qeF), pk_subc<FR>(f1u, c.e));
+    const uint32_t et2 = pk_max(pk_subc<FR>(hl, c.q2e2), pk_subc<FR>(e2l, c.e2));
+    const uint32_t ft2 = pk_max(pk_subc<FR>(hu, c.q2e2F), pk_subc<FR>(f2u, c.e2));
     asm("v_and_or_b32 %0, %1, %2, %3" : "=v"(ve1) : "v"(et1), "v"(0xFFF8FFF8u), "v"(0x00030003u));
     asm("v_and_or_b32 %0, %1, %2, %3" : "=v"(vf1) : "v"(ft1), "v"(0xFFF8FFF8u), "v"(0x00020002u));
     asm("v_and_or_b32 %0, %1, %2, %3" : "=v"(ve2) : "v"(et2), "v"(0xFFF8FFF8u), "v"(0x00010001u));
     vf2 = ft2 & 0xFFF8FFF8u;
-    uint32_t ne, hda = pk_add(hd, c.a), ht;
+    uint32_t ne, hda = pk_addc<FR>(hd, c.a), ht;
     asm("v_pk_min_u16 %0, %1, %2" : "=v"(ne) : "v"(qb ^ tbv), "v"(0x00010001u));
     asm("v_pk_mad_i16 %0, %1, %2, %3" : "=v"(ht) : "v"(ne), "v"(c.nab), "v"(hda));
     ht = pk_max(pk_max(ht, ve1), pk_max(vf1, pk_max(ve2, vf2)));
@@ -2986,13 +2994,31 @@
     return hi >= lo ? ((hi - lo) >> 1) + 1 : 0;
 }
 
-template <int LPP, int R, bool EXT, int NW = 1, int FULL = 0, bool ONEP = false, bool TB4 = false, bool TAG8 = false, bool CX = false>
+#ifdef PK_RANGE_TAP
+__device__ unsigned long long g_pk_range_tap;
+__device__ __forceinline__ uint32_t d_pk_out(uint32_t v, uint32_t lo, uint32_t hi)
+{
+    const uint32_t l = v & 0xffffu, h = v >> 16;
+    return (uint32_t)(l < lo || l > hi) + (uint32_t)(h < lo || h > hi);
+}
+#define PK_TAP(H, E1, F1, E2, F2) \
+    if constexpr (FR) { if (have && a <= mn) { _Pragma("unroll") for (int r = 0; r < R; ++r) { \
+        tap += d_pk_out(H[r], tap_lo, tap_hi) + d_pk_out(E1[r], tap_lo, tap_hi) + d_pk_out(F1[r], tap_lo, tap_hi); \
+        if constexpr (TAG8) tap += d_pk_out(E2[r], tap_lo, tap_hi) + d_pk_out(F2[r], tap_lo, tap_hi); } } }
+#else
+#define PK_TAP(H, E1, F1, E2, F2)
+#endif
+template <int LPP, int R, bool EXT, int NW = 1, int FULL = 0, bool ONEP = false, bool TB4 = false, bool TAG8 = false, bool CX = false, bool FR = false>
 __device__ __forceinline__ void d_dp_pkr(const DpArgs &A, const int32_t *__restrict__ list, int nlist, int first_prob, uint32_t *xch = nullptr)
 {
     static_assert(NW == 1 || LPP == 64 * NW, "multi-wave problems use whole waves");
     static_assert(!TB4 || (ONEP && LPP == 1 && !EXT), "nibble spill: one-piece cell, one problem per lane");
     static_assert(!TAG8 || (!ONEP && !TB4 && !EXT && NW == 1), "tagged two-piece cell: fills of the one-launch classes");
     static_assert(!CX || (!ONEP && !TB4 && !TAG8), "convex cell: plain flags, byte spill");
+    static_assert(!FR || TB4 || TAG8, "biased halves: the two tagged cells");
+    constexpr int BIAS = !FR ? 0 : TB4 ? PK_BIAS4 : PK_BIAS8;
+    constexpr uint32_t NEG = ((0xC000u + (uint32_t)BIAS) & 0xffffu) * 0x00010001u;
+    static_assert(BIAS % 8 == 0 && BIAS >= 0 && BIAS < 0x8000, "the bias keeps the tag bits");
     constexpr int RW = LPP * R;
     const int lane = threadIdx.x, sub = lane / LPP, l = lane % LPP;
     const int wv = NW > 1 ? lane >> 6 : 0, wl = lane & 63;
@@ -3005,7 +3031,7 @@
     c.ab = pk_dup(o.a + o.b); c.b = pk_dup(o.b); c.a = pk_dup(o.a); c.nab = pk_dup(-(o.a + o.b)); c.qeF = c.qe;
     c.q2e2F = c.q2e2;
     c.cx_oe0 = pk_dup(o.cx_open + d_cx_ext(o, 0)); c.cx_e1 = pk_dup(d_cx_ext(o, 1)); c.cx_emin = pk_dup(o.cx_emin); c.cx_dec = pk_dup(o.cx_dec);
-    const uint32_t XN = CX ? c.cx_emin : PK_NEG;
+    const uint32_t XN = CX ? c.cx_emin : NEG;
     if constexpr (TB4) {
         c.qe = pk_dup(4 * (o.q + o.e) - 2); c.qeF = pk_dup(4 * (o.q + o.e) - 1); c.e = pk_dup(4 * o.e);
         c.a = pk_dup(4 * o.a + 2); c.nab = pk_dup(-4 * (o.a + o.b));
@@ -3015,18 +3041,26 @@
         c.q2e2 = pk_dup(8 * (o.q2 + o.e2) - 2); c.q2e2F = pk_dup(8 * (o.q2 + o.e2) - 1); c.e2 = pk_dup(8 * o.e2);
         c.a = pk_dup(8 * o.a + 4); c.nab = pk_dup(-8 * (o.a + o.b));
     }
+#ifdef PK_RANGE_TAP
+    uint32_t tap = 0, tap_lo = c.qe & 0xffffu;
+    {
+        const uint32_t cs[5] = { c.qeF, c.e, TAG8 ? c.q2e2 : 0u, TAG8 ? c.q2e2F : 0u, TAG8 ? c.e2 : 0u };
+        for (int x = 0; x < 5; ++x) tap_lo = (cs[x] & 0xffffu) > tap_lo ? (cs[x] & 0xffffu) : tap_lo;
+    }
+    const uint32_t tap_hi = 32767u - (c.a & 0xffffu);
+#endif
     const int m = have ? P.m : 0, n = have ? P.n : 0, dlo = P.dlo;
     const int de0 = dlo + 4 * R * l;
     const int dhi = have ? P.dhi : dlo - 1;
     uint32_t He[R], E1e[R], E2e[R], F1e[R], F2e[R], Ho[R], E1o[R], E2o[R], F1o[R], F2o[R], inE[R], inO[R], qb[R], tbv[R];
 #pragma unroll
     for (int r = 0; r < R; ++r) {
-        He[r] = E1e[r] = F1e[r] = Ho[r] = E1o[r] = F1o[r] = PK_NEG; E2e[r] = F2e[r] = E2o[r] = F2o[r] = XN;
+        He[r] = E1e[r] = F1e[r] = Ho[r] = E1o[r] = F1o[r] = NEG; E2e[r] = F2e[r] = E2o[r] = F2o[r] = XN;
         if constexpr (TB4) { E1e[r] |= 0x00010001u; E1o[r] |= 0x00010001u; }
         if constexpr (TAG8) { E1e[r] |= 0x00030003u; E1o[r] |= 0x00030003u; F1e[r] |= 0x00020002u; F1o[r] |= 0x00020002u; E2e[r] |= 0x00010001u; E2o[r] |= 0x00010001u; }
         const int d0 = de0 + 4 * r;
-        if (d0 == 0) He[r] &= 0xffff0000u;
-        if (d0 + 2 == 0) He[r] &= 0x0000ffffu;
+        if (d0 == 0) He[r] = (He[r] & 0xffff0000u) | (uint32_t)BIAS;
+        if (d0 + 2 == 0) He[r] = (He[r] & 0x0000ffffu) | (uint32_t)BIAS << 16;
         inE[r] = (d0 <= dhi ? 0x0000ffffu : 0u) | (d0 + 2 <= dhi ? 0xffff0000u : 0u);
         inO[r] = (d0 + 1 <= dhi ? 0x0000ffffu : 0u) | (d0 + 3 <= dhi ? 0xffff0000u : 0u);
         qb[r] = 0; tbv[r] = 0;
@@ -3059,7 +3093,7 @@
     const int xf = (n - m) - de0;
     const bool fin_here = have && xf >= 0 && xf < 4 * R;
     const int fin_r = xf >> 2, fin_hi = (xf >> 1) & 1;
-    uint32_t fin = PK_NEG, te[R], prow[R];
+    uint32_t fin = NEG, te[R], prow[R];
 #pragma unroll
     for (int r = 0; r < R; ++r) { te[r] = 0; prow[r] = 0; }
     if (NW > 1) {
@@ -3072,24 +3106,25 @@
             const int a = 2 * k;
             if (qleft == 0) { d_stream_fill_acgt(QS, A.qseq2, P.qi0, qs_, ((a - de0) >> 1) - 1, P.qcomp, A.qtot); qleft = 32; }
             { uint32_t qv = (uint32_t)d_stream_next_acgt(QS); if (EXT && ((a - de0) >> 1) - 1 >= m) qv |= 8u; d_push_q<R>(qb, qv); } --qleft;
-            uint32_t ph = PK_NEG, pe1 = PK_NEG, pe2 = XN;
+            uint32_t ph = NEG, pe1 = NEG, pe2 = XN;
             if (LPP > 1) {
-                ph = DPP_SHR1((int)PK_NEG, (int)Ho[R - 1]); pe1 = DPP_SHR1((int)PK_NEG, (int)E1o[R - 1]); pe2 = DPP_SHR1((int)XN, (int)E2o[R - 1]);
+                ph = DPP_SHR1((int)NEG, (int)Ho[R - 1]); pe1 = DPP_SHR1((int)NEG, (int)E1o[R - 1]); pe2 = DPP_SHR1((int)XN, (int)E2o[R - 1]);
                 if (NW > 1 && wl == 0 && wv > 0) { const uint32_t *x = xch + (1 * NW + wv - 1) * 3; ph = x[0]; pe1 = x[1]; pe2 = x[2]; }
-                if (first) { ph = PK_NEG; pe1 = PK_NEG; pe2 = XN; }
+                if (first) { ph = NEG; pe1 = NEG; pe2 = XN; }
             }
 #pragma unroll
             for (int r = 0; r < R; ++r) {
                 const uint32_t lh = r ? Ho[r - 1] : ph, le1 = r ? E1o[r - 1] : pe1, le2 = r ? E2o[r - 1] : pe2;
                 const uint32_t hl = __builtin_amdgcn_alignbit(Ho[r], lh, 16), e1l = __builtin_amdgcn_alignbit(E1o[r], le1, 16), e2l = __builtin_amdgcn_alignbit(E2o[r], le2, 16);
-                if constexpr (TB4) { te[r] = d_cell_pk4<0>(c, He[r], hl, e1l, Ho[r], F1o[r], qb[r], tbv[r], h, ve1, vf1); ve2 = PK_NEG; vf2 = PK_NEG; }
-                else if constexpr (TAG8) te[r] = d_cell_pk8(c, He[r], hl, e1l, e2l, Ho[r], F1o[r], F2o[r], qb[r], tbv[r], h, ve1, vf1, ve2, vf2);
+                if constexpr (TB4) { te[r] = d_cell_pk4<0, FR>(c, He[r], hl, e1l, Ho[r], F1o[r], qb[r], tbv[r], h, ve1, vf1); ve2 = NEG; vf2 = NEG; }
+                else if constexpr (TAG8) te[r] = d_cell_pk8<FR>(c, He[r], hl, e1l, e2l, Ho[r], F1o[r], F2o[r], qb[r], tbv[r], h, ve1, vf1, ve2, vf2);
                 else if constexpr (CX) te[r] = d_cell_pk_cx(c, He[r], hl, e1l, e2l, Ho[r], F1o[r], F2o[r], qb[r], tbv[r], h, ve1, vf1, ve2, vf2);
                 else te[r] = d_cell_pk<ONEP>(c, He[r], hl, e1l, e2l, Ho[r], F1o[r], F2o[r], qb[r], tbv[r], h, ve1, vf1, ve2, vf2);
                 if (r < FULL) { He[r] = h; F1e[r] = vf1; F2e[r] = vf2; }
-                else { He[r] = (h & inE[r]) | (PK_NEG & ~inE[r]); F1e[r] = (vf1 & inE[r]) | (PK_NEG & ~inE[r]); F2e[r] = (vf2 & inE[r]) | (XN & ~inE[r]); }
+                else { He[r] = (h & inE[r]) | (NEG & ~inE[r]); F1e[r] = (vf1 & inE[r]) | (NEG & ~inE[r]); F2e[r] = (vf2 & inE[r]) | (XN & ~inE[r]); }
                 E1e[r] = ve1; E2e[r] = ve2;
             }
+            PK_TAP(He, E1e, F1e, E2e, F2e)
             if (!EXT && a >= amin) {
 #pragma unroll
                 for (int r = 0; r < R; ++r) if (a == mn && r == fin_r) { fin = He[r]; fin_off = off; }
@@ -3101,7 +3136,7 @@
             if (EXT) {
                 uint32_t hv[R];
 #pragma unroll
-                for (int r = 0; r < R; ++r) hv[r] = pk_sel(pk_sign(PKU(PKS(qb[r] | tbv[r]) << (pk_s2)(12))), PK_NEG, He[r]);
+                for (int r = 0; r < R; ++r) hv[r] = pk_sel(pk_sign(PKU(PKS(qb[r] | tbv[r]) << (pk_s2)(12))), NEG, He[r]);
                 const int cur_rel = d_pk_rowmax<LPP, R>(hv), cur = cur_rel + off;
                 if (!done) {
                     if (cur > best) { const int cd = d_pk_argd<LPP, R>(hv, cur_rel, de0, 0); best = cur; bi = (a - cd) >> 1; bj = (a + cd) >> 1; }
@@ -3115,11 +3150,11 @@
             const int a = 2 * k + 1;
             if (tleft == 0) { d_stream_fill_acgt(TS, A.tseq2, P.ti0, ts_, ((a + de0 + 1) >> 1) + 2 * R - 2, 0, A.ttot); tleft = 32; }
             { uint32_t tv = (uint32_t)d_stream_next_acgt(TS); if (EXT && ((a + de0 + 1) >> 1) + 2 * R - 2 >= n) tv |= 8u; d_push_t<R>(tbv, tv); } --tleft;
-            uint32_t nh = PK_NEG, nf1 = PK_NEG, nf2 = XN;
+            uint32_t nh = NEG, nf1 = NEG, nf2 = XN;
             if (LPP > 1) {
-                nh = DPP_SHL1((int)PK_NEG, (int)He[0]); nf1 = DPP_SHL1((int)PK_NEG, (int)F1e[0]); nf2 = DPP_SHL1((int)XN, (int)F2e[0]);
+                nh = DPP_SHL1((int)NEG, (int)He[0]); nf1 = DPP_SHL1((int)NEG, (int)F1e[0]); nf2 = DPP_SHL1((int)XN, (int)F2e[0]);
                 if (NW > 1 && wl == 63 && wv < NW - 1) { const uint32_t *x = xch + (0 * NW + wv + 1) * 3; nh = x[0]; nf1 = x[1]; nf2 = x[2]; }
-                if (last) { nh = PK_NEG; nf1 = PK_NEG; nf2 = XN; }
+                if (last) { nh = NEG; nf1 = NEG; nf2 = XN; }
             }
             uint32_t row[R];
 #pragma unroll
@@ -3127,15 +3162,16 @@
                 const uint32_t uh = r < R - 1 ? He[r + 1] : nh, uf1 = r < R - 1 ? F1e[r + 1] : nf1, uf2 = r < R - 1 ? F2e[r + 1] : nf2;
                 const uint32_t hu = __builtin_amdgcn_alignbit(uh, He[r], 16), f1u = __builtin_amdgcn_alignbit(uf1, F1e[r], 16), f2u = __builtin_amdgcn_alignbit(uf2, F2e[r], 16);
                 uint32_t t;
-                if constexpr (TB4) { t = d_cell_pk4<4>(c, Ho[r], He[r], E1e[r], hu, f1u, qb[r], tbv[r], h, ve1, vf1); ve2 = PK_NEG; vf2 = PK_NEG; }
-                else if constexpr (TAG8) t = d_cell_pk8(c, Ho[r], He[r], E1e[r], E2e[r], hu, f1u, f2u, qb[r], tbv[r], h, ve1, vf1, ve2, vf2);
+                if constexpr (TB4) { t = d_cell_pk4<4, FR>(c, Ho[r], He[r], E1e[r], hu, f1u, qb[r], tbv[r], h, ve1, vf1); ve2 = NEG; vf2 = NEG; }
+                else if constexpr (TAG8) t = d_cell_pk8<FR>(c, Ho[r], He[r], E1e[r], E2e[r], hu, f1u, f2u, qb[r], tbv[r], h, ve1, vf1, ve2, vf2);
                 else if constexpr (CX) t = d_cell_pk_cx(c, Ho[r], He[r], E1e[r], E2e[r], hu, f1u, f2u, qb[r], tbv[r], h, ve1, vf1, ve2, vf2);
                 else t = d_cell_pk<ONEP>(c, Ho[r], He[r], E1e[r], E2e[r], hu, f1u, f2u, qb[r], tbv[r], h, ve1, vf1, ve2, vf2);
                 if (r < FULL) { Ho[r] = h; F1o[r] = vf1; F2o[r] = vf2; }
-                else { Ho[r] = (h & inO[r]) | (PK_NEG & ~inO[r]); F1o[r] = (vf1 & inO[r]) | (PK_NEG & ~inO[r]); F2o[r] = (vf2 & inO[r]) | (XN & ~inO[r]); }
+                else { Ho[r] = (h & inO[r]) | (NEG & ~inO[r]); F1o[r] = (vf1 & inO[r]) | (NEG & ~inO[r]); F2o[r] = (vf2 & inO[r]) | (XN & ~inO[r]); }
                 E1o[r] = ve1; E2o[r] = ve2;
                 row[r] = TB4 ? (te[r] | t) : __builtin_amdgcn_perm(t, te[r], 0x06040200u);
             }
+            PK_TAP(Ho, E1o, F1o, E2o, F2o)
             if (!EXT && a >= amin) {
 #pragma unroll
                 for (int r = 0; r < R; ++r) if (a == mn && r == fin_r) { fin = Ho[r]; fin_off = off; }
@@ -3143,7 +3179,7 @@
             if (EXT) {
                 uint32_t hv[R];
 #pragma unroll
-                for (int r = 0; r < R; ++r) hv[r] = pk_sel(pk_sign(PKU(PKS(qb[r] | tbv[r]) << (pk_s2)(12))), PK_NEG, Ho[r]);
+                for (int r = 0; r < R; ++r) hv[r] = pk_sel(pk_sign(PKU(PKS(qb[r] | tbv[r]) << (pk_s2)(12))), NEG, Ho[r]);
                 const int cur_rel = d_pk_rowmax<LPP, R>(hv), cur = cur_rel + off;
                 if (!done) {
                     if (cur > best) { const int cd = d_pk_argd<LPP, R>(hv, cur_rel, de0, 1); best = cur; bi = (a - cd) >> 1; bj = (a + cd) >> 1; }
@@ -3264,8 +3300,11 @@
         }
         return;
     }
+#ifdef PK_RANGE_TAP
+    if (tap) atomicAdd(&g_pk_range_tap, (unsigned long long)tap);
+#endif
     if (fin_here) {
-        int sc = (int)(short)(fin_hi ? (fin >> 16) : (fin & 0xffffu)) + fin_off;
+        int sc = (int)(short)(fin_hi ? (fin >> 16) : (fin & 0xffffu)) + fin_off - BIAS;
         if constexpr (TB4) sc >>= 2;
         if constexpr (TAG8) sc >>= 3;
         DpRes Rr; Rr.score = sc; Rr.bi = m; Rr.bj = n; Rr.nops = 0; Rr.mlen = 0; Rr.cells = P.pad[1]; Rr.tbases = n; Rr.mcols = 0;
@@ -3301,25 +3340,25 @@
     const DpProb P0 = probs[*first];
     return P0.m + P0.n <= tag8_steps ? CELL_TAG8 : CELL_PLAIN;
 }
-template <int CLS, bool EXACT, bool ONEP, bool TB4, bool TAG8, bool CX>
+template <int CLS, bool EXACT, bool ONEP, bool TB4, bool TAG8, bool CX, bool FR = false>
 __device__ __forceinline__ void d_dp_pk_cls(const DpArgs &A, const int32_t *__restrict__ list, int n, int first)
 {
     static_assert(DP_CLASS[CLS].family == DPF_PK && EXACT == (DP_CLASS[CLS].layout == TBL_INTERLEAVED && CLS != CLS_PK16), "class table");
-    d_dp_pkr<DP_CLASS[CLS].lpp, DP_CLASS[CLS].regs, false, 1, EXACT ? DP_CLASS[CLS].regs - 1 : 0, ONEP, TB4, TAG8, CX>(A, list, n, first);
-}
-template <bool TAG8, bool CX>
+    d_dp_pkr<DP_CLASS[CLS].lpp, DP_CLASS[CLS].regs, false, 1, EXACT ? DP_CLASS[CLS].regs - 1 : 0, ONEP, TB4, TAG8, CX, FR>(A, list, n, first);
+}
+template <bool TAG8, bool CX, bool FR = false>
 __device__ __forceinline__ void d_dp_pk_any(int cls, const DpArgs &A, const int32_t *__restrict__ list, int n, int first)
 {
     switch (cls) {
-    case CLS_PK20: d_dp_pk_cls<CLS_PK20, true, false, false, TAG8, CX>(A, list, n, first); break;
-    case CLS_PK24: d_dp_pk_cls<CLS_PK24, true, false, false, TAG8, CX>(A, list, n, first); break;
-    case CLS_PK28: d_dp_pk_cls<CLS_PK28, true, false, false, TAG8, CX>(A, list, n, first); break;
-    case CLS_PK32: d_dp_pk_cls<CLS_PK32, true, false, false, TAG8, CX>(A, list, n, first); break;
-    case CLS_PK16: d_dp_pk_cls<CLS_PK16, false, false, false, TAG8, CX>(A, list, n, first); break;
-    case CLS_PK40: d_dp_pk_cls<CLS_PK40, false, false, false, TAG8, CX>(A, list, n, first); break;
-    case CLS_PK48: d_dp_pk_cls<CLS_PK48, false, false, false, TAG8, CX>(A, list, n, first); break;
-    case CLS_PK128: d_dp_pk_cls<CLS_PK128, false, false, false, TAG8, CX>(A, list, n, first); break;
-    default: d_dp_pk_cls<CLS_PK64, false, false, false, TAG8, CX>(A, list, n, first); break;
+    case CLS_PK20: d_dp_pk_cls<CLS_PK20, true, false, false, TAG8, CX, FR>(A, list, n, first); break;
+    case CLS_PK24: d_dp_pk_cls<CLS_PK24, true, false, false, TAG8, CX, FR>(A, list, n, first); break;
+    case CLS_PK28: d_dp_pk_cls<CLS_PK28, true, false, false, TAG8, CX, FR>(A, list, n, first); break;
+    case CLS_PK32: d_dp_pk_cls<CLS_PK32, true, false, false, TAG8, CX, FR>(A, list, n, first); break;
+    case CLS_PK16: d_dp_pk_cls<CLS_PK16, false, false, false, TAG8, CX, FR>(A, list, n, first); break;
+    case CLS_PK40: d_dp_pk_cls<CLS_PK40, false, false, false, TAG8, CX, FR>(A, list, n, first); break;
+    case CLS_PK48: d_dp_pk_cls<CLS_PK48, false, false, false, TAG8, CX, FR>(A, list, n, first); break;
+    case CLS_PK128: d_dp_pk_cls<CLS_PK128, false, false, false, TAG8, CX, FR>(A, list, n, first); break;
+    default: d_dp_pk_cls<CLS_PK64, false, false, false, TAG8, CX, FR>(A, list, n, first); break;
     }
 }
 #ifndef PK_WPE
@@ -3334,6 +3373,16 @@
     const int n = off.off[cls + 1] - off.off[cls];
     const int cell = d_pk_cell(cls, A.o, A.tb4, A.tag8_steps, A.probs, list + first);
     if (cell == CELL_CX) { d_dp_pk_any<false, true>(cls, A, list, n, first); return; }
+    if constexpr (PK_FULLRATE) {
+        const DpProb P0 = A.probs[list[first]];
+        const int steps = P0.m + P0.n;
+        if (cell == CELL_NIBBLE && steps <= A.bias_steps4) {
+            if (cls == CLS_PK16) d_dp_pk_cls<CLS_PK16, false, true, true, false, false, true>(A, list, n, first);
+            else d_dp_pk_cls<CLS_PK20, true, true, true, false, false, true>(A, list, n, first);
+            return;
+        }
+        if (cell == CELL_TAG8 && steps <= A.bias_steps8) { d_dp_pk_any<true, false, true>(cls, A, list, n, first); return; }
+    }
     if (cell >= CELL_ONEP && cls == CLS_PK16) { if (cell == CELL_NIBBLE) d_dp_pk_cls<CLS_PK16, false, true, true, false, false>(A, list, n, first); else d_dp_pk_cls<CLS_PK16, false, true, false, false, false>(A, list, n, first); return; }
     if (cell >= CELL_ONEP) { if (cell == CELL_NIBBLE) d_dp_pk_cls<CLS_PK20, true, true, true, false, false>(A, list, n, first); else d_dp_pk_cls<CLS_PK20, true, true, false, false, false>(A, list, n, first); return; }
     if (cell == CELL_TAG8) { d_dp_pk_any<true, false>(cls, A, list, n, first); return; }
diff --git a/telr_amd/csrc/telr_engine.hip b/telr_amd/csrc/telr_engine.hip
--- a/telr_amd/csrc/telr_engine.hip
+++ b/telr_amd/csrc/telr_engine.hip
@@ -1303,6 +1303,27 @@
     if (L.pk_steps && !cx && !one_launch && !no_tag8) L.tag8_steps = affine_steps(mo, 1975, 128, 4000, mo->q2, mo->e2);
     return L;
 }
+static void pk_bias_steps(const telr_map_opt *mo, int32_t *out)
+{
+    out[0] = out[1] = 0;
+    if (mo->cx_scale > 0 || mo->a < 0 || mo->b < 0) return;
+    const int a = mo->a > 0 ? mo->a : 1, b = mo->b > 0 ? mo->b : 1;
+    int Dw[2] = { 0, 0 };
+    for (const DpClassRow &r : DP_CLASS) if (r.family == DPF_PK) { if (r.nibble && r.maxd > Dw[0]) Dw[0] = r.maxd; if (r.maxd > Dw[1]) Dw[1] = r.maxd; }
+    for (int x = 0; x < 2; ++x) {
+        const int S = x ? 8 : 4, B = x ? PK_BIAS8 : PK_BIAS4, D = Dw[x];
+        const int go = x ? mo->q2 : mo->q, ge = x ? mo->e2 : mo->e;
+        int c_max = S * (mo->q + mo->e);
+        if (x && S * (mo->q2 + mo->e2) > c_max) c_max = S * (mo->q2 + mo->e2);
+        if (S * mo->e > c_max) c_max = S * mo->e;
+        const int a_max = S * mo->a + S / 2;
+        const int sink = (D + 1) / 2 * (S * mo->b + S / 2);
+        if (go < 0 || ge < 0 || 16384 + sink + 2 * c_max > B) continue;
+        const int by_b = 2 * ((B - 2 * c_max) / S - go - D * ge) / b - 2, by_a = 2 * (32767 - B - a_max - (S - 1)) / (S * a) - 2;
+        const int lim = by_b < by_a ? by_b : by_a;
+        out[x] = lim > 0 ? lim : 0;
+    }
+}
 typedef void (*DpKernel)(DpArgs);
 template <int CLS> static constexpr DpKernel reg_kernel() { return k_dp_reg<DP_CLASS[CLS].lpp, DP_CLASS[CLS].regs, (DP_CLASS[CLS].lpp + 63) / 64>; }
 template <int CLS> static constexpr DpKernel pkw_kernel() { return k_dp_pkw<DP_CLASS[CLS].lpp / 64>; }
@@ -1387,6 +1408,7 @@
     }
     D.tb = d_tb; D.cig = *d_rawcig_io; D.res = d_res; D.dcap = 0;
     D.retry = d_retry; D.tb4 = L.tb4_mask; D.tag8_steps = L.tag8_steps;
+    { int32_t bs[2]; pk_bias_steps(mo, bs); D.bias_steps4 = bs[0]; D.bias_steps8 = bs[1]; }
     static const bool tb_split = !ab_on("tb_one_launch");
     int nw = 0; uint32_t *d_wv2 = nullptr;
     {
@@ -2470,6 +2492,34 @@
     out[0] = L.pk_steps; out[1] = L.pk_wide; out[2] = L.pk_wide_maxd; out[3] = L.pk_ext;
     out[4] = L.pk_ext_maxd; out[5] = L.tb4_mask; out[6] = L.tb4_steps; out[7] = L.tag8_steps;
     return TELR_OK;
+}
+extern "C" int telr_debug_pk_bias(const telr_map_opt *mo, int32_t *out)
+{
+    if (!mo || !out) return TELR_E_ARG;
+    pk_bias_steps(mo, out);
+    return TELR_OK;
+}
+extern "C" int telr_debug_pk_build(int32_t *out)
+{
+    if (!out) return TELR_E_ARG;
+    out[0] = PK_FULLRATE; out[2] = PK_BIAS4; out[3] = PK_BIAS8;
+#ifdef PK_RANGE_TAP
+    out[1] = 1;
+#else
+    out[1] = 0;
+#endif
+    return TELR_OK;
+}
+extern "C" int64_t telr_debug_pk_range_tap(telr_ctx *ctx)
+{
+#ifdef PK_RANGE_TAP
+    if (!ctx || hipSetDevice(ctx->device) != hipSuccess || hipStreamSynchronize(ctx->stream) != hipSuccess) return -1;
+    unsigned long long v = 0, z = 0;
+    if (hipMemcpyFromSymbol(&v, HIP_SYMBOL(g_pk_range_tap), 8) != hipSuccess || hipMemcpyToSymbol(HIP_SYMBOL(g_pk_range_tap), &z, 8) != hipSuccess) return -1;
+    return (int64_t)v;
+#else
+    (void)ctx; return -1;
+#endif
 }
 extern "C" int telr_debug_dp_class_table(int32_t *out)
 {
```

New measurement: 23.29. No clear change (-0.4%).
